# YuePanEdward/MULLS

Hardware: AMD Instinct MI355X
Metric: scan-pair registrations/sec (64-beam ~120k pts, 20 ICP iters); dT vs ref (higher is better)
Workload: dtype f32

## Files before the change

mulls_amd/csrc/accum.h:

```cpp
#pragma once
#include "device_util.h"

namespace
{
__device__ __forceinline__ float w_dist_adaptive(float dist, int iter_num)
{
	const float unit_dist = 30.0f, b_min = 0.7f, b_max = 1.3f, b_step = 0.05f;
	float t = b_min + b_step * iter_num;
	float b_current = (t < b_max) ? t : b_max;
	float temp = (float)(b_current + (1.0 - b_current) * dist / unit_dist);
	temp = (float)((temp > 0.01) ? (double)temp : 0.01);
	return temp;
}
__device__ __forceinline__ float w_intensity(float i1, float i2)
{
	float ratio = fabsf(i1 - i2) / 255.0f;
	return (float)exp(-1.0 * ratio);
}
__device__ __forceinline__ float w_residual(float res, float thre)
{
	return (res > thre) ? ((2 * res * thre + (1 * 1 - 2 * 1) * (thre * thre)) / res / res) : 1.0f;
}
__device__ __forceinline__ int metric_of(int cls) { return (cls == 1 || cls == 3) ? 1 : (cls == 5 ? 2 : 0); }
}


__device__ __forceinline__ float point_wi(const float4 P, const float4 Q) { return w_intensity((float)(P.w + 0.0001), (float)(Q.w + 0.0001)); }

struct AccumCtx
{
	int metric, iter_num;
	bool residual_pass, dist_w, resid_w, inten_w, faithful;
	bool li_diag;
	float class_w, window;
};
__device__ __forceinline__ float class_weight(const RunParams &rp, int cls, bool residual_pass, const int cnt[MULLS_NC])
{
	if (rp.force_class_w)
		return rp.class_w_value;
	if (!residual_pass && rp.w_balance && (cls == 0 || cls == 4))
	{
		const int m1 = cnt[0] + cnt[4], m2 = cnt[2], m3 = cnt[1], m4 = cnt[3];
		const double v = rp.z_xy_ratio * (m2 + 2 * m3 - m4) / (0.0001 + 2.0 * m1);
		return (float)((0.01 > v) ? 0.01 : v);
	}
	return 1.0f;
}
__device__ __forceinline__ AccumCtx accum_ctx(const RunParams &rp, int cls, int iter_num, bool residual_pass, float class_w)
{
	AccumCtx A;
	A.metric = metric_of(cls);
	A.iter_num = iter_num;
	A.residual_pass = residual_pass;
	A.dist_w = rp.w_dist;
	A.resid_w = rp.w_resid && iter_num > rp.resid_from_iter;
	A.inten_w = rp.w_inten;
	A.faithful = rp.faithful;
	A.li_diag = A.metric == 1 && rp.faithful && rp.pull_comb && !residual_pass;
	A.class_w = class_w;
	A.window = A.metric == 0 ? rp.win_pl : (A.metric == 1 ? rp.win_li : rp.win_pt);
	return A;
}

__device__ __forceinline__ float corr_weight(const AccumCtx &A, int metric, const float4 P, const float4 Q, const float4 N, float wi)
{
	const float px = P.x, py = P.y, pz = P.z;
	const float qx = Q.x, qy = Q.y, qz = Q.z;
	const float dist = sqrtf(qx * qx + qy * qy + qz * qz);
	if (metric == 0)
	{
		float ntx = N.x, nty = N.y, ntz = N.z;
		float w = A.class_w;
		float dd = ntx * qx + nty * qy + ntz * qz - ntx * px - nty * py - ntz * pz;
		if (A.dist_w)
			w = w * w_dist_adaptive(dist, A.iter_num);
		if (A.resid_w)
			w = w * w_residual(fabsf(dd), A.window);
		if (A.inten_w)
			w = w * wi;
		return w;
	}
	if (metric == 1)
	{
		float vx = N.x, vy = N.y, vz = N.z;
		float dx = px - qx, dy = py - qy, dz = pz - qz;
		const double b0 = -vy * dz + vz * dy, b1 = -vz * dx + vx * dz, b2 = -vx * dy + vy * dx;
		float ex = (float)fabs(b0), ey = (float)fabs(b1), ez = (float)fabs(b2);
		float ed = sqrtf(ex * ex + ey * ey + ez * ez);
		float wx = A.class_w;
		if (A.dist_w)
			wx *= w_dist_adaptive(dist, A.iter_num);
		if (A.inten_w)
			wx *= wi;
		if (A.resid_w)
			wx = wx * w_residual(ed, A.window);
		return wx;
	}
	float dx = px - qx, dy = py - qy, dz = pz - qz;
	float wx = A.class_w;
	if (A.dist_w)
		wx = wx * w_dist_adaptive(dist, A.iter_num);
	if (A.resid_w)
		wx = wx * w_residual(sqrtf(dx * dx + dy * dy + dz * dz), A.window);
	if (A.inten_w)
		wx = wx * wi;
	return wx;
}

__device__ __forceinline__ constexpr int li_slot(int k) { return k == 0 ? 0 : (k == 6 ? 1 : (k == 11 ? 2 : (k == 15 ? 3 : (k == 18 ? 4 : (k == 20 ? 5 : (k >= 21 ? k - 15 : -1)))))); }
__device__ __forceinline__ constexpr int li_term(int slot) { return slot == 0 ? 0 : (slot == 1 ? 6 : (slot == 2 ? 11 : (slot == 3 ? 15 : (slot == 4 ? 18 : (slot == 5 ? 20 : slot + 15))))); }
#define ACC(k, v)                                              \
	do                                                         \
	{                                                          \
		if (MODE == 1)                                         \
		{                                                      \
			if (li_slot(k) >= T0 && li_slot(k) < T0 + NT)      \
				t[li_slot(k) >= T0 ? li_slot(k) - T0 : 0] = (TS)(v); \
		}                                                      \
		else if ((k) >= T0 && (k) < T0 + NT)                   \
			t[(k)-T0] = (TS)(v);                               \
	} while (0)
template <typename TS, int T0, int NT, int MODE = 0, int METRIC = -1>
__device__ __forceinline__ void point_terms(const AccumCtx &A, const double *x, const float4 P, const float4 Q, const float4 N, float wi, float &wdg, TS t[NT],
											 const float *wpre = nullptr)
{
	const int metric = METRIC >= 0 ? METRIC : A.metric;
	const bool residual_pass = A.residual_pass, faithful = A.faithful;
	const float px = P.x, py = P.y, pz = P.z;
	const float qx = Q.x, qy = Q.y, qz = Q.z;

	if (residual_pass)
	{
				const float cw = wdg;
		if (metric == 0)
		{
			float ntx = N.x, nty = N.y, ntz = N.z;
			float a = ntz * py - nty * pz;
			float b = ntx * pz - ntz * px;
			float c = nty * px - ntx * py;
			float dd = ntx * qx + nty * qy + ntz * qz - ntx * px - nty * py - ntz * pz;
			float res = (float)(ntx * x[0] + nty * x[1] + ntz * x[2] + a * x[3] + b * x[4] + c * x[5] - dd);
			ACC(0, cw * res * res);
			ACC(1, 1.0);
		}
		else
		{
			float dx = px - qx, dy = py - qy, dz = pz - qz;
			double A[3][6], bb[3];
			if (metric == 1)
			{
				float vx = N.x, vy = N.y, vz = N.z;
				A[0][0] = 0;
				A[0][1] = vz;
				A[0][2] = -vy;
				A[0][3] = -vz * pz - vy * py;
				A[0][4] = vy * px;
				A[0][5] = vz * px;
				A[1][0] = -vz;
				A[1][1] = 0;
				A[1][2] = vx;
				A[1][3] = vx * py;
				A[1][4] = -vx * px - vz * pz;
				A[1][5] = vz * py;
				A[2][0] = vy;
				A[2][1] = -vx;
				A[2][2] = 0;
				A[2][3] = vx * pz;
				A[2][4] = vy * pz;
				A[2][5] = -vy * py - vx * px;
				bb[0] = -vz * dy + vy * dz;
				bb[1] = -vx * dz + vz * dx;
				bb[2] = -vy * dx + vx * dy;
			}
			else
			{
				A[0][0] = 1, A[0][1] = 0, A[0][2] = 0, A[0][3] = 0, A[0][4] = pz, A[0][5] = -py;
				A[1][0] = 0, A[1][1] = 1, A[1][2] = 0, A[1][3] = -pz, A[1][4] = 0, A[1][5] = px;
				A[2][0] = 0, A[2][1] = 0, A[2][2] = 1, A[2][3] = py, A[2][4] = -px, A[2][5] = 0;
				bb[0] = -dx, bb[1] = -dy, bb[2] = -dz;
			}
			double r[3];
			for (int k = 0; k < 3; k++)
			{
				double t = 0;
				for (int j = 0; j < 6; j++)
					t += A[k][j] * x[j];
				r[k] = t - bb[k];
			}
			ACC(0, cw * (r[0] * r[0] + r[1] * r[1] + r[2] * r[2]));
			ACC(1, 3.0);
		}
		return;
	}

	if (metric == 0)
	{
		float ntx = N.x, nty = N.y, ntz = N.z;
		float a = ntz * py - nty * pz;
		float b = ntx * pz - ntz * px;
		float c = nty * px - ntx * py;
		float dd = ntx * qx + nty * qy + ntz * qz - ntx * px - nty * py - ntz * pz;
		const float w = wpre ? *wpre : corr_weight(A, 0, P, Q, N, wi);
		wdg = w;
		ACC(0, w * ntx * ntx);
		ACC(1, w * ntx * nty);
		ACC(2, w * ntx * ntz);
		ACC(3, w * a * ntx);
		ACC(4, w * b * ntx);
		ACC(5, w * c * ntx);
		ACC(6, w * nty * nty);
		ACC(7, w * nty * ntz);
		ACC(8, w * a * nty);
		ACC(9, w * b * nty);
		ACC(10, w * c * nty);
		ACC(11, w * ntz * ntz);
		ACC(12, w * a * ntz);
// ... 181 lines not shown
	{
		__syncthreads();
		if (threadIdx.x < 21 && li_slot((int)threadIdx.x) < 0)
			part[threadIdx.x] = 0.0;
		if (HALF)
		{
			slot_terms<double, 0, 6, 1, LANES>(A, x, valid, P, Q, N, wi, wdg, static_cast<double *>(R));
			__syncthreads();
			reduce_terms<double, 0, 6, 1, LANES>(static_cast<const double *>(R), part);
			__syncthreads();
			slot_terms<double, 6, 6, 1, LANES>(A, x, valid, P, Q, N, wi, wdg, static_cast<double *>(R));
			__syncthreads();
			reduce_terms<double, 6, 6, 1, LANES>(static_cast<const double *>(R), part);
		}
		else
		{
			slot_terms<double, 0, 12, 1, LANES>(A, x, valid, P, Q, N, wi, wdg, static_cast<double *>(R));
			__syncthreads();
			reduce_terms<double, 0, 12, 1, LANES>(static_cast<const double *>(R), part);
		}
	}
	else if (A.metric == 1 && HALF)
	{
		__syncthreads();
		slot_terms<double, 0, 7, 0, LANES>(A, x, valid, P, Q, N, wi, wdg, static_cast<double *>(R));
		__syncthreads();
		reduce_terms<double, 0, 7, 0, LANES>(static_cast<const double *>(R), part);
		__syncthreads();
		slot_terms<double, 7, 7, 0, LANES>(A, x, valid, P, Q, N, wi, wdg, static_cast<double *>(R));
		__syncthreads();
		reduce_terms<double, 7, 7, 0, LANES>(static_cast<const double *>(R), part);
		__syncthreads();
		slot_terms<double, 14, 7, 0, LANES>(A, x, valid, P, Q, N, wi, wdg, static_cast<double *>(R));
		__syncthreads();
		reduce_terms<double, 14, 7, 0, LANES>(static_cast<const double *>(R), part);
		__syncthreads();
		slot_terms<double, 21, 6, 0, LANES>(A, x, valid, P, Q, N, wi, wdg, static_cast<double *>(R));
		__syncthreads();
		reduce_terms<double, 21, 6, 0, LANES>(static_cast<const double *>(R), part);
	}
	else if (A.metric == 1)
	{
		__syncthreads();
		slot_terms<double, 0, 13, 0, LANES>(A, x, valid, P, Q, N, wi, wdg, static_cast<double *>(R));
		__syncthreads();
		reduce_terms<double, 0, 13, 0, LANES>(static_cast<const double *>(R), part);
		__syncthreads();
		slot_terms<double, 13, 13, 0, LANES>(A, x, valid, P, Q, N, wi, wdg, static_cast<double *>(R));
		__syncthreads();
		reduce_terms<double, 13, 13, 0, LANES>(static_cast<const double *>(R), part);
		__syncthreads();
		slot_terms<double, 26, 1, 0, LANES>(A, x, valid, P, Q, N, wi, wdg, static_cast<double *>(R));
		__syncthreads();
		reduce_terms<double, 26, 1, 0, LANES>(static_cast<const double *>(R), part);
	}
	else if (HALF)
	{
		__syncthreads();
		slot_terms<float, 0, 14, 0, LANES>(A, x, valid, P, Q, N, wi, wdg, static_cast<float *>(R));
		__syncthreads();
		reduce_terms<float, 0, 14, 0, LANES>(static_cast<const float *>(R), part);
		__syncthreads();
		slot_terms<float, 14, 13, 0, LANES>(A, x, valid, P, Q, N, wi, wdg, static_cast<float *>(R));
		__syncthreads();
		reduce_terms<float, 14, 13, 0, LANES>(static_cast<const float *>(R), part);
	}
	else
	{
		__syncthreads();
		slot_terms<float, 0, 27, 0, LANES>(A, x, valid, P, Q, N, wi, wdg, static_cast<float *>(R));
		__syncthreads();
		reduce_terms<float, 0, 27, 0, LANES>(static_cast<const float *>(R), part);
	}
	__syncthreads();
}

template <bool HALF = false, int LANES = MULLS_ACC_LANES>
__device__ __forceinline__ void trip_sum(const AccumCtx &A, const double *x, const CloudDesc &d, uint32_t trip0, const float4 *__restrict__ spos,
										  const float4 *__restrict__ mq, const uint8_t *__restrict__ flag, float *__restrict__ wd, void *R, double *part)
{
	const uint32_t s = trip0 + threadIdx.x;
	bool valid = false;
	float4 P = make_float4(0.0f, 0.0f, 0.0f, 0.0f), Q = P, N = P;
	float w = 0.0f, w0 = 0.0f;
	uint32_t g = 0;
	if (s < d.src_n)
	{
		g = d.src_off + s;
		const uint32_t f = flag[g];
		P = spos[g], Q = mq[2u * g], N = mq[2u * g + 1u];
		w = w0 = wd[g];
		valid = (f & (MULLS_F_ALIVE | MULLS_F_VALID)) == (MULLS_F_ALIVE | MULLS_F_VALID);
	}
	trip_sum_regs<HALF, LANES>(A, x, valid, P, Q, N, w, R, part);
	if (valid && __float_as_uint(w) != __float_as_uint(w0))
		wd[g] = w;
}

__device__ __forceinline__ void combine_rows(const RunParams &rp, bool want_residual, const double (*sums)[MULLS_NTERM_PAD], double *comb, int t)
{
	const int order[MULLS_NC] = {0, 2, 4, 1, 3, 5};
	double val;
	if (want_residual)
	{
		val = 0.0;
		if (t < 2)
			for (int i = 0; i < MULLS_NC; i++)
				if (rp.used[order[i]])
					val += sums[order[i]][t];
	}
	else if (t < 21)
	{
		int r = 0, rem = t;
		while (rem >= 6 - r)
		{
			rem -= 6 - r;
			r++;
		}
		const bool diag = rem == 0;
		double lower = 0.0, upper = 0.0;
		for (int i = 0; i < MULLS_NC; i++)
		{
			const int cls = order[i];
			if (!rp.used[cls])
				continue;
			const double v = sums[cls][t];
			if (metric_of(cls) == 1 && !diag)
				upper += v;
			else
				lower += v;
		}
		val = diag ? lower : (rp.faithful ? lower : lower + upper);
	}
	else
	{
		val = 0.0;
		for (int i = 0; i < MULLS_NC; i++)
			if (rp.used[order[i]])
				val += sums[order[i]][t];
	}
	comb[t] = val;
}
```

mulls_amd/csrc/batch.cpp:

```cpp
#include "batch.h"

namespace mulls_drv
{
void rows12(const double colmajor[16], double out[12])
{
	for (int r = 0; r < 3; r++)
		for (int c = 0; c < 4; c++)
			out[r * 4 + c] = colmajor[r + 4 * c];
}


void fill_crop_box(const RunParams &rp, const double tgt_bound[6], const uint32_t keys[6], mulls_result &R)
{
	R.cropped = rp.crop ? 1 : 0;
	for (int k = 0; k < 3 && rp.crop; k++)
	{
		const uint32_t kmin = keys[k], kmax = keys[3 + k];
		const bool none = kmin == 0xffffffffu && kmax == 0u;
		const double mmin = none ? 1.7976931348623157e308 : (double)ord_to_float(kmin);
		const double mmax = none ? -1.7976931348623157e308 : (double)ord_to_float(kmax);
		const double b1min = tgt_bound[k], b1max = tgt_bound[3 + k];
		const float pad = 1.0f;
		R.crop_box[k] = ((b1min > mmin) ? b1min : mmin) - pad;
		R.crop_box[3 + k] = ((b1max < mmax) ? b1max : mmax) + pad;
// ... 241 lines not shown
		for (int p = 0; p < B->n; p++)
			for (int c = 0; c < MULLS_NC; c++)
				if (P->used_feature_type[c] == '1')
					for (uint32_t s = 0; s < B->descs_h[p * MULLS_NC + c].src_cap; s += MULLS_SRC_PER_BLOCK)
					{
						Job j = {(uint32_t)p, (uint32_t)c, s, MULLS_SRC_PER_BLOCK};
						B->cjobs_h.push_back(j);
					}
	}
	B->bjobs_h.clear();
	B->fjobs_h.clear();
	B->ejobs_h.clear();
	bool any_class_job = false;
	for (int p = 0; p < B->n; p++)
		for (int c = 0; c < MULLS_NC; c++)
		{
			const CloudDesc &d = B->descs_h[p * MULLS_NC + c];
			if (!used[c] || d.src_cap == 0 || d.tier != MULLS_TIER_BM)
				continue;
			const bool whole = mode == 3 && d.src_cap <= MULLS_BIG_CLASS_MAX;
			if (whole)
			{
				Job j = {(uint32_t)p, (uint32_t)c, 0u, d.src_cap | MULLS_JOB_CLASS};
				B->bjobs_h.push_back(j);
				any_class_job = true;
			}
			for (uint32_t s = 0; s < d.src_cap; s += MULLS_SRC_PER_BLOCK)
			{
				Job j = {(uint32_t)p, (uint32_t)c, s, MULLS_SRC_PER_BLOCK};
				B->ejobs_h.push_back(j);
				if (!whole)
				{
					B->bjobs_h.push_back(j);
					B->fjobs_h.push_back(j);
				}
			}
		}
	if (!any_class_job)
		B->ejobs_h.clear();
	B->cjobs_dev_h = B->cjobs_h;
	{
		auto first_of = [&](uint32_t pair) {
			return std::lower_bound(B->cjobs_dev_h.begin(), B->cjobs_dev_h.end(), pair, [](const Job &j, uint32_t q) { return j.pair < q; });
		};
		auto cost = [&](const Job &j) {
			const CloudDesc &d = B->descs_h[j.pair * MULLS_NC + j.cls];
			return (uint64_t)j.count * (uint64_t)(64u + d.tgt_n0 / 64u);
		};
		for (int k = 0; k < nsub; k++)
			std::stable_sort(first_of((uint32_t)((long)B->n * k / nsub)), first_of((uint32_t)((long)B->n * (k + 1) / nsub)),
							 [&](const Job &a, const Job &b) { return cost(a) > cost(b); });
	}
	B->tjobs_h.clear();
	for (int p = 0; p < B->n; p++)
		for (int c = 0; c < MULLS_NC; c++)
			if (P->used_feature_type[c] == '1' && B->descs_h[p * MULLS_NC + c].tier == MULLS_TIER_BM)
				for (uint32_t s = 0; s < B->descs_h[p * MULLS_NC + c].tgt_n0; s += MULLS_BLOCK)
				{
					Job j = {(uint32_t)p, (uint32_t)c, s, 0};
					B->tjobs_h.push_back(j);
				}
	B->ajobs_h.clear();
	{
		for (int k = 0; k < 2; k++)
			for (int b = 0; b < 4; b++)
				B->ajob_split[k][b] = 0;
		for (int k = 0; k < nsub; k++)
		{
			const uint32_t lo = (uint32_t)((long)B->n * k / nsub), hi = (uint32_t)((long)B->n * (k + 1) / nsub);
			for (int bucket = 0; bucket < 3; bucket++)
			{
				B->ajob_split[k][bucket] = (uint32_t)B->ajobs_h.size();
				for (uint32_t j = 0; j < (uint32_t)B->jobs_h.size(); j++)
				{
					const Job &jb = B->jobs_h[j];
					if (jb.start % 1024u != 0u || jb.pair < lo || jb.pair >= hi)
						continue;
					const uint32_t slots = std::min(1024u, B->descs_h[jb.pair * MULLS_NC + jb.cls].src_cap - jb.start);
					if ((slots > 512u ? 0 : (slots > 256u ? 1 : 2)) == bucket)
						B->ajobs_h.push_back(j);
				}
			}
			B->ajob_split[k][3] = (uint32_t)B->ajobs_h.size();
		}
	}
	{
		std::vector<uint32_t> &tab = B->setup_tab_h;
		tab.clear();
		const uint32_t *trips = tgt_grid_bucket_trips();
		for (int k = 0; k < MULLS_TG_BUCKETS; k++)
		{
			B->tg_split[k] = (uint32_t)tab.size();
			for (uint32_t ci = 0; ci < (uint32_t)B->descs_h.size(); ci++)
			{
				const CloudDesc &d = B->descs_h[ci];
				const uint32_t need = (d.tgt_n0 + 511u) / 512u;
				if (d.tier == MULLS_TIER_LDS && need <= trips[k] && (k == 0 || need > trips[k - 1]))
					tab.push_back(ci);
			}
		}
		B->tg_split[MULLS_TG_BUCKETS] = (uint32_t)tab.size();
		for (int seg = 0; seg < 3; seg++)
		{
			B->crop_split[seg] = (uint32_t)tab.size();
			for (uint32_t ci = 0; ci < (uint32_t)B->descs_h.size(); ci++)
			{
				const bool lds = B->descs_h[ci].tier == MULLS_TIER_LDS;
				if (seg == 0 ? !B->src_one_wg[ci / MULLS_NC] : (seg == 1 ? !lds : lds))
					tab.push_back(ci * 2u + (seg ? 1u : 0u));
			}
		}
		B->crop_split[3] = (uint32_t)tab.size();
		B->srcp_split[0] = (uint32_t)tab.size();
		for (int p = 0; p < B->n; p++)
			if (B->src_one_wg[p])
				tab.push_back((uint32_t)p);
		B->srcp_split[1] = (uint32_t)tab.size();
	}
	B->njobs = (uint32_t)B->jobs_h.size();
	B->jobs_key = key;
}

int wait_epoch_word(mulls_ctx *ctx, volatile uint32_t *word, uint32_t want, hipEvent_t last, hipStream_t stream)
{
	const auto t0 = std::chrono::steady_clock::now();
	bool seen = false;
	for (uint64_t spins = 0;; spins++)
	{
		if (*word == want)
		{
			std::atomic_thread_fence(std::memory_order_acquire);
			seen = true;
			break;
		}
		if ((spins & 0xfff) == 0xfff && std::chrono::duration<double>(std::chrono::steady_clock::now() - t0).count() > 2.0)
			break;
	}
	if (seen && ctx->profiling != 1)
		return MULLS_OK;
	if (seen && last)
	{
		hipError_t e;
		while ((e = hipEventQuery(last)) == hipErrorNotReady)
		{
		}
		if (e == hipSuccess)
			return MULLS_OK;
	}
	HIPCHK(ctx, hipStreamSynchronize(stream ? stream : ctx->stream));
	if (*word != want)
	{
		ctx->err = "device did not publish the iteration epoch";
		return MULLS_E_HIP;
	}
	return MULLS_OK;
}

void unpack_out(const mulls_batch *B, const uint8_t used[MULLS_NC], int p, PairOut &o, bool comb)
{
	int n_used = 0;
	for (int c = 0; c < MULLS_NC; c++)
		n_used += used[c] ? 1 : 0;
	const size_t row = sizeof(double) * MULLS_NTERM_PAD, rec = 128 + row * (size_t)(comb ? 1 : n_used);
	const unsigned char *src = reinterpret_cast<const unsigned char *>(B->outs_h) + rec * (size_t)p;
	std::memcpy(o.n_valid, src, 128);
	src += 128;
// ... 366 lines not shown
	B->fill_ms = std::chrono::duration<double>(std::chrono::steady_clock::now() - t_fill0).count() * 1e3;
	B->fill_pack_ms = pack_s * 1e3;
	B->fill_bytes = (uint64_t)stage_rec * 16;
	return MULLS_OK;
}

int prepare_run(mulls_ctx *ctx, mulls_batch *B, const mulls_params *P_jobs, RunParams &rp, uint32_t *lds_cap_out, int *tier_out, int nsub, bool allow_mixed)
{
	hipStream_t st = ctx->stream;
	const int n = B->n;
	uint32_t lds_cap = 0;
	const int tier = choose_tier(ctx, B, rp.used, &lds_cap, allow_mixed ? P_jobs : nullptr);
	if (tier < 0)
	{
		ctx->err = "nn mode 3 (grid staged in LDS) needs every searched target class cloud to hold <= 9728 points";
		return MULLS_E_INVALID;
	}
	build_jobs(B, P_jobs, nsub > 0 ? nsub : subbatch_count(ctx, n), tier);
	*lds_cap_out = lds_cap;
	*tier_out = tier;
	int n_used = 0;
	for (int c = 0; c < MULLS_NC; c++)
		n_used += rp.used[c];
	rp.bm_h0 = 0.0f;
	rp.bm_maxwords = rp.bm_stride = 0u;
	rp.grid_h0 = ctx->opt[MULLS_OPT_GRID_H0] > 0.0 ? std::max(0.05f, (float)ctx->opt[MULLS_OPT_GRID_H0]) : MULLS_GRID_H0;
	rp.lds_dedup = 0;
	rp.grid_maxcells = MULLS_MAXCELLS;
	rp.cell_stride = ((rp.grid_maxcells + 1u + 15u) & ~15u);
	if (tier == 2 || tier == 3)
	{
		rp.grid_maxcells = lds_cells_for(lds_cap);
		const bool class_level = tier == 3 || (!B->cjobs_h.empty() && B->cjobs_h[0].count != MULLS_SRC_PER_BLOCK);
		const long left = 160L * 1024L - 64L - (long)MULLS_LDS_CELL_RESERVE - (long)MULLS_LDS_QCHUNK * 16L - (long)MULLS_LDS_AUX - (long)lds_cap * 18L;
		const bool dedup_fits = !rp.normal_shooting && left / 2 - 8 >= 4096 && ctx->opt[MULLS_OPT_LDS_DEDUP] != 0.0;
		if (tier == 3 && !dedup_fits)
		{
			ctx->err = "internal: a mixed batch whose LDS-tier clouds do not fit the on-chip duplicate table";
			return MULLS_E_INVALID;
		}
		if (class_level && dedup_fits)
		{
			rp.lds_dedup = 1;
			rp.grid_maxcells = (uint32_t)std::min<long>(left / 2 - 8, (long)MULLS_MAXCELLS);
		}
		rp.cell_stride = ((rp.grid_maxcells + 1u + 15u) & ~15u);
	}
	const size_t nl = B->lclouds_h.size();
	if (nl)
	{
		rp.bm_h0 = MULLS_BM_H0;
		rp.bm_auto = 1;
		if (ctx->opt[MULLS_OPT_BM_H0] > 0.0)
		{
			rp.bm_h0 = std::max(0.05f, (float)ctx->opt[MULLS_OPT_BM_H0]);
			rp.bm_auto = 0;
		}
		size_t words = std::min<size_t>(MULLS_BM_MAXWORDS, MULLS_BM_TOTALWORDS / nl);
		words = std::max<size_t>(words & ~(size_t)15, 4096);
		rp.bm_maxwords = rp.bm_stride = (uint32_t)words;
	}

	bool grew = false, g2 = false;
	int rc = MULLS_OK;
	auto A = [&](int r) { if (rc == MULLS_OK) rc = r; };
	A(grow(ctx, &B->jobs, &B->cap_jobs[0], (size_t)B->njobs, &g2));
	grew |= g2;
	A(grow(ctx, &B->partial, &B->cap_jobs[1], (size_t)B->njobs * MULLS_NTERM));
	A(grow(ctx, &B->tjobs, &B->cap_jobs[2], B->tjobs_h.size(), &g2));
	grew |= g2;
	A(grow(ctx, &B->cjobs, &B->cap_jobs[3], B->cjobs_h.size(), &g2));
	grew |= g2;
	A(grow(ctx, &B->bjobs, &B->cap_bjobs[0], B->bjobs_h.size(), &g2));
	grew |= g2;
	A(grow(ctx, &B->fjobs, &B->cap_bjobs[1], B->fjobs_h.size(), &g2));
	grew |= g2;
	A(grow(ctx, &B->lclouds, &B->cap_bjobs[2], B->lclouds_h.size(), &g2));
	grew |= g2;
	A(grow(ctx, &B->ejobs, &B->cap_bjobs[3], B->ejobs_h.size(), &g2));
	grew |= g2;
	A(grow(ctx, &B->wl, &B->cap_wl, B->cjobs_h.size()));
	A(grow(ctx, &B->ajobs, &B->cap_ajobs, B->ajobs_h.size(), &g2));
	grew |= g2;
	A(grow(ctx, &B->setup_tab, &B->cap_setup_tab, B->setup_tab_h.size(), &g2));
	grew |= g2;
	if (!B->wl_ctr)
		A(dmalloc(ctx, &B->wl_ctr, 16));
	if (rc == MULLS_OK)
		HIPCHK(ctx, hipMemsetAsync(B->wl_ctr, 0, 16 * sizeof(uint32_t), st));
	A(grow(ctx, &B->descs_init, &B->cap_jobs[4], B->descs_h.size(), &g2));
	grew |= g2;
	A(grow(ctx, &B->bbox_init, &B->cap_jobs[5], (size_t)n * 6, &g2));
	grew |= g2;
	if (tier == 2 || tier == 3)
		A(grow(ctx, &B->cell_start, &B->cap_cells[1], (size_t)n * n_used * rp.cell_stride));
	if (nl)
	{
		const size_t words = nl * (size_t)rp.bm_stride, cells = B->n_tgt + (size_t)n * MULLS_NC + 1;
		A(grow(ctx, &B->bm, &B->cap_bm, words));
		A(grow(ctx, &B->pf, &B->cap_pf, words));
		A(grow(ctx, &B->bm_cs, &B->cap_bm_cs, cells));
		A(grow(ctx, &B->cell_cnt, &B->cap_cells[0], cells));
		A(grow(ctx, &B->bm_rank, &B->cap_bm_rank, 2 * B->n_tgt));
		if (rc == MULLS_OK)
		{
			HIPCHK(ctx, hipMemsetAsync(B->cell_cnt, 0, cells * sizeof(uint32_t), st));
		}
	}
	if (rc != MULLS_OK)
		return rc;
	if (grew || B->dev_key != B->jobs_key || B->dev_key.empty())
	{
		SegCopier up(ctx);
		up.add_host(B->jobs, B->jobs_h.data(), sizeof(Job) * B->njobs);
		up.add_host(B->tjobs, B->tjobs_h.data(), sizeof(Job) * B->tjobs_h.size());
		up.add_host(B->cjobs, B->cjobs_dev_h.data(), sizeof(Job) * B->cjobs_dev_h.size());
		up.add_host(B->bjobs, B->bjobs_h.data(), sizeof(Job) * B->bjobs_h.size());
		up.add_host(B->fjobs, B->fjobs_h.data(), sizeof(Job) * B->fjobs_h.size());
		up.add_host(B->ejobs, B->ejobs_h.data(), sizeof(Job) * B->ejobs_h.size());
		up.add_host(B->lclouds, B->lclouds_h.data(), sizeof(uint32_t) * B->lclouds_h.size());
		up.add_host(B->ajobs, B->ajobs_h.data(), sizeof(uint32_t) * B->ajobs_h.size());
		up.add_host(B->setup_tab, B->setup_tab_h.data(), sizeof(uint32_t) * B->setup_tab_h.size());
		up.add_host(B->descs_init, B->descs_h.data(), sizeof(CloudDesc) * B->descs_h.size());
		up.add_host(B->bbox_init, B->bbox_h, sizeof(uint32_t) * 6 * n);
		if (up.flush(st) != MULLS_OK)
		{
			(void)hipStreamSynchronize(st);
			return MULLS_E_HIP;
		}
		HIPCHK(ctx, hipStreamSynchronize(st));
		B->dev_key = B->jobs_key;
	}
	{
		SegCopier reset(ctx);
		reset.add_dev(B->descs, B->descs_init, sizeof(CloudDesc) * B->descs_h.size());
		reset.add_dev(B->bbox, B->bbox_init, sizeof(uint32_t) * 6 * n);
		if (reset.flush(st) != MULLS_OK)
			return MULLS_E_HIP;
	}
	return MULLS_OK;
}


bool setup_former_shape(const RunParams &rp) { return rp.debug_stop == 30u; }

void queue_clone_crop(hipStream_t st, const mulls_batch *B, const RunParams &rp)
{
	const uint32_t nbig_segs = (uint32_t)B->big_segs_h.size(), nbig_clouds = (uint32_t)B->big_clouds_h.size();
	if (setup_former_shape(rp))
	{
		launch_clone_src(st, *B, rp, (uint32_t)B->setup_jobs_h.size());
		launch_crop(st, *B, rp, (uint32_t)B->n, nbig_segs, nbig_clouds);
		return;
	}
	const bool one_wg = !rp.undistort;
	launch_clone_src(st, *B, rp, one_wg ? B->n_setup_jobs_rest : (uint32_t)B->setup_jobs_h.size());
	if (one_wg)
		launch_src_setup(st, *B, rp, B->setup_tab + B->srcp_split[0], B->srcp_split[1] - B->srcp_split[0]);
	if (one_wg)
		launch_crop(st, *B, rp, (uint32_t)B->n, nbig_segs, nbig_clouds, B->setup_tab + B->crop_split[0], B->crop_split[rp.tgt_map ? 2 : 3] - B->crop_split[0]);
	else
		launch_crop(st, *B, rp, (uint32_t)B->n, nbig_segs, nbig_clouds);
}

int apply_keep_masks(mulls_ctx *ctx, const mulls_batch *B, const std::vector<uint8_t> &skeep, const std::vector<uint8_t> &tkeep, const char *what)
{
	hipStream_t st = ctx->stream;
	uint8_t *d_sk = nullptr, *d_tk = nullptr;
	if (dmalloc(ctx, &d_sk, skeep.size()) != MULLS_OK || dmalloc(ctx, &d_tk, tkeep.size()) != MULLS_OK)
		return MULLS_E_HIP;
	hipError_t e = hipMemcpyAsync(d_sk, skeep.data(), skeep.size(), hipMemcpyHostToDevice, st);
	if (e == hipSuccess)
		e = hipMemcpyAsync(d_tk, tkeep.data(), tkeep.size(), hipMemcpyHostToDevice, st);
	if (e == hipSuccess)
	{
		launch_thin(st, *B, (uint32_t)B->n, d_sk, d_tk);
		e = hipStreamSynchronize(st);
	}
	(void)hipFree(d_sk);
	(void)hipFree(d_tk);
	if (e != hipSuccess)
	{
		ctx->err = std::string(what) + hipGetErrorString(e);
		return MULLS_E_HIP;
	}
	return MULLS_OK;
}

void queue_target_grids(hipStream_t st, const mulls_batch *B, const RunParams &rp, int tier, bool fused_tgt)
{
	if (fused_tgt && setup_former_shape(rp))
		(void)launch_tgt_grid(st, *B, rp, (uint32_t)B->n);
	else if (fused_tgt)
		(void)launch_tgt_grid(st, *B, rp, (uint32_t)B->n, B->setup_tab, B->tg_split);
	else if (tier == 2)
		launch_grid_build_sort(st, *B, rp, (uint32_t)B->n);
	launch_bm_build(st, *B, (uint32_t)B->lclouds_h.size(), (uint32_t)B->tjobs_h.size());
}

int queue_tier_search(mulls_ctx *ctx, const mulls_batch *B, const RunParams &rp, int tier, uint32_t lds_cap, uint32_t parity)
{
	hipStream_t st = ctx->stream;
	if (tier == 2)
	{
// ... 51 lines not shown
```

mulls_amd/csrc/batch.h:

```cpp
#pragma once
#include <hip/hip_runtime_api.h>

#include <algorithm>
#include <atomic>
#include <chrono>
#include <cmath>
#include <cstdio>
#include <cstdlib>
#include <cstring>
#include <string>
#include <vector>

#include "../../include/mulls_hip.h"
#include "device_types.h"
#include "hostmath.h"
#include "icp_step.h"
#include "launch.h"
#include "ctx.h"

struct SegCopier
{
	mulls_ctx *ctx;
	std::vector<CopySeg> segs;
	struct Pending
	{
		void *dst;
		const void *src;
		size_t bytes;
	};
	std::vector<Pending> host;
	explicit SegCopier(mulls_ctx *c) : ctx(c) {}
	void add_host(void *dst, const void *src, size_t bytes)
	{
		if (bytes)
			host.push_back({dst, src, bytes});
	}
	void add_dev(void *dst, const void *src, size_t bytes)
	{
		const size_t piece = (size_t)0xfffffff0u;
		for (size_t off = 0; off < bytes; off += piece)
		{
			const size_t b = std::min(piece, bytes - off);
			segs.push_back({(unsigned long long)(uintptr_t)dst + off, (unsigned long long)(uintptr_t)src + off, (uint32_t)b, 0u});
		}
	}
	int flush(hipStream_t st);
};

struct mulls_batch : BatchDev
{
	int n = 0;
	size_t n_src = 0, n_tgt = 0;
	std::vector<CloudDesc> descs_h;
	std::vector<PairSetup> setup_h;
	std::vector<Job> setup_jobs_h;
	uint32_t n_setup_jobs_rest = 0;
	std::vector<uint8_t> src_one_wg;
	std::vector<uint32_t> setup_tab_h;
	uint32_t tg_split[MULLS_TG_BUCKETS + 1] = {}, crop_split[4] = {}, srcp_split[2] = {};
	size_t cap_setup_tab = 0;
	std::vector<Job> big_segs_h, big_clouds_h;
	uint32_t n_big_tgt = 0;
	std::vector<Job> jobs_h;
	std::vector<Job> cjobs_h;
	std::vector<Job> cjobs_dev_h;
	std::vector<Job> bjobs_h;
	std::vector<Job> fjobs_h;
	std::vector<Job> ejobs_h;
	std::vector<uint32_t> lclouds_h;
	int tier_mode = -1;
	std::vector<Job> tjobs_h;
	std::vector<uint32_t> ajobs_h;
	uint32_t ajob_split[2][4] = {{0, 0, 0, 0}, {0, 0, 0, 0}};
	IcpOut *icp_outs_pin = nullptr;
	size_t cap_icp_pin = 0;
	std::string jobs_key;
	uint32_t njobs = 0;
	uint4 *nn_cand = nullptr;
	LiveWord *live_mask = nullptr;
	size_t cap_live = 0;
	uint32_t tick = 1;
	size_t cap_outs = 0;
	size_t cap_big[4] = {};
	size_t cap_bjobs[4] = {};
	size_t cap_bm_cs = 0;
	size_t cap_bm_rank = 0;
	size_t cap_ajobs = 0;
	size_t cap_icp_outs = 0;
	size_t cap_steps = 0;
	uint32_t epoch2 = 0, epoch3 = 0;
	int nsub = 1;
	double fill_ms = 0.0, fill_pack_ms = 0.0;
	uint64_t fill_bytes = 0;
	size_t cap_wl = 0;
	unsigned long long *dbg = nullptr;
	size_t cap_bm = 0, cap_pf = 0;
	PairState *states_h = nullptr;
	PairOut *outs_h = nullptr;
	volatile uint32_t *epoch_h = nullptr;
	uint32_t *epoch_dev = nullptr;
	uint32_t epoch = 0;
	uint32_t epoch1 = 0;
	uint32_t *bbox_h = nullptr;
	uint8_t *upload_h = nullptr;
	CloudDesc *descs_init = nullptr;
	uint32_t *bbox_init = nullptr;
	std::string dev_key;
	size_t cap_jobs[6] = {}, cap_cells[2] = {};
	size_t cap_stage = 0, cap_src[13] = {}, cap_tgt[5] = {}, cap_pairs[5] = {}, cap_setup_jobs = 0, cap_pin[4] = {};
};

namespace mulls_drv
{
using mulls::Mat4;
using mulls::Mat6;

inline float ord_to_float(uint32_t k)
{
	const uint32_t u = (k & 0x80000000u) ? (k & 0x7fffffffu) : ~k;
	float f;
	std::memcpy(&f, &u, sizeof(f));
	return f;
}
inline int metric_of(int c) { return (c == MULLS_PILLAR || c == MULLS_BEAM) ? 1 : (c == MULLS_VERTEX ? 2 : 0); }
inline int packed(int r, int c) { return r * 6 - r * (r - 1) / 2 + (c - r); }
void rows12(const double colmajor[16], double out[12]);

struct PairHost : mulls::PairIter
{
	bool first = true;
	uint32_t alive_prev[MULLS_NC];
};

void fill_crop_box(const RunParams &rp, const double tgt_bound[6], const uint32_t keys[6], mulls_result &R);
int check_params(mulls_ctx *ctx, const mulls_params *P);
void init_cert(const mulls_ctx *ctx, RunParams &rp);
int subbatch_count(const mulls_ctx *ctx, int n);
void options_init(mulls_ctx *ctx);
bool option_value_ok(int option, double *value);
uint32_t lds_dedup_max_pts();
void assign_tiers(mulls_batch *B, const uint8_t used[MULLS_NC], int mode);
void build_jobs(mulls_batch *B, const mulls_params *P, int nsub, int mode);
int wait_epoch_word(mulls_ctx *ctx, volatile uint32_t *word, uint32_t want, hipEvent_t last = nullptr, hipStream_t stream = nullptr);
inline int wait_epoch(mulls_ctx *ctx, mulls_batch *B) { return wait_epoch_word(ctx, B->epoch_h, B->epoch); }
void unpack_out(const mulls_batch *B, const uint8_t used[MULLS_NC], int p, PairOut &o, bool comb = false);
uint32_t lds_cells_for(uint32_t cap);
int choose_tier(const mulls_ctx *ctx, const mulls_batch *B, const uint8_t used[MULLS_NC], uint32_t *lds_cap, const mulls_params *P_mixed = nullptr);
int batch_fill(mulls_ctx *ctx, mulls_batch *B, const mulls_pair *pairs, int n, const mulls_params *P = nullptr);
int prepare_run(mulls_ctx *ctx, mulls_batch *B, const mulls_params *P_jobs, RunParams &rp, uint32_t *lds_cap_out, int *tier_out, int nsub = 0, bool allow_mixed = false);
void queue_clone_crop(hipStream_t st, const mulls_batch *B, const RunParams &rp);
bool setup_former_shape(const RunParams &rp);
int apply_keep_masks(mulls_ctx *ctx, const mulls_batch *B, const std::vector<uint8_t> &skeep, const std::vector<uint8_t> &tkeep, const char *what);
void queue_target_grids(hipStream_t st, const mulls_batch *B, const RunParams &rp, int tier, bool fused_tgt);
int queue_tier_search(mulls_ctx *ctx, const mulls_batch *B, const RunParams &rp, int tier, uint32_t lds_cap, uint32_t parity);
mulls::IcpConst icp_const(const mulls_params *P);
int take_epochs(mulls_ctx *ctx, mulls_batch *B, uint32_t n, RunParams &rp);

struct EvTimer
{
	mulls_ctx *ctx;
	hipStream_t stream = nullptr;
	int base = 0;
	int used = 0;
	bool open = false;
	double *slot[5];
	void begin(double *acc)
	{
		open = ctx->profiling == 1 || (ctx->profiling == 2 && acc == &ctx->prof.ms_nn);
		if (!open)
			return;
		slot[used / 2] = acc;
		(void)hipEventRecord(ctx->ev[base + used], stream ? stream : ctx->stream);
// ... 27 lines not shown
```

mulls_amd/csrc/big_tier.h:

```cpp
#pragma once
#include "lds_tier.h"

namespace
{
__device__ __forceinline__ void grp16_min2(nnkey &bk, float &sec)
{
	nnkey g = bk;
	dpp_min_step<0xB1>(g);
	dpp_min_step<0x4E>(g);
	dpp_min_step<0x141>(g);
	dpp_min_step<0x140>(g);
	float c = (bk == g) ? sec : key_dist(bk);
	dpp_fmin_step<0xB1>(c);
	dpp_fmin_step<0x4E>(c);
	dpp_fmin_step<0x141>(c);
	dpp_fmin_step<0x140>(c);
	sec = c;
	bk = g;
}
__device__ __forceinline__ void take_one(const float4 c, float px, float py, float pz, nnkey &bk, float &sec)
{
	const float dx = px - c.x, dy = py - c.y, dz = pz - c.z;
	const float dist = (dx * dx + dy * dy) + dz * dz;
	sec = __builtin_amdgcn_fmed3f(sec, dist, key_dist(bk));
// ... 437 lines not shown
		}
	}
	if (U)
	{
		const bool dbg = rp.dbg_ticks && rp.debug_stop == 21u;
		const unsigned long long t_dbg = dbg ? wall_clock64() : 0ull;
		const uint32_t sub = threadIdx.x & (MULLS_GRID_GROUP - 1u), grp = threadIdx.x / MULLS_GRID_GROUP;
		const bool probe_own = tgt_n >= 4u * g.nocc;
		for (uint32_t i = grp; i < U; i += BLK / MULLS_GRID_GROUP)
		{
			nnkey bk;
			float sec, Rfin;
			CandOut co = {0xffffffffu, 0xffffffffu, 0.0f};
			search_query_bm(g, B, ts, CL.uq[i], C.r, C.m, sub, probe_own, bk, sec, Rfin, co);
			if (sub == 0)
			{
				const uint32_t slot = CL.us[i] & ~MULLS_US16_KCERT, s = q0 + slot, gi = d.src_off + s;
				const float best = key_dist(bk);
				const int bi = (int)(uint32_t)bk;
				const bool matched = bi >= 0 && !((double)best > C.max_dist_sqr);
				if (class_level)
					CL.res[slot] = make_uint2(matched ? (uint32_t)bi : 0xffffffffu, __float_as_uint(best));
				else
				{
					nn_idx[gi] = matched ? bi : -1;
					nn_d2[gi] = best;
				}
				const float lb_new = fminf(sqrtf(sec), Rfin);
				hint2[gi] = make_int2(bi, __float_as_int(lb_new));
				if (C.cand)
					C.cand[gi] = make_uint4(co.cx, co.cy, __float_as_uint(fminf(sqrtf(co.b2), Rfin) - lb_new), C.epoch);
				if (matched)
				{
					matched_cnt++;
					if (C.gate)
						claim((uint32_t)bi, s);
				}
			}
		}
		if (dbg)
		{
			__syncthreads();
			if (threadIdx.x == 0)
			{
				atomicAdd(&rp.dbg_ticks[13], (unsigned long long)U);
				atomicAdd(&rp.dbg_ticks[7], wall_clock64() - t_dbg);
			}
		}
	}
	for (int off = 32; off > 0; off >>= 1)
		matched_cnt += __shfl_down(matched_cnt, off);
	if (!class_level)
	{
#pragma unroll
		for (int k = 0; k < TRIPS; k++)
			if ((ST[k] & MULLS_FS_ALIVE) && M[k] != MULLS_NEEDS_SEARCH)
			{
				const uint32_t gi = d.src_off + q0 + threadIdx.x + (uint32_t)k * BLK;
				nn_idx[gi] = M[k];
				nn_d2[gi] = D0[k];
			}
		if ((threadIdx.x & 63) == 0)
			CL.red[threadIdx.x >> 6] = matched_cnt;
		__syncthreads();
		if (threadIdx.x == 0)
		{
			uint32_t any = 0;
			for (int w = 0; w < BLK / 64; w++)
				any |= CL.red[w];
			if (any)
				d.n_matched = 1u;
		}
		return;
	}
	if ((threadIdx.x & 63) == 0)
		CL.red[threadIdx.x >> 6] = matched_cnt;
	__threadfence_block();
	__syncthreads();
	uint32_t total_matched = 0;
	for (int w = 0; w < BLK / 64; w++)
		total_matched += CL.red[w];

	const float thr = ps.thr[cls], max_sqr = thr * thr;
	const bool any_match = total_matched > 0u, strict = rp.rej_strict != 0;
	uint32_t n_alive = 0, n_valid = 0;
#pragma unroll
	for (int k = 0; k < TRIPS; k++)
	{
		const uint32_t st = ST[k];
		if (!(st & MULLS_FS_ALIVE))
			continue;
		const uint32_t s = q0 + threadIdx.x + (uint32_t)k * BLK, gi = d.src_off + s;
		int32_t m = M[k];
		float dist = D0[k];
		bool standing = (st & MULLS_FS_STANDING) != 0;
		if (m == MULLS_NEEDS_SEARCH)
		{
			const uint2 found = CL.res[threadIdx.x + (uint32_t)k * BLK];
			m = (int32_t)found.x;
			standing = m >= 0 && __float_as_int(dist) == m;
			dist = __uint_as_float(found.y);
		}
		if (hashed && m >= 0 && big_hash_get(CL, (uint32_t)m) != s)
			m = -1;
		bool alive = true, valid, dir_ok = (st & MULLS_FS_DIR_OK) != 0;
		if (any_match)
		{
			valid = m >= 0;
			if (C.gate && m < 0)
			{
				alive = false;
				valid = false;
			}
			if (valid)
			{
				valid = strict ? dist < max_sqr : !(dist > max_sqr);
				if (valid)
				{
					wd[gi] = dist;
					if (!standing)
					{
						match[gi] = m;
						const float4 q2 = tpos[d.tgt_off + (uint32_t)m], n2 = tnrm[d.tgt_off + (uint32_t)m];
						mq[2u * gi] = q2;
						mq[2u * gi + 1u] = n2;
						if (normal_check)
						{
							const float3 n1 = *reinterpret_cast<const float3 *>(snrm + gi);
							const double dot = (double)n1.x * (double)n2.x + (double)n1.y * (double)n2.y + (double)n1.z * (double)n2.z;
							const float c = (float)fabs(dot);
							dir_ok = !((double)c < rp.cos_bearing);
						}
					}
				}
			}
		}
		else if (C.gate)
		{
			alive = false;
			valid = false;
		}
		else
			valid = (st & MULLS_FS_VALID) != 0;
		if (valid && normal_check && !dir_ok)
			valid = false;
		const uint32_t nf = (alive ? MULLS_F_ALIVE : 0u) | (valid ? MULLS_F_VALID : 0u);
		if (nf != (st & (MULLS_FS_ALIVE | MULLS_FS_VALID)))
			flag[gi] = (uint8_t)nf;
		n_alive += alive ? 1u : 0u;
		n_valid += valid ? 1u : 0u;
	}
	for (int off = 32; off > 0; off >>= 1)
	{
		n_alive += __shfl_down(n_alive, off);
		n_valid += __shfl_down(n_valid, off);
	}
	if ((threadIdx.x & 63) == 0)
	{
		CL.red[BLK / 64 + (threadIdx.x >> 6)] = n_alive;
		CL.red[2 * (BLK / 64) + (threadIdx.x >> 6)] = n_valid;
	}
	__syncthreads();
	if (threadIdx.x == 0)
	{
		uint32_t ta = 0, tv = 0;
		for (int w = 0; w < BLK / 64; w++)
		{
			ta += CL.red[BLK / 64 + w];
			tv += CL.red[2 * (BLK / 64) + w];
		}
		d.n_matched = total_matched;
		d.alive_next = ta;
		d.valid_next = tv;
		d.n_search = U;
	}
}
}
```

mulls_amd/csrc/device_types.h:

```cpp
#pragma once
#include <stdint.h>

#define MULLS_NC 6
#define MULLS_NTERM 27
#define MULLS_BLOCK 256
#define MULLS_SRC_PER_THREAD 2
#define MULLS_SRC_PER_BLOCK (MULLS_BLOCK * MULLS_SRC_PER_THREAD)
#define MULLS_NN_BLOCK 128
#define MULLS_NN_PTS 4
#define MULLS_TILE 2048

#define MULLS_MAXCELLS 65536u
#define MULLS_BM_MAXWORDS (1u << 22)
#define MULLS_BM_TOTALWORDS (1u << 28)
#define MULLS_BM_H0 0.25f
#define MULLS_LDS_BLOCK 1024
#define MULLS_LDS_MAXPTS 9728u
#define MULLS_ACC_BLOCK 128
#define MULLS_LDS_QCHUNK 1024u
#define MULLS_LDS_AUX (320u + 2u * MULLS_LDS_QCHUNK)
#define MULLS_CERT_BLOCK 512
#define MULLS_CERT_SMALL 64u
#define MULLS_CERT_SMALL_LOCKSTEP 512u
#define MULLS_LDS_CELL_RESERVE 9216
// ... 40 lines not shown
	uint32_t src_cap;
	uint32_t big_slot;
	uint32_t src_big_slot;
	uint32_t n_search;
	uint32_t stage_fmt;
	uint32_t tier;
	uint32_t grid_slot;
	uint32_t src_c;
	uint32_t compacted;
};
struct LiveWord
{
	unsigned long long alive;
	uint32_t below, pad_;
};
#define MULLS_STAGE_AOS48 0u
#define MULLS_STAGE_PACK32 1u
#define MULLS_STAGE_PACK28 2u

struct GridDesc
{
	float ox, oy, oz;
	float inv_h, h;
	uint32_t nx, ny, nz;
	uint32_t ncell;
	uint32_t cell_off;
	uint32_t wpr;
	uint32_t nocc;
};

struct PairState
{
	double T[12];
	double x[6];
	float thr[MULLS_NC];
	int32_t iter;
	int32_t active;
	int32_t want_residual;
	int32_t pad_[3];
};

struct PairSetup
{
	double guess[12];
	double tgt_bound[6];
	double inv_q[4];
	double inv_t[4];
};

#define MULLS_NTERM_PAD 28
struct PairOut
{
	double sums[MULLS_NC][MULLS_NTERM_PAD];
	double comb[MULLS_NTERM_PAD];
	uint32_t n_valid[MULLS_NC];
	uint32_t n_alive[MULLS_NC];
	uint32_t src_n[MULLS_NC];
	uint32_t tgt_n[MULLS_NC];
	uint32_t bbox[6];
	uint32_t pad_[2];
};

struct IcpOut
{
	double T[16];
	double info[36];
	double sigma2;
	unsigned long long src_pts, tgt_pts, corr_pts;
	float ratio;
	int32_t code, iters, singular, trace_len;
	uint32_t ncorr[MULLS_NC], nsrc0[MULLS_NC], ntgt0[MULLS_NC], bbox[6];
	uint32_t pad_;
	unsigned long long tgt_job_pts, pair_evals;
};

struct Job
{
	uint32_t pair;
	uint32_t cls;
	uint32_t start;
	uint32_t count;
};

#define MULLS_COPY_SEGS 24
struct CopySeg
{
	unsigned long long dst, src;
	uint32_t bytes, pad_;
};
struct CopyArgs
{
	CopySeg seg[MULLS_COPY_SEGS];
};

struct RunParams
{
	uint8_t used[MULLS_NC];
	uint8_t w_balance, w_resid, w_dist, w_inten;
	uint8_t crop;
	uint8_t undistort;
	uint8_t normal_shooting;
	uint8_t faithful;
	uint8_t rej_strict;
	float z_xy_ratio;
	float win_pt, win_pl, win_li;
	uint8_t force_class_w;
	uint8_t bm_auto;
	float class_w_value;
	double cos_bearing;
	int32_t resid_from_iter;
	uint32_t debug_stop;
	uint32_t cell_stride;
	uint32_t grid_maxcells;
	float grid_h0;
	float bm_h0;
	uint32_t bm_maxwords;
	uint32_t bm_stride;
	uint32_t pull_comb;
	uint32_t lds_dedup;
	uint32_t tick_base;
	uint32_t cert;
	float cert_slack_min, cert_slack_max, cert_slack_rate;
	uint32_t kcert;
	uint32_t kcert_min;
	uint4 *cand;
	const float4 *tgt_stage;
	const uint16_t *tgt_map;
	unsigned long long *dbg_ticks;
	LiveWord *live_mask;
};
#define MULLS_COMPACT_MAX (3u * MULLS_CERT_BLOCK)
```

mulls_amd/csrc/device_util.h:

```cpp

#pragma once
#include <hip/hip_runtime.h>
#include <stdint.h>

#include "device_types.h"

#pragma clang fp contract(off)

__device__ __forceinline__ uint32_t xcd_job(uint32_t b, uint32_t n)
{
	const uint32_t q = n >> 3, r = n & 7u, x = b & 7u;
	return x * q + min(x, r) + (b >> 3);
}

namespace
{

typedef float f2 __attribute__((ext_vector_type(2)));

__device__ __forceinline__ uint32_t f2ord(float f)
{
	uint32_t u = __float_as_uint(f);
	return (u & 0x80000000u) ? ~u : (u | 0x80000000u);
}
__device__ __forceinline__ float ord2f(uint32_t k)
{
	uint32_t u = (k & 0x80000000u) ? (k & 0x7fffffffu) : ~k;
	return __uint_as_float(u);
}

__device__ __forceinline__ void load_staged(const float4 *__restrict__ stage, uint32_t off, uint32_t fmt, uint32_t n, uint32_t i, float4 &pos, float4 &nrm)
{
	if (fmt == MULLS_STAGE_PACK32)
	{
		pos = stage[(size_t)off + i];
		nrm = stage[(size_t)off + n + i];
	}
	else if (fmt == MULLS_STAGE_PACK28)
	{
		pos = stage[(size_t)off + i];
		const float *f = reinterpret_cast<const float *>(stage + (size_t)off + n) + 3u * (size_t)i;
		nrm = make_float4(f[0], f[1], f[2], 0.0f);
	}
	else
	{
		const float4 *rec = stage + (size_t)off + (size_t)i * 3;
		const float4 a = rec[0], b = rec[1], c = rec[2];
		pos = make_float4(a.x, a.y, a.z, c.x);
		nrm = make_float4(b.x, b.y, b.z, c.y);
	}
}
__device__ __forceinline__ void identity_step(float4 &p, float4 &n)
{
	const double x = p.x, y = p.y, z = p.z, nx = n.x, ny = n.y, nz = n.z;
	p.x = (float)(1.0 * x + 0.0 * y + 0.0 * z + 0.0);
	p.y = (float)(0.0 * x + 1.0 * y + 0.0 * z + 0.0);
	p.z = (float)(0.0 * x + 0.0 * y + 1.0 * z + 0.0);
	n.x = (float)(1.0 * nx + 0.0 * ny + 0.0 * nz);
	n.y = (float)(0.0 * nx + 1.0 * ny + 0.0 * nz);
	n.z = (float)(0.0 * nx + 0.0 * ny + 1.0 * nz);
}
__device__ __forceinline__ float4 load_staged_pos(const float4 *__restrict__ stage, uint32_t off, uint32_t fmt, uint32_t i)
{
	return fmt == MULLS_STAGE_AOS48 ? stage[(size_t)off + (size_t)i * 3] : stage[(size_t)off + i];
}

__device__ __forceinline__ void tgt_record(const float4 *__restrict__ tgt_stage, const uint16_t *__restrict__ tgt_map, const CloudDesc &d, uint32_t m,
											const float4 *__restrict__ tpos, const float4 *__restrict__ tnrm, float4 &q, float4 &n)
{
	if (tgt_map)
		load_staged(tgt_stage, d.tgt_stage, (d.stage_fmt >> 2) & 3u, d.tgt_n0, tgt_map[d.tgt_off + m], q, n);
	else
		q = tpos[d.tgt_off + m], n = tnrm[d.tgt_off + m];
}
__device__ __forceinline__ float4 tgt_point(const float4 *__restrict__ tgt_stage, const uint16_t *__restrict__ tgt_map, const CloudDesc &d, uint32_t m,
											 const float4 *__restrict__ tpos)
{
	return tgt_map ? load_staged_pos(tgt_stage, d.tgt_stage, (d.stage_fmt >> 2) & 3u, tgt_map[d.tgt_off + m]) : tpos[d.tgt_off + m];
}

__device__ __forceinline__ uint32_t live_word_base(const CloudDesc &d, uint32_t cloud) { return (d.src_off >> 6) + cloud; }

__device__ __forceinline__ bool class_called(const RunParams &rp, const CloudDesc &d, int cls)
{
	return rp.used[cls] && d.alive_cur >= 3u && d.tgt_n >= 3u;
}

__device__ __forceinline__ uint32_t block_sum_u32(uint32_t v, uint32_t *lds4)
{
	for (int off = 32; off > 0; off >>= 1)
		v += __shfl_down(v, off);
	int lane = threadIdx.x & 63, wave = threadIdx.x >> 6;
	__syncthreads();
	if (lane == 0)
		lds4[wave] = v;
	__syncthreads();
	return lds4[0] + lds4[1] + lds4[2] + lds4[3];
}

}

namespace
{
__device__ __forceinline__ int grid_cell(float v, float o, float inv_h, uint32_t n)
{
	const float c = floorf((v - o) * inv_h);
	return (int)fminf(fmaxf(c, 0.0f), (float)(n - 1u));
}
__device__ __forceinline__ uint32_t grid_cell_id(const GridDesc &g, float x, float y, float z)
{
	return ((uint32_t)grid_cell(z, g.oz, g.inv_h, g.nz) * g.ny + (uint32_t)grid_cell(y, g.oy, g.inv_h, g.ny)) * g.nx +
		   (uint32_t)grid_cell(x, g.ox, g.inv_h, g.nx);
}
struct BmGrid
{
	const unsigned long long *bm;
	const uint32_t *pf;
	const uint32_t *cs;
};
__device__ __forceinline__ void bm_row_range(const BmGrid &B, uint32_t rowword, uint32_t xa, uint32_t xb, uint32_t &lo, uint32_t &hi)
{
	const uint32_t wa = rowword + (xa >> 6), wb = rowword + (xb >> 6);
	const unsigned long long A = B.bm[wa], Z = B.bm[wb];
	const uint32_t r0 = B.pf[wa] + (uint32_t)__popcll(A & ((1ull << (xa & 63u)) - 1ull));
	const uint32_t r1 = B.pf[wb] + (uint32_t)__popcll(Z & (~0ull >> (63u - (xb & 63u))));
	lo = hi = 0;
	if (r1 > r0)
	{
		lo = B.cs[r0];
		hi = B.cs[r1];
	}
}
__device__ __forceinline__ void grid_scan_box(const GridDesc &g, const BmGrid &B, const float4 *__restrict__ ts,
											   float px, float py, float pz, float R, uint32_t sub, float &best, int &bi)
{
	const float Rm = R * 1.0001f + 1e-4f;
	const int x0 = grid_cell(px - Rm, g.ox, g.inv_h, g.nx), x1 = grid_cell(px + Rm, g.ox, g.inv_h, g.nx);
	const int y0 = grid_cell(py - Rm, g.oy, g.inv_h, g.ny), y1 = grid_cell(py + Rm, g.oy, g.inv_h, g.ny);
	const int z0 = grid_cell(pz - Rm, g.oz, g.inv_h, g.nz), z1 = grid_cell(pz + Rm, g.oz, g.inv_h, g.nz);
	const int nyc = y1 - y0 + 1, nrows = nyc * (z1 - z0 + 1);
	const uint32_t gshift = (threadIdx.x & 63u) & ~(MULLS_GRID_GROUP - 1u);
	for (int base = 0; base < nrows; base += (int)MULLS_GRID_GROUP)
	{
		const int j = base + (int)sub;
		uint32_t lo = 0, hi = 0;
		if (j < nrows)
		{
			const uint32_t rowword = ((uint32_t)(z0 + j / nyc) * g.ny + (uint32_t)(y0 + j % nyc)) * g.wpr;
			bm_row_range(B, rowword, (uint32_t)x0, (uint32_t)x1, lo, hi);
		}
		const uint32_t nonempty = (uint32_t)(__ballot(hi > lo) >> gshift) & 0xffffu;
		if (!nonempty)
			continue;
#pragma unroll
		for (int half = 0; half < 2; half++)
		{
			if (!((nonempty >> (8 * half)) & 0xffu))
				continue;
			float4 q[8];
			bool ok[8];
#pragma unroll
			for (int jj = 0; jj < 8; jj++)
			{
				const uint32_t t = __shfl(lo, 8 * half + jj, MULLS_GRID_GROUP) + sub;
				ok[jj] = t < __shfl(hi, 8 * half + jj, MULLS_GRID_GROUP);
				if (ok[jj])
					q[jj] = ts[t];
			}
#pragma unroll
// ... 117 lines not shown
```

mulls_amd/csrc/driver.cpp:

```cpp
#include "batch.h"

#include <sched.h>
#include <cstdio>
#include <cstdlib>

#include <mutex>
#include <unordered_map>
namespace
{
std::mutex g_stagger_mu;
std::unordered_map<void *, void *> g_stagger;
}
void staggered_note(void *p, void *base)
{
	std::lock_guard<std::mutex> lk(g_stagger_mu);
	g_stagger[p] = base;
}
void *staggered_base(void *p, bool forget)
{
	std::lock_guard<std::mutex> lk(g_stagger_mu);
	auto it = g_stagger.find(p);
	if (it == g_stagger.end())
		return p;
	void *b = it->second;
// ... 231 lines not shown
			if (e)
				(void)hipEventDestroy(e);
		if (ctx->ev_setup)
			(void)hipEventDestroy(ctx->ev_setup);
		if (ctx->stream2)
			(void)hipStreamDestroy(ctx->stream2);
		if (ctx->stream)
			(void)hipStreamDestroy(ctx->stream);
		delete ctx;
	}

	const char *mulls_last_error(const mulls_ctx *ctx) { return ctx ? ctx->err.c_str() : "null context"; }

	int mulls_set_profiling(mulls_ctx *ctx, int on)
	try
	{
		if (!ctx)
			return MULLS_E_INVALID;
		ctx->profiling = on == 2 ? 2 : (on != 0 ? 1 : 0);
		return MULLS_OK;
	}
	catch (...)
	{
		return mulls::abi_caught(const_cast<mulls_ctx *>(ctx));
	}

	int mulls_get_profile(const mulls_ctx *ctx, mulls_profile *out)
	try
	{
		if (!ctx || !out)
			return MULLS_E_INVALID;
		*out = ctx->prof;
		return MULLS_OK;
	}
	catch (...)
	{
		return mulls::abi_caught(const_cast<mulls_ctx *>(ctx));
	}

	void *mulls_stream(mulls_ctx *ctx) { return ctx ? (void *)ctx->stream : nullptr; }

	int mulls_set_option(mulls_ctx *ctx, int option, double value)
	{
		if (!ctx || !option_known(option))
			return MULLS_E_INVALID;
		if (!option_value_ok(option, &value))
		{
			ctx->err = "mulls_set_option: value out of the option's range";
			return MULLS_E_INVALID;
		}
		ctx->opt[option] = value;
		return MULLS_OK;
	}
	int mulls_get_option(const mulls_ctx *ctx, int option, double *value)
	{
		if (!ctx || !value || !option_known(option))
			return MULLS_E_INVALID;
		*value = ctx->opt[option];
		return MULLS_OK;
	}

	int mulls_set_nn_mode(mulls_ctx *ctx, int mode)
	try
	{
		if (!ctx || mode < 0 || mode > 4)
			return MULLS_E_INVALID;
		ctx->nn_mode = mode;
		return MULLS_OK;
	}
	catch (...)
	{
		return mulls::abi_caught(const_cast<mulls_ctx *>(ctx));
	}

	void mulls_batch_destroy(mulls_ctx *ctx, mulls_batch *B)
	{
		if (!B)
			return;
		if (ctx)
			(void)hipSetDevice(ctx->device);
		void *dev[] = {B->stage, B->tmp_pos, B->tmp_nrm, B->spos, B->snrm, B->tpos, B->tnrm, B->flag, B->match, B->nn_idx, B->nn_hint, B->nn_cand, B->live_mask, B->mq, B->wd,
					   B->nn_d2, B->winner, B->descs, B->setup, B->states, B->outs, B->ticket, B->bbox, B->setup_jobs, B->big_segs, B->big_clouds, B->seg_cnt, B->big_box, B->jobs, B->partial,
					   B->tjobs, B->cjobs, B->bjobs, B->fjobs, B->ejobs, B->lclouds, B->bm_cs, B->wl, B->wl_ctr, B->grids, B->tsorted, B->tmap, B->dbg, B->cell_cnt, B->cell_start, B->bm, B->pf, B->descs_init, B->bbox_init,
					   B->ajobs, B->icp_outs, B->steps, B->bm_rank, B->setup_tab};
		for (void *p : dev)
			if (p)
				staggered_free(p);
		if (B->states_h)
			(void)hipHostFree(B->states_h);
		if (B->outs_h)
			(void)hipHostFree(B->outs_h);
		if (B->bbox_h)
			(void)hipHostFree(B->bbox_h);
		if (B->epoch_h)
			(void)hipHostFree((void *)B->epoch_h);
		if (B->upload_h)
			(void)hipHostFree(B->upload_h);
		if (B->icp_outs_pin)
			(void)hipHostFree(B->icp_outs_pin);
		delete B;
	}

	int mulls_batch_create(mulls_ctx *ctx, const mulls_pair *pairs, int n, mulls_batch **out)
	try
	{
		if (!ctx || !pairs || n <= 0 || !out)
			return MULLS_E_INVALID;
		*out = nullptr;
		mulls_batch *B = new mulls_batch();
		const int rc = batch_fill(ctx, B, pairs, n);
		if (rc != MULLS_OK)
		{
			mulls_batch_destroy(ctx, B);
			return rc;
		}
		*out = B;
		return MULLS_OK;
	}
	catch (...)
	{
		return mulls::abi_caught(const_cast<mulls_ctx *>(ctx));
	}


	int mulls_icp_batch(mulls_ctx *ctx, const mulls_pair *pairs, int n, const mulls_params *params, mulls_result *results)
	try
	{
		if (!ctx)
			return MULLS_E_INVALID;
		int rc = check_params(ctx, params);
		if (rc != MULLS_OK)
			return rc;
		if (!pairs || n <= 0 || !results)
			return MULLS_E_INVALID;
		if (!ctx->scratch)
			ctx->scratch = new mulls_batch();
		rc = batch_fill(ctx, ctx->scratch, pairs, n, params);
		if (rc != MULLS_OK)
			return rc;
		rc = mulls_batch_run(ctx, ctx->scratch, params, results);
		ctx->prof.ms_stage = ctx->scratch->fill_ms, ctx->prof.ms_stage_pack = ctx->scratch->fill_pack_ms, ctx->prof.stage_bytes = ctx->scratch->fill_bytes;
		return rc;
	}
	catch (...)
	{
		return mulls::abi_caught(const_cast<mulls_ctx *>(ctx));
	}

	int mulls_icp(mulls_ctx *ctx, const mulls_pair *pair, const mulls_params *params, mulls_result *result)
	try
	{
		return mulls_icp_batch(ctx, pair, 1, params, result);
	}
	catch (...)
	{
		return mulls::abi_caught(const_cast<mulls_ctx *>(ctx));
	}

}
```

mulls_amd/csrc/k_reduce.hip:

```cpp
#include "device_util.h"
#include "accum.h"
#include "solve_wave.h"

template <int LANES, int MIN_WG>
__global__ __launch_bounds__(LANES, MIN_WG) void k_accum(const uint32_t *__restrict__ leaders, const Job *__restrict__ jobs, const CloudDesc *__restrict__ descs,
														 const PairState *__restrict__ states, RunParams rp, const float4 *__restrict__ spos,
														 const float4 *__restrict__ mq, const uint8_t *__restrict__ flag, float *__restrict__ wd,
														 double *__restrict__ partial)
{
	extern __shared__ __attribute__((aligned(16))) unsigned char lds_raw[];
	__shared__ double part[MULLS_NTERM_PAD];
	const uint32_t job_idx = leaders[xcd_job(blockIdx.x, gridDim.x)];
	const Job job = jobs[job_idx];
	const PairState &ps = states[job.pair];
	if (!ps.active && !ps.want_residual)
		return;
	const CloudDesc *pd = descs + job.pair * MULLS_NC;
	const bool residual_pass = ps.want_residual != 0;
	int cnt[MULLS_NC];
	for (int c = 0; c < MULLS_NC; c++)
		cnt[c] = (int)(class_called(rp, pd[c], c) ? pd[c].valid_next : pd[c].n_valid);
	const AccumCtx A = accum_ctx(rp, job.cls, ps.iter, residual_pass, class_weight(rp, job.cls, residual_pass, cnt));
	trip_sum<true, LANES>(A, ps.x, pd[job.cls], job.start, spos, mq, flag, wd, lds_raw, part);
	if (threadIdx.x < MULLS_NTERM)
		partial[(size_t)job_idx * MULLS_NTERM + threadIdx.x] = part[threadIdx.x];
}

namespace
{
template <typename TS, int W0, int WIN, int MODE, int METRIC, int A0>
__device__ __forceinline__ void add_window(const AccumCtx &A, const double *x, const float4 P, const float4 Q, const float4 N, float wi, float &w, double *acc, const float *wpre)
{
	TS t[WIN];
#pragma unroll
	for (int k = 0; k < WIN; k++)
		t[k] = (TS)0;
	point_terms<TS, W0, WIN, MODE, METRIC>(A, x, P, Q, N, wi, w, t, wpre);
#pragma unroll
	for (int k = 0; k < WIN; k++)
		acc[W0 - A0 + k] += (double)t[k];
}
#ifndef MULLS_ACCW_WIN
#define MULLS_ACCW_WIN 9
#endif
#ifndef MULLS_ACCW_WIN_D
#define MULLS_ACCW_WIN_D 12
#endif
template <typename TS, int W0, int REM, int MODE, int METRIC, int A0>
__device__ __forceinline__ void add_windows(const AccumCtx &A, const double *x, const float4 P, const float4 Q, const float4 N, float wi, float &w, double *acc, const float *wpre)
{
	constexpr int WMAX = sizeof(TS) == 8 ? MULLS_ACCW_WIN_D : MULLS_ACCW_WIN;
	constexpr int WIN = REM < WMAX ? REM : WMAX;
	add_window<TS, W0, WIN, MODE, METRIC, A0>(A, x, P, Q, N, wi, w, acc, wpre);
	if constexpr (REM > WIN)
		add_windows<TS, W0 + WIN, REM - WIN, MODE, METRIC, A0>(A, x, P, Q, N, wi, w, acc, wpre);
}
template <typename TS, int NT, int MODE, int METRIC, int T0, int NTW>
__device__ __forceinline__ void wave_trip(const AccumCtx &A, const double *x, const CloudDesc &d, uint32_t trip0, const float4 *__restrict__ spos, const float4 *__restrict__ mq,
										   const uint8_t *__restrict__ flag, float *__restrict__ wd, double *__restrict__ out, bool owner, const LiveWord *__restrict__ live,
										   uint32_t cloud)
{
	const uint32_t lane = threadIdx.x & 63u;
	const uint32_t src_n = d.src_n, src_off = d.src_off;
	const uint32_t n_here = min(src_n - trip0, (uint32_t)MULLS_ACC_LANES), iters = (n_here + 63u) >> 6;
	const bool compacted = d.compacted != 0u;
	const uint32_t last = src_off + (compacted ? max(d.src_c, 1u) : src_n) - 1u;
	const unsigned long long below_me = (1ull << lane) - 1ull;
	static_assert(MULLS_ACC_LANES / 64 <= 64, "one LiveWord per lane covers a trip");
	uint32_t lw_lo = 0u, lw_hi = 0u, lw_below = 0u;
	if (compacted)
	{
		const LiveWord w = live[live_word_base(d, cloud) + (trip0 >> 6) + min(lane, iters - 1u)];
		lw_lo = (uint32_t)w.alive, lw_hi = (uint32_t)(w.alive >> 32), lw_below = w.below;
	}
	struct Rec
	{
		uint32_t f, g;
		bool live;
		float4 P, Q;
		float3 N;
		float w;
	};
	const bool need_w = A.residual_pass, writes_w = !A.residual_pass && (METRIC != 2 || !A.faithful);
	auto load = [&](uint32_t i) {
		Rec r;
		uint32_t g = src_off + trip0 + lane + 64u * i;
		r.live = true;
		if (compacted)
		{
			const unsigned long long alive = ((unsigned long long)(uint32_t)__builtin_amdgcn_readlane((int)lw_hi, (int)i) << 32) | (uint32_t)__builtin_amdgcn_readlane((int)lw_lo, (int)i);
			g = src_off + (uint32_t)__builtin_amdgcn_readlane((int)lw_below, (int)i) + (uint32_t)__popcll(alive & below_me);
			r.live = ((alive >> lane) & 1ull) != 0ull;
		}
		g = min(g, last);
		r.g = g;
		r.f = flag[g];
		r.P = spos[g], r.Q = mq[2u * g], r.N = *reinterpret_cast<const float3 *>(mq + 2u * g + 1u);
		r.w = need_w ? wd[g] : 0.0f;
		return r;
	};
	double acc[NTW];
#pragma unroll
	for (int k = 0; k < NTW; k++)
		acc[k] = -0.0;
#define MULLS_PIN_REC(r) asm volatile("" : "+v"((r).f), "+v"((r).P.x), "+v"((r).Q.x), "+v"((r).N.x), "+v"((r).w))
#if MULLS_ACCW_PREFETCH
	Rec cur = load(0);
#endif
	for (uint32_t i = 0; i < iters; i++)
	{
#if MULLS_ACCW_PREFETCH
		MULLS_PIN_REC(cur);
		Rec nxt = cur;
		if (i + 1u < iters)
			nxt = load(i + 1u);
#else
		Rec cur = load(i);
		MULLS_PIN_REC(cur);
#endif
		const uint32_t s = trip0 + lane + 64u * i;
		const bool valid = s < src_n && cur.live && (cur.f & (MULLS_F_ALIVE | MULLS_F_VALID)) == (MULLS_F_ALIVE | MULLS_F_VALID);
		if (valid)
		{
			float w = cur.w;
			const float4 N4 = make_float4(cur.N.x, cur.N.y, cur.N.z, 0.0f);
			const float wi = (A.inten_w && !A.residual_pass) ? point_wi(cur.P, cur.Q) : 1.0f;
			const float wpre = A.residual_pass ? 0.0f : corr_weight(A, METRIC, cur.P, cur.Q, N4, wi);
			add_windows<TS, T0, NTW, MODE, METRIC, T0>(A, x, cur.P, cur.Q, N4, wi, w, acc, A.residual_pass ? nullptr : &wpre);
			if (owner && writes_w)
				wd[cur.g] = w;
		}
#if MULLS_ACCW_PREFETCH
		cur = nxt;
#endif
	}
	if (NTW == NT && lane < MULLS_NTERM)
	{
		const bool has = MODE == 1 ? li_slot((int)lane) >= 0 : (int)lane < NT;
		if (!has)
			out[lane] = 0.0;
	}
#pragma unroll
	for (int k = 0; k < NTW; k++)
	{
		double sum = acc[k];
		sum = dpp_add_f64<0xB1>(sum);
		sum = dpp_add_f64<0x4E>(sum);
		sum = dpp_add_f64<0x141>(sum);
		sum = dpp_add_f64<0x140>(sum);
		sum = dpp_add_f64_rows<0x142, 0xa>(sum);
		sum = dpp_add_f64_rows<0x143, 0xc>(sum);
		acc[k] = sum;
	}
	if (lane == 63u)
	{
#pragma unroll
		for (int k = 0; k < NTW; k++)
			out[MODE == 1 ? li_term(T0 + k) : T0 + k] = acc[k];
	}
}
}

#ifndef MULLS_ACCW_SPLIT
#define MULLS_ACCW_SPLIT 1
#endif
#ifndef MULLS_ACCW_PREFETCH
#define MULLS_ACCW_PREFETCH 0
#endif
#ifndef MULLS_ACCW_OCC
#define MULLS_ACCW_OCC 4
#endif
#define MULLS_ACCW_WAVES 4
__global__ __launch_bounds__(64 * MULLS_ACCW_WAVES, MULLS_ACCW_OCC) void k_accum_wave(const uint32_t *__restrict__ leaders, uint32_t n_trips, const Job *__restrict__ jobs,
																					   const CloudDesc *__restrict__ descs, const PairState *__restrict__ states, RunParams rp,
																					   const float4 *__restrict__ spos, const float4 *__restrict__ mq, const uint8_t *__restrict__ flag,
																					   float *__restrict__ wd, double *__restrict__ partial)
{
	const uint32_t wave = threadIdx.x >> 6, part = wave % MULLS_ACCW_SPLIT;
	const uint32_t trip = blockIdx.x * (MULLS_ACCW_WAVES / MULLS_ACCW_SPLIT) + wave / MULLS_ACCW_SPLIT;
	if (trip >= n_trips)
		return;
	const uint32_t job_idx = leaders[trip];
	const Job job = jobs[job_idx];
	const PairState &ps = states[job.pair];
	if (!ps.active && !ps.want_residual)
		return;
	const CloudDesc *pd = descs + job.pair * MULLS_NC;
	const bool residual_pass = ps.want_residual != 0;
	int cnt[MULLS_NC];
	for (int c = 0; c < MULLS_NC; c++)
		cnt[c] = (int)(class_called(rp, pd[c], c) ? pd[c].valid_next : pd[c].n_valid);
	const AccumCtx A = accum_ctx(rp, job.cls, ps.iter, residual_pass, class_weight(rp, job.cls, residual_pass, cnt));
	const CloudDesc &d = pd[job.cls];
	const uint32_t ci = job.pair * MULLS_NC + job.cls;
	double *out = partial + (size_t)job_idx * MULLS_NTERM;
	if (d.src_n <= job.start)
	{
		if (part == 0u && (threadIdx.x & 63u) < MULLS_NTERM)
			out[threadIdx.x & 63u] = 0.0;
		return;
	}
	if (residual_pass || A.metric == 1)
	{
		if (part)
			return;
		if (!residual_pass)
			wave_trip<double, 12, 1, 1, 0, 12>(A, ps.x, d, job.start, spos, mq, flag, wd, out, true, rp.live_mask, ci);
		else if (A.metric == 0)
			wave_trip<double, 2, 0, 0, 0, 2>(A, ps.x, d, job.start, spos, mq, flag, wd, out, true, rp.live_mask, ci);
		else if (A.metric == 1)
			wave_trip<double, 2, 0, 1, 0, 2>(A, ps.x, d, job.start, spos, mq, flag, wd, out, true, rp.live_mask, ci);
		else
			wave_trip<double, 2, 0, 2, 0, 2>(A, ps.x, d, job.start, spos, mq, flag, wd, out, true, rp.live_mask, ci);
	}
#if MULLS_ACCW_SPLIT == 2
	else if (A.metric == 0)
	{
		if (part == 0u)
			wave_trip<float, 27, 0, 0, 0, 14>(A, ps.x, d, job.start, spos, mq, flag, wd, out, true, rp.live_mask, ci);
		else
			wave_trip<float, 27, 0, 0, 14, 13>(A, ps.x, d, job.start, spos, mq, flag, wd, out, false, rp.live_mask, ci);
	}
	else
	{
		if (part == 0u)
			wave_trip<float, 27, 0, 2, 0, 14>(A, ps.x, d, job.start, spos, mq, flag, wd, out, true, rp.live_mask, ci);
		else
			wave_trip<float, 27, 0, 2, 14, 13>(A, ps.x, d, job.start, spos, mq, flag, wd, out, false, rp.live_mask, ci);
	}
#else
	else if (A.metric == 0)
		wave_trip<float, 27, 0, 0, 0, 27>(A, ps.x, d, job.start, spos, mq, flag, wd, out, true, rp.live_mask, ci);
	else
		wave_trip<float, 27, 0, 2, 0, 27>(A, ps.x, d, job.start, spos, mq, flag, wd, out, true, rp.live_mask, ci);
#endif
}

namespace
{
struct FinishLds
{
	double sums[MULLS_NC][MULLS_NTERM_PAD], comb[MULLS_NTERM_PAD];
	uint32_t cnt[32];
};
__device__ __forceinline__ void finish_pair(CloudDesc *pd, const PairState &ps, const RunParams &rp, const double *__restrict__ partial,
											 PairOut &o, const uint32_t *__restrict__ pair_bbox, FinishLds *M = nullptr)
{
	if (threadIdx.x >= 192 && threadIdx.x < 198)
	{
		const uint32_t v = pair_bbox[threadIdx.x - 192];
		o.bbox[threadIdx.x - 192] = v;
		if (M)
			M->cnt[24 + threadIdx.x - 192] = v;
	}
	if (threadIdx.x < MULLS_NC * MULLS_NTERM)
	{
		const int c = threadIdx.x / MULLS_NTERM, t = threadIdx.x % MULLS_NTERM;
		if (rp.used[c])
		{
			constexpr uint32_t STEP = MULLS_ACC_LANES / MULLS_SRC_PER_BLOCK;
			double sum = 0.0;
			uint32_t j = pd[c].job_begin;
			const uint32_t je = pd[c].job_end;
			for (; j + 32u * STEP <= je; j += 32u * STEP)
			{
				double v[32];
#pragma unroll
				for (uint32_t k = 0; k < 32u; k++)
					v[k] = partial[(size_t)(j + k * STEP) * MULLS_NTERM + t];
#pragma unroll
				for (uint32_t k = 0; k < 32u; k++)
					sum += v[k];
			}
			for (; j + 16u * STEP <= je; j += 16u * STEP)
			{
				double v[16];
#pragma unroll
				for (uint32_t k = 0; k < 16u; k++)
					v[k] = partial[(size_t)(j + k * STEP) * MULLS_NTERM + t];
#pragma unroll
				for (uint32_t k = 0; k < 16u; k++)
					sum += v[k];
			}
			for (; j < je; j += STEP)
				sum += partial[(size_t)j * MULLS_NTERM + t];
			o.sums[c][t] = sum;
			if (M)
				M->sums[c][t] = sum;
		}
	}
	__syncthreads();
	if (rp.pull_comb && threadIdx.x >= 64 && threadIdx.x < 64 + MULLS_NTERM)
	{
		if (M)
		{
			combine_rows(rp, ps.want_residual != 0, M->sums, M->comb, (int)threadIdx.x - 64);
			o.comb[threadIdx.x - 64] = M->comb[threadIdx.x - 64];
		}
		else
			combine_rows(rp, ps.want_residual != 0, o.sums, o.comb, (int)threadIdx.x - 64);
	}
	if (threadIdx.x < MULLS_NC)
	{
		const int c = threadIdx.x;
		CloudDesc &d = pd[c];
		if (ps.active)
		{
			if (class_called(rp, d, c))
			{
				d.n_valid = d.valid_next;
				d.alive_cur = d.alive_next;
			}
			d.alive_next = 0;
			d.valid_next = 0;
			d.n_matched = 0;
		}
		o.n_valid[c] = d.n_valid;
// ... 286 lines not shown
					S.alive_prev[c] = n_alive[c];
					S.ncorr[c] = n_valid[c];
					S.corr_pts += n_valid[c];
				}
				L.go = mulls::step_counts(h, K, n_valid) ? 1 : 0;
			}
		}
		__syncthreads();
		if (L.go && l < 64)
			solve_wave(h, K, L.comb, L.iter, L.ws);
		__syncthreads();
		if (l == 0)
		{
			L.done = (!h.active && !h.want_residual) ? 1 : 0;
			L.left = L.done ? 0 : 1;
			if (L.done)
				h.guess = h.temp * h.guess;
		}
		__syncthreads();
		PairState &ps = states[pair];
		if (l < 12)
			ps.T[l] = h.temp.at(l / 4, l % 4);
		else if (l < 18)
			ps.x[l - 12] = h.x[l - 12];
		else if (l < 24)
			ps.thr[l - 18] = h.thr[l - 18];
		else if (l == 24)
		{
			ps.iter = h.want_residual ? h.iters - 1 : L.iter + 1;
			ps.active = h.active ? 1 : 0;
			ps.want_residual = h.want_residual ? 1 : 0;
		}
		if (l < 64)
		{
			unsigned long long *dst = reinterpret_cast<unsigned long long *>(&steps[pair]);
			const unsigned long long *src = reinterpret_cast<const unsigned long long *>(&S);
			for (uint32_t w = (uint32_t)l; w < sizeof(mulls::StepState) / 8; w += 64u)
				dst[w] = src[w];
		}
		if (L.done)
		{
			IcpOut &O = results[pair];
			if (l < 16)
				O.T[l] = h.guess.v[l];
			if (l < 36)
				O.info[l] = h.info.v[l];
			if (l >= 40 && l < 46)
			{
				const int c = l - 40;
				O.ncorr[c] = S.ncorr[c];
				O.nsrc0[c] = S.nsrc0[c];
				O.ntgt0[c] = S.ntgt0[c];
				O.bbox[c] = S.bbox[c];
			}
			if (l == 63)
			{
				O.sigma2 = h.sigma2;
				O.ratio = h.ratio;
				O.code = h.code;
				O.iters = h.iters;
				O.singular = h.singular;
				O.trace_len = 0;
				O.src_pts = S.src_pts;
				O.tgt_pts = S.tgt_pts;
				O.corr_pts = S.corr_pts;
				O.tgt_job_pts = S.tgt_job_pts;
				O.pair_evals = S.pair_evals;
			}
		}
	}
	return L.left != 0;
}

__global__ __launch_bounds__(64) void k_step(const CloudDesc *__restrict__ descs, PairState *__restrict__ states, RunParams rp, mulls::IcpConst K,
											 const PairOut *__restrict__ out, mulls::StepState *__restrict__ steps, IcpOut *__restrict__ results, int brute,
											 uint32_t pair_base)
{
	__shared__ StepLds L;
	(void)step_pair(pair_base + blockIdx.x, descs, states, rp, K, out, steps, results, brute, L);
}

__global__ __launch_bounds__(64) void k_sum_step(CloudDesc *__restrict__ descs, PairState *__restrict__ states, RunParams rp, mulls::IcpConst K,
												 const double *__restrict__ partial, PairOut *__restrict__ out, const uint32_t *__restrict__ bbox,
												 mulls::StepState *__restrict__ steps, IcpOut *__restrict__ results, int brute, uint32_t pair_base)
{
	__shared__ StepLds L;
	__shared__ FinishLds F;
	const uint32_t pair = pair_base + blockIdx.x;
	const bool live = states[pair].active || states[pair].want_residual;
	unsigned long long sw[STEP_WORDS_PER_LANE];
	if (live)
	{
		const unsigned long long *src = reinterpret_cast<const unsigned long long *>(&steps[pair]);
#pragma unroll
		for (uint32_t k = 0; k < STEP_WORDS_PER_LANE; k++)
			sw[k] = src[min(threadIdx.x + 64u * k, STEP_WORDS - 1u)];
		finish_pair_wave(descs + pair * MULLS_NC, states[pair], rp, partial, out[pair], bbox + pair * 6, F);
	}
	__syncthreads();
	if (threadIdx.x < MULLS_NTERM_PAD)
		L.comb[threadIdx.x] = F.comb[threadIdx.x];
	if (threadIdx.x < 30u)
		L.cnt[threadIdx.x] = F.cnt[threadIdx.x];
	(void)step_pair(pair, descs, states, rp, K, out, steps, results, brute, L, sw);
}

__global__ __launch_bounds__(MULLS_BLOCK) void k_finish_step(CloudDesc *__restrict__ descs, PairState *__restrict__ states, RunParams rp, mulls::IcpConst K,
															  const double *__restrict__ partial, PairOut *__restrict__ out, const uint32_t *__restrict__ bbox,
															  mulls::StepState *__restrict__ steps, IcpOut *__restrict__ results, int brute, uint32_t *__restrict__ ticket,
															  volatile unsigned long long *host_word, uint32_t epoch, uint32_t pair_base)
{
	__shared__ StepLds L;
	const uint32_t pair = pair_base + blockIdx.x;
	const bool live = states[pair].active || states[pair].want_residual;
	unsigned long long sw[STEP_WORDS_PER_LANE];
	if (live && threadIdx.x < 64u)
	{
		const unsigned long long *src = reinterpret_cast<const unsigned long long *>(&steps[pair]);
#pragma unroll
		for (uint32_t k = 0; k < STEP_WORDS_PER_LANE; k++)
			sw[k] = src[min(threadIdx.x + 64u * k, STEP_WORDS - 1u)];
	}
	__shared__ FinishLds F;
	if (live)
		finish_pair(descs + pair * MULLS_NC, states[pair], rp, partial, out[pair], bbox + pair * 6, &F);
	__syncthreads();
	if (threadIdx.x < MULLS_NTERM_PAD)
		L.comb[threadIdx.x] = F.comb[threadIdx.x];
	else if (threadIdx.x >= 64u && threadIdx.x < 94u)
		L.cnt[threadIdx.x - 64u] = F.cnt[threadIdx.x - 64u];
	const bool left = step_pair(pair, descs, states, rp, K, out, steps, results, brute, L, sw);
	if (threadIdx.x == 0)
	{
		unsigned long long *t64 = reinterpret_cast<unsigned long long *>(ticket);
		const unsigned long long old = atomicAdd(t64, ((unsigned long long)(left ? 1u : 0u) << 32) | 1ull);
		if ((uint32_t)old == gridDim.x - 1u)
		{
			const uint32_t n_left = (uint32_t)(old >> 32) + (left ? 1u : 0u);
			*t64 = 0ull;
			__threadfence_system();
			*host_word = (unsigned long long)epoch << 32 | n_left;
		}
	}
}

__global__ __launch_bounds__(1024) void k_step_publish(const PairState *__restrict__ states, uint32_t npairs, volatile unsigned long long *host_word, uint32_t epoch)
{
	int mine = 0;
	for (uint32_t p = threadIdx.x; p < npairs; p += 1024u)
		mine += (states[p].active || states[p].want_residual) ? 1 : 0;
	__shared__ uint32_t s_left;
	if (threadIdx.x == 0)
		s_left = 0u;
	__syncthreads();
	for (int off = 32; off > 0; off >>= 1)
		mine += __shfl_down(mine, off);
	if ((threadIdx.x & 63u) == 0u && mine)
		atomicAdd(&s_left, (uint32_t)mine);
	__syncthreads();
	if (threadIdx.x == 0)
	{
		__threadfence_system();
		*host_word = (unsigned long long)epoch << 32 | s_left;
	}
}

static_assert(sizeof(PairState) % 16 == 0, "PairState must be a whole number of uint4 words");
__global__ void k_push_states(const uint4 *__restrict__ host_words, uint4 *__restrict__ dev_words, uint32_t nwords)
{
	const uint32_t i = blockIdx.x * blockDim.x + threadIdx.x;
	if (i < nwords)
		dev_words[i] = host_words[i];
}

__global__ void k_transform_aos(float4 *__restrict__ recs, uint32_t n, const double *__restrict__ T )
{
	const uint32_t i = blockIdx.x * blockDim.x + threadIdx.x;
	if (i >= n)
		return;
	float4 a = recs[(size_t)i * 3], b = recs[(size_t)i * 3 + 1];
	double x = a.x, y = a.y, z = a.z, nx = b.x, ny = b.y, nz = b.z;
	a.x = (float)(T[0] * x + T[1] * y + T[2] * z + T[3]);
	a.y = (float)(T[4] * x + T[5] * y + T[6] * z + T[7]);
	a.z = (float)(T[8] * x + T[9] * y + T[10] * z + T[11]);
	b.x = (float)(T[0] * nx + T[1] * ny + T[2] * nz);
	b.y = (float)(T[4] * nx + T[5] * ny + T[6] * nz);
	b.z = (float)(T[8] * nx + T[9] * ny + T[10] * nz);
	recs[(size_t)i * 3] = a;
	recs[(size_t)i * 3 + 1] = b;
}

__global__ void k_set_corr(uint32_t src_off, const int32_t *__restrict__ cs, const int32_t *__restrict__ ct, const float *__restrict__ cd,
						   uint32_t n, uint8_t *__restrict__ flag, int32_t *__restrict__ match, float *__restrict__ wd, uint32_t tgt_off,
						   const float4 *__restrict__ tpos, const float4 *__restrict__ tnrm, float4 *__restrict__ mq)
{
	const uint32_t i = blockIdx.x * blockDim.x + threadIdx.x;
	if (i >= n)
		return;
	const uint32_t g = src_off + (uint32_t)cs[i];
	flag[g] = MULLS_F_ALIVE | MULLS_F_VALID;
	match[g] = ct[i];
	mq[2u * g] = tpos[tgt_off + (uint32_t)ct[i]];
	mq[2u * g + 1u] = tnrm[tgt_off + (uint32_t)ct[i]];
	wd[g] = cd ? cd[i] : 0.0f;
}

#include "launch.h"

bool accum_takes_waves(const RunParams &rp, const uint32_t split[4], uint32_t wave_min_trips)
{
	const uint32_t n_trips = split[3] - split[0];
	return wave_min_trips && n_trips >= wave_min_trips && rp.faithful && rp.pull_comb;
}

void launch_accum(hipStream_t st, const BatchDev &b, const RunParams &rp, const uint32_t split[4], bool single, uint32_t wave_min_trips)
{
	(void)dev_launch<3>([](DevLaunch &) {
		return hipFuncSetAttribute(reinterpret_cast<const void *>(k_accum<1024, 2>), hipFuncAttributeMaxDynamicSharedMemorySize, (int)MULLS_RED_BYTES_HALF) == hipSuccess;
	});
	const uint32_t n_trips = split[3] - split[0];
	if (accum_takes_waves(rp, split, wave_min_trips))
	{
		hipLaunchKernelGGL(k_accum_wave, dim3((n_trips + MULLS_ACCW_WAVES / MULLS_ACCW_SPLIT - 1u) / (MULLS_ACCW_WAVES / MULLS_ACCW_SPLIT)), dim3(64 * MULLS_ACCW_WAVES), 0, st, b.ajobs + split[0], n_trips, b.jobs, b.descs, b.states, rp, b.spos,
						   b.mq, b.flag, b.wd, b.partial);
		return;
	}
	if (single)
	{
		if (split[3] > split[0])
			hipLaunchKernelGGL((k_accum<1024, 2>), dim3(split[3] - split[0]), dim3(1024), MULLS_RED_BYTES_HALF, st, b.ajobs + split[0], b.jobs, b.descs, b.states, rp, b.spos, b.mq,
							   b.flag, b.wd, b.partial);
		return;
	}
	if (split[1] > split[0])
		hipLaunchKernelGGL((k_accum<1024, 2>), dim3(split[1] - split[0]), dim3(1024), MULLS_RED_BYTES_HALF, st, b.ajobs + split[0], b.jobs, b.descs, b.states, rp, b.spos, b.mq, b.flag,
						   b.wd, b.partial);
	if (split[2] > split[1])
		hipLaunchKernelGGL((k_accum<512, 4>), dim3(split[2] - split[1]), dim3(512), MULLS_RED_BYTES_HALF / 2, st, b.ajobs + split[1], b.jobs, b.descs, b.states, rp, b.spos, b.mq, b.flag,
						   b.wd, b.partial);
	if (split[3] > split[2])
		hipLaunchKernelGGL((k_accum<256, 8>), dim3(split[3] - split[2]), dim3(256), MULLS_RED_BYTES_HALF / 4, st, b.ajobs + split[2], b.jobs, b.descs, b.states, rp, b.spos, b.mq, b.flag,
						   b.wd, b.partial);
}

void launch_finish(hipStream_t st, const BatchDev &b, const RunParams &rp, uint32_t pair_base, uint32_t npairs, uint32_t *ticket, volatile uint32_t *host_epoch, uint32_t epoch)
{
	if (!npairs)
		return;
	const bool direct = rp.pull_comb && npairs <= 64u;
	hipLaunchKernelGGL(k_finish, dim3(npairs), dim3(MULLS_BLOCK), 0, st, b.descs, b.states, rp, b.partial, b.outs, b.bbox, pair_base,
					   direct ? reinterpret_cast<uint4 *>(b.outs_pin) : nullptr, ticket, host_epoch, epoch);
	if (direct)
		return;
	uint32_t n_used = 0;
	for (int c = 0; c < MULLS_NC; c++)
		n_used += rp.used[c] ? 1u : 0u;
	const uint32_t nwords = npairs * (8u + (MULLS_NTERM_PAD / 2u) * (rp.pull_comb ? 1u : n_used));
	hipLaunchKernelGGL(k_pull_outs, dim3((nwords + MULLS_BLOCK - 1) / MULLS_BLOCK), dim3(MULLS_BLOCK), 0, st, reinterpret_cast<const uint4 *>(b.outs),
					   reinterpret_cast<uint4 *>(b.outs_pin), rp, pair_base, npairs, ticket, host_epoch, epoch);
}

void launch_step_init(hipStream_t st, const BatchDev &b, const mulls::IcpConst &K, uint32_t npairs)
{
	if (npairs)
		hipLaunchKernelGGL(k_step_init, dim3((npairs + 63u) / 64u), dim3(64), 0, st, npairs, b.setup, K, b.steps, b.states);
}

void launch_finish_step(hipStream_t st, const BatchDev &b, const RunParams &rp, const mulls::IcpConst &K, uint32_t pair_base, uint32_t npairs, unsigned long long *host_word, uint32_t epoch,
						int brute, uint32_t *ticket, bool sum_step)
{
	if (!npairs)
		return;
	if (ticket)
	{
		hipLaunchKernelGGL(k_finish_step, dim3(npairs), dim3(MULLS_BLOCK), 0, st, b.descs, b.states, rp, K, b.partial, b.outs, b.bbox, b.steps, b.icp_outs, brute, ticket, host_word, epoch,
						   pair_base);
		return;
	}
	if (sum_step && rp.pull_comb)
		hipLaunchKernelGGL(k_sum_step, dim3(npairs), dim3(64), 0, st, b.descs, b.states, rp, K, b.partial, b.outs, b.bbox, b.steps, b.icp_outs, brute, pair_base);
	else
	{
		hipLaunchKernelGGL(k_finish, dim3(npairs), dim3(MULLS_BLOCK), 0, st, b.descs, b.states, rp, b.partial, b.outs, b.bbox, pair_base, static_cast<uint4 *>(nullptr),
						   static_cast<uint32_t *>(nullptr), static_cast<volatile uint32_t *>(nullptr), 0u);
		hipLaunchKernelGGL(k_step, dim3(npairs), dim3(64), 0, st, b.descs, b.states, rp, K, b.outs, b.steps, b.icp_outs, brute, pair_base);
	}
	hipLaunchKernelGGL(k_step_publish, dim3(1), dim3(1024), 0, st, b.states + pair_base, npairs, host_word, epoch);
}

void launch_push_states(hipStream_t st, const BatchDev &b, uint32_t pair_base, uint32_t npairs)
{
	const PairState *host_states = b.states_pin + pair_base;
	PairState *dev_states = b.states + pair_base;
	const uint32_t nwords = npairs * (uint32_t)(sizeof(PairState) / 16);
	if (nwords)
		hipLaunchKernelGGL(k_push_states, dim3((nwords + 255) / 256), dim3(256), 0, st, reinterpret_cast<const uint4 *>(host_states),
						   reinterpret_cast<uint4 *>(dev_states), nwords);
}

void launch_transform_aos(hipStream_t st, float4 *recs, uint32_t n, const double *T12)
{
	if (n)
		hipLaunchKernelGGL(k_transform_aos, dim3((n + 255) / 256), dim3(256), 0, st, recs, n, T12);
}

void launch_set_corr(hipStream_t st, const BatchDev &b, uint32_t src_off, const int32_t *cs, const int32_t *ct, const float *cd, uint32_t n, uint32_t tgt_off)
{
	if (n)
		hipLaunchKernelGGL(k_set_corr, dim3((n + 255) / 256), dim3(256), 0, st, src_off, cs, ct, cd, n, b.flag, b.match, b.wd, tgt_off, b.tpos, b.tnrm, b.mq);
}
```

mulls_amd/csrc/k_search.hip:

```cpp
#include "device_util.h"
#include "lds_tier.h"
#include "big_tier.h"

template <int NPTS>
__device__ __forceinline__ void nn_scan_group(const float *__restrict__ X, const float *__restrict__ Y, const float *__restrict__ Z, uint32_t j,
											   const float (&px)[NPTS], const float (&py)[NPTS], const float (&pz)[NPTS], float (&best)[NPTS],
											   uint32_t (&grp)[NPTS], uint32_t gidx)
{
	const float4 x0 = *reinterpret_cast<const float4 *>(X + j), x1 = *reinterpret_cast<const float4 *>(X + j + 4);
	const float4 y0 = *reinterpret_cast<const float4 *>(Y + j), y1 = *reinterpret_cast<const float4 *>(Y + j + 4);
	const float4 z0 = *reinterpret_cast<const float4 *>(Z + j), z1 = *reinterpret_cast<const float4 *>(Z + j + 4);
	const float tx[8] = {x0.x, x0.y, x0.z, x0.w, x1.x, x1.y, x1.z, x1.w};
	const float ty[8] = {y0.x, y0.y, y0.z, y0.w, y1.x, y1.y, y1.z, y1.w};
	const float tz[8] = {z0.x, z0.y, z0.z, z0.w, z1.x, z1.y, z1.z, z1.w};
#pragma unroll
	for (int u = 0; u < NPTS; u++)
	{
		float dd[8];
#pragma unroll
		for (int v = 0; v < 8; v++)
		{
			const float dx = px[u] - tx[v], dy = py[u] - ty[v], dz = pz[u] - tz[v];
			dd[v] = (dx * dx + dy * dy) + dz * dz;
		}
// ... 91 lines not shown
		{
			const uint32_t t = grp[u] + v;
			if (t < tgt_n)
			{
				float ddx = px[u] - tp[4 * t], ddy = py[u] - tp[4 * t + 1], ddz = pz[u] - tp[4 * t + 2];
				float dist = (ddx * ddx + ddy * ddy) + ddz * ddz;
				if (dist == best[u])
					idx = (int)t;
			}
		}
		const bool matched = idx >= 0 && !((double)best[u] > max_dist_sqr);
		nn_idx[d.src_off + s[u]] = matched ? idx : -1;
		nn_d2[d.src_off + s[u]] = best[u];
		if (matched)
		{
			matched_cnt++;
			if (gate)
				atomicMin(&winner[d.tgt_off + idx], key_hi | (unsigned long long)s[u]);
		}
	}
	for (int off = 32; off > 0; off >>= 1)
		matched_cnt += __shfl_down(matched_cnt, off);
	if ((threadIdx.x & 63) == 0 && matched_cnt)
		atomicAdd(&d.n_matched, matched_cnt);
}

__global__ __launch_bounds__(MULLS_BIG_BLOCK, 4) void k_cert_big(const Job *__restrict__ jobs, CloudDesc *__restrict__ descs, const PairState *__restrict__ states, RunParams rp,
																 float4 *__restrict__ spos, float4 *__restrict__ snrm, const GridDesc *__restrict__ grids,
																 const unsigned long long *__restrict__ bm, const uint32_t *__restrict__ pf, const uint32_t *__restrict__ cs,
																 const float4 *__restrict__ tsorted, uint8_t *flag, int32_t *__restrict__ nn_idx, float *__restrict__ nn_d2,
																 unsigned long long *__restrict__ winner, uint32_t split, const float4 *__restrict__ tpos,
																 const float4 *__restrict__ tnrm, int32_t *__restrict__ nn_hint, int32_t *__restrict__ match, float *__restrict__ wd,
																 float4 *__restrict__ mq)
{
	__shared__ BigLds<MULLS_BIG_BLOCK * 3> s_big;
	const uint32_t wg = xcd_job(blockIdx.x, gridDim.x);
	const Job job = jobs[wg / split];
	const uint32_t part = wg % split;
	const PairState &ps = states[job.pair];
	if (!ps.active || (rp.normal_shooting && (job.cls == 0 || job.cls == 2 || job.cls == 4)))
		return;
	const uint32_t ci = job.pair * MULLS_NC + job.cls;
	CloudDesc &d = descs[ci];
	const bool class_level = (job.count & MULLS_JOB_CLASS) != 0u;
	const uint32_t cnt = (job.count & ~MULLS_JOB_CLASS) ? (job.count & ~MULLS_JOB_CLASS) : (uint32_t)MULLS_SRC_PER_BLOCK;
	uint32_t q0, q1;
	if (class_level)
	{
		if (part)
			return;
		q0 = 0u, q1 = min(d.src_n, cnt);
	}
	else
	{
		const uint32_t per = cnt / split;
		q0 = job.start + part * per, q1 = min(d.src_n, q0 + per);
		if (q0 >= q1)
			return;
	}
	const GridDesc g = grids[ci];
	const BmGrid B = {bm + g.cell_off, pf + g.cell_off, cs + d.tgt_off + ci};
	cert_big<MULLS_BIG_BLOCK, 3>(s_big, rp, ps, job.cls, q0, q1, class_level, d, g, B, tsorted + d.tgt_off, spos, snrm, flag, nn_idx, nn_d2, winner, tnrm, match, wd, tpos,
								 reinterpret_cast<int2 *>(nn_hint), mq);
}

__global__ __launch_bounds__(MULLS_BLOCK) void k_filter(const Job *__restrict__ jobs, CloudDesc *__restrict__ descs,
														 const PairState *__restrict__ states, RunParams rp,
														 const float4 *__restrict__ snrm, const float4 *__restrict__ tnrm, uint8_t *__restrict__ flag,
														 const int32_t *__restrict__ nn_idx, const float *__restrict__ nn_d2,
														 int32_t *__restrict__ match, float *__restrict__ wd,
														 const unsigned long long *__restrict__ winner, const float4 *__restrict__ tpos,
														 float4 *__restrict__ mq, uint32_t big)
{
	__shared__ uint32_t red4[4];
	const Job job = jobs[xcd_job(blockIdx.x, gridDim.x)];
	const PairState &ps = states[job.pair];
	if (!ps.active)
		return;
	CloudDesc &d = descs[job.pair * MULLS_NC + job.cls];
	if (!class_called(rp, d, job.cls))
		return;
	const float thr = ps.thr[job.cls];
	const FilterCtx F = {d.alive_cur >= 500u, d.n_matched > 0u, job.cls != 5, rp.lds_dedup != 0u && !big, rp.rej_strict != 0, thr * thr, rp.cos_bearing,
						 (unsigned long long)(0xffffffffu - (rp.tick_base + (uint32_t)ps.iter)) << 32, big ? nullptr : rp.tgt_stage, big ? nullptr : rp.tgt_map};
	uint32_t n_alive = 0, n_valid = 0;
#pragma unroll
	for (int u = 0; u < MULLS_SRC_PER_THREAD; u++)
	{
		const uint32_t s = job.start + threadIdx.x + u * MULLS_BLOCK;
		if (s < d.src_n)
			filter_point(F, d, s, snrm, tnrm, flag, nn_idx, nn_d2, match, wd, winner, tpos, mq, n_alive, n_valid);
	}
	const uint32_t ta = block_sum_u32(n_alive, red4);
	const uint32_t tv = block_sum_u32(n_valid, red4);
	if (threadIdx.x == 0)
	{
		if (ta)
			atomicAdd(&d.alive_next, ta);
		if (tv)
			atomicAdd(&d.valid_next, tv);
	}
}


__device__ __forceinline__ bool first_goes_direct(const RunParams &rp, const CloudDesc &d, int cls)
{
	return class_called(rp, d, cls);
}

template <int BLK, int SMALL, bool PARK = false, int FLAT_TRIPS = (BLK == 512 ? 3 : 2)>
__device__ __forceinline__ bool cert_job(CertLds<SMALL> &CL, const RunParams &rp, const PairState &ps, const Job &job, CloudDesc &d, const GridDesc &g, uint32_t *W, float4 *__restrict__ spos,
										  float4 *__restrict__ snrm, const uint32_t *__restrict__ cell_start, const float4 *__restrict__ tsorted, uint8_t *flag,
										  int32_t *__restrict__ nn_idx, float *__restrict__ nn_d2, unsigned long long *__restrict__ winner, const float4 *__restrict__ tnrm,
										  int32_t *__restrict__ match, float *__restrict__ wd, const float4 *__restrict__ tpos, int32_t *__restrict__ nn_hint,
										  float4 *__restrict__ mq, uint32_t *park = nullptr)
{
	const bool flat = rp.lds_dedup != 0u && rp.debug_stop != 9u && job.start == 0u && job.count >= d.src_n && d.src_n <= (uint32_t)(BLK * FLAT_TRIPS) && class_called(rp, d, job.cls);
	return flat ? cert_class_flat<BLK, FLAT_TRIPS, true, SMALL, PARK>(CL, rp, ps, job, d, g, W, spos, snrm, cell_start, tsorted, flag, nn_idx, nn_d2, winner, tnrm, match, wd, tpos, nn_hint, mq, park)
				: cert_class<BLK, true, SMALL>(CL, rp, ps, job, d, g, W, spos, snrm, cell_start, tsorted, flag, nn_idx, nn_d2, winner, tnrm, match, wd, tpos, nn_hint, mq);
}

template <int BLK, int TRIPS = (BLK == 512 ? 3 : 2), int SMALL = MULLS_CERT_SMALL_LOCKSTEP>
__global__ __launch_bounds__(BLK, BLK == 512 ? 8 : 4) void k_cert(const Job *__restrict__ cjobs, CloudDesc *__restrict__ descs,
															const PairState *__restrict__ states, RunParams rp, float4 *__restrict__ spos,
															float4 *__restrict__ snrm, const GridDesc *__restrict__ grids,
															const uint32_t *__restrict__ cell_start, const float4 *__restrict__ tsorted, uint8_t *flag,
															int32_t *__restrict__ nn_idx, float *__restrict__ nn_d2, unsigned long long *__restrict__ winner,
															const float4 *__restrict__ tnrm, int32_t *__restrict__ match, float *__restrict__ wd,
															const float4 *__restrict__ tpos, int32_t *__restrict__ nn_hint, float4 *__restrict__ mq,
															uint32_t *__restrict__ wl, uint32_t *__restrict__ wl_ctr, uint32_t parity)
{
	extern __shared__ __attribute__((aligned(16))) unsigned char lds_raw[];
	uint32_t *W = reinterpret_cast<uint32_t *>(lds_raw);
	if (blockIdx.x == 0 && threadIdx.x == 0)
		wl_ctr[2u * (parity ^ 1u)] = wl_ctr[2u * (parity ^ 1u) + 1u] = 0u;
	const Job job = cjobs[blockIdx.x];
	const PairState &ps = states[job.pair];
	if (!ps.active || (rp.normal_shooting && (job.cls == 0 || job.cls == 2 || job.cls == 4)))
		return;
	CloudDesc &d = descs[job.pair * MULLS_NC + job.cls];
	const GridDesc g = grids[job.pair * MULLS_NC + job.cls];
	__shared__ CertLds<SMALL> s_cert;
	constexpr bool PARK = BLK == 512;
	__shared__ uint32_t s_park[PARK ? 2 * TRIPS * BLK : 1];
	if (!cert_job<BLK, SMALL, PARK, TRIPS>(s_cert, rp, ps, job, d, g, W, spos, snrm, cell_start, tsorted, flag, nn_idx, nn_d2, winner, tnrm, match, wd, tpos, nn_hint, mq, s_park))
		if (threadIdx.x == 0)
			wl[atomicAdd(&wl_ctr[2u * parity], 1u)] = blockIdx.x;
}

#define MULLS_FUSED_PARK_BYTES (2u * 3u * MULLS_LDS_BLOCK * 4u)
__device__ __forceinline__ uint32_t *fused_park(unsigned char *lds_raw, uint32_t cap) { return reinterpret_cast<uint32_t *>(lds_raw + (((size_t)cap * 2u + 15u) & ~(size_t)15)); }

__global__ __launch_bounds__(MULLS_LDS_BLOCK) void k_cert_nn(const Job *__restrict__ cjobs, CloudDesc *__restrict__ descs, const PairState *__restrict__ states,
															  RunParams rp, float4 *__restrict__ spos, float4 *__restrict__ snrm, const GridDesc *__restrict__ grids,
															  const uint32_t *__restrict__ cell_start, const float4 *__restrict__ tsorted, uint8_t *flag,
															  int32_t *__restrict__ nn_idx, float *__restrict__ nn_d2, unsigned long long *__restrict__ winner,
															  const float4 *__restrict__ tnrm, int32_t *__restrict__ match, float *__restrict__ wd,
															  const float4 *__restrict__ tpos, int32_t *__restrict__ nn_hint, float4 *__restrict__ mq, uint32_t cap, uint32_t first)
{
	extern __shared__ __attribute__((aligned(16))) unsigned char lds_raw[];
	const Job job = cjobs[blockIdx.x];
	const PairState &ps = states[job.pair];
	if (!ps.active || (rp.normal_shooting && (job.cls == 0 || job.cls == 2 || job.cls == 4)))
		return;
	CloudDesc &d = descs[job.pair * MULLS_NC + job.cls];
	const GridDesc g = grids[job.pair * MULLS_NC + job.cls];
	__shared__ CertLds<MULLS_CERT_SMALL> s_cert;
// ... 359 lines not shown
```

mulls_amd/csrc/launch.h:

```cpp
#pragma once
#include <hip/hip_runtime_api.h>
#include <stdint.h>

#include "device_types.h"

#include <hip/hip_vector_types.h>
#include <mutex>

struct DevLaunch
{
	bool ready = false, ok = false;
	size_t dyn_max[2] = {0, 0};
	uint32_t n_cu = 256;
};
template <int TAG, class Init>
inline DevLaunch dev_launch(Init init)
{
	static std::mutex mu;
	static DevLaunch table[64];
	int dev = 0;
	if (hipGetDevice(&dev) != hipSuccess || dev < 0 || dev >= 64)
		dev = 0;
	std::lock_guard<std::mutex> lock(mu);
	DevLaunch &D = table[dev];
	if (!D.ready)
	{
		int cus = 0;
		if (hipDeviceGetAttribute(&cus, hipDeviceAttributeMultiprocessorCount, dev) == hipSuccess && cus > 0)
			D.n_cu = (uint32_t)cus;
		D.ok = init(D);
		D.ready = true;
	}
	return D;
}
namespace mulls
{
struct IcpConst;
struct StepState;
}
struct BatchDev
{
	float4 *stage = nullptr;
	float4 *tmp_pos = nullptr, *tmp_nrm = nullptr;
	float4 *spos = nullptr, *snrm = nullptr, *tpos = nullptr, *tnrm = nullptr;
	uint8_t *flag = nullptr;
	int32_t *match = nullptr, *nn_idx = nullptr, *nn_hint = nullptr;
	float4 *mq = nullptr;
	float *wd = nullptr, *nn_d2 = nullptr;
	unsigned long long *winner = nullptr;
	CloudDesc *descs = nullptr;
	PairSetup *setup = nullptr;
	PairState *states = nullptr;
	PairState *states_pin = nullptr;
	PairOut *outs = nullptr;
	PairOut *outs_pin = nullptr;
	uint32_t *bbox = nullptr;
	Job *setup_jobs = nullptr;
	uint32_t *setup_tab = nullptr;
	Job *big_segs = nullptr, *big_clouds = nullptr;
	uint32_t *seg_cnt = nullptr, *big_box = nullptr;
	Job *jobs = nullptr;
	double *partial = nullptr;
	Job *tjobs = nullptr;
	Job *cjobs = nullptr;
	Job *bjobs = nullptr, *fjobs = nullptr, *ejobs = nullptr;
	uint32_t *lclouds = nullptr;
	uint32_t *bm_cs = nullptr;
	uint32_t *bm_rank = nullptr;
	uint32_t *ajobs = nullptr;
	IcpOut *icp_outs = nullptr;
	mulls::StepState *steps = nullptr;
	uint32_t *wl = nullptr;
	uint32_t *wl_ctr = nullptr;
	GridDesc *grids = nullptr;
	float4 *tsorted = nullptr;
	uint16_t *tmap = nullptr;
	uint32_t *cell_cnt = nullptr, *cell_start = nullptr;
	unsigned long long *bm = nullptr;
	uint32_t *pf = nullptr;
	uint32_t *ticket = nullptr;
};
void launch_clone_src(hipStream_t st, const BatchDev &b, const RunParams &rp, uint32_t njobs);
void launch_crop(hipStream_t st, const BatchDev &b, const RunParams &rp, uint32_t npairs, uint32_t nbig_segs, uint32_t nbig_clouds, const uint32_t *wgs = nullptr, uint32_t nwgs = 0);
void launch_src_setup(hipStream_t st, const BatchDev &b, const RunParams &rp, const uint32_t *pairs, uint32_t npairs);
void launch_copy_segs(hipStream_t st, const CopySeg *segs, uint32_t n);
void launch_motion_comp(hipStream_t st, float4 *recs, uint32_t n, const double q[4], const double t[3], float thre);
void launch_thin(hipStream_t st, const BatchDev &b, uint32_t npairs, const uint8_t *src_keep, const uint8_t *tgt_keep);
int launch_tgt_grid(hipStream_t st, const BatchDev &b, const RunParams &rp, uint32_t npairs, const uint32_t *clouds = nullptr, const uint32_t *split = nullptr);
const uint32_t *tgt_grid_bucket_trips();
void launch_grid_build_sort(hipStream_t st, const BatchDev &b, const RunParams &rp, uint32_t npairs);
void launch_bm_build(hipStream_t st, const BatchDev &b, uint32_t nl, uint32_t ntjobs);
size_t nn_lds_bytes(uint32_t cap, uint32_t maxcells, bool dedup);
int launch_nn_lds(hipStream_t st, const BatchDev &b, const RunParams &rp, const Job *jobs, uint32_t njobs, uint32_t cap, uint32_t *wl, uint32_t *wl_ctr, uint32_t parity,
				  bool first = false);
int launch_cert_mixed(hipStream_t st, const BatchDev &b, const RunParams &rp, const Job *cjobs, uint32_t n_lds, const Job *bjobs, uint32_t n_big, uint32_t max_wgs, uint32_t rounds,
					  uint32_t cap, bool first = false);
void launch_cert_big(hipStream_t st, const BatchDev &b, const RunParams &rp, const Job *jobs, uint32_t njobs, uint32_t max_wgs);
void launch_nn(hipStream_t st, const BatchDev &b, const RunParams &rp, const Job *jobs, uint32_t njobs);
void launch_nn_shoot(hipStream_t st, const BatchDev &b, const RunParams &rp, const Job *jobs, uint32_t njobs);
void launch_filter(hipStream_t st, const BatchDev &b, const RunParams &rp, const Job *jobs, uint32_t njobs, bool big = false);
void launch_accum(hipStream_t st, const BatchDev &b, const RunParams &rp, const uint32_t split[4], bool single = false, uint32_t wave_min_trips = 0);
bool accum_takes_waves(const RunParams &rp, const uint32_t split[4], uint32_t wave_min_trips);
void launch_finish(hipStream_t st, const BatchDev &b, const RunParams &rp, uint32_t pair_base, uint32_t npairs, uint32_t *ticket, volatile uint32_t *host_epoch, uint32_t epoch);
void launch_push_states(hipStream_t st, const BatchDev &b, uint32_t pair_base, uint32_t npairs);
void launch_step_init(hipStream_t st, const BatchDev &b, const mulls::IcpConst &K, uint32_t npairs);
void launch_finish_step(hipStream_t st, const BatchDev &b, const RunParams &rp, const mulls::IcpConst &K, uint32_t pair_base, uint32_t npairs, unsigned long long *host_word, uint32_t epoch,
						int brute, uint32_t *ticket = nullptr, bool sum_step = false);
void launch_transform_aos(hipStream_t st, float4 *recs, uint32_t n, const double *T12);
void launch_set_corr(hipStream_t st, const BatchDev &b, uint32_t src_off, const int32_t *cs, const int32_t *ct, const float *cd, uint32_t n, uint32_t tgt_off);
```

mulls_amd/csrc/lds_tier.h:

```cpp
#pragma once
#include "device_util.h"
struct FilterCtx
{
	bool gate, any_match, normal_check, dedup_done, strict;
	float max_sqr;
	double cos_thre;
	unsigned long long key_hi;
	const float4 *tgt_stage;
	const uint16_t *tgt_map;
};
__device__ __forceinline__ void filter_point(const FilterCtx &F, const CloudDesc &d, uint32_t s, const float4 *__restrict__ snrm,
											  const float4 *__restrict__ tnrm, uint8_t *__restrict__ flag, const int32_t *__restrict__ nn_idx,
											  const float *__restrict__ nn_d2, int32_t *__restrict__ match, float *__restrict__ wd,
											  const unsigned long long *__restrict__ winner, const float4 *__restrict__ tpos,
											  float4 *__restrict__ mq, uint32_t &n_alive, uint32_t &n_valid)
{
	const uint32_t g = d.src_off + s;
	const uint32_t f = flag[g];
	if (!(f & MULLS_F_ALIVE))
		return;
	bool alive = true, valid, fresh = false;
	int m;
	float4 n2 = make_float4(0.0f, 0.0f, 0.0f, 0.0f);
	if (F.any_match)
	{
		m = nn_idx[g];
		valid = m >= 0;
		if (F.gate && (m < 0 || (!F.dedup_done && winner[d.tgt_off + m] != (F.key_hi | (unsigned long long)s))))
		{
			alive = false;
			valid = false;
		}
		if (valid)
		{
			const float dist = nn_d2[g];
			valid = F.strict ? dist < F.max_sqr : !(dist > F.max_sqr);
			if (valid)
			{
				wd[g] = dist;
				if (match[g] == m)
					n2 = mq[2u * g + 1u];
				else
				{
					match[g] = m;
					float4 q2;
					tgt_record(F.tgt_stage, F.tgt_map, d, (uint32_t)m, tpos, tnrm, q2, n2);
					mq[2u * g] = q2;
					mq[2u * g + 1u] = n2;
				}
				fresh = true;
			}
		}
	}
	else if (F.gate)
	{
		alive = false;
		valid = false;
		m = -1;
	}
	else
	{
		valid = (f & MULLS_F_VALID) != 0;
		m = match[g];
	}
	if (valid && F.normal_check)
	{
		const float4 n1 = snrm[g];
		if (!fresh)
			n2 = mq[2u * g + 1u];
		const double dot = (double)n1.x * (double)n2.x + (double)n1.y * (double)n2.y + (double)n1.z * (double)n2.z;
		const float c = (float)fabs(dot);
		if ((double)c < F.cos_thre)
			valid = false;
	}
	flag[g] = (uint8_t)((alive ? MULLS_F_ALIVE : 0u) | (valid ? MULLS_F_VALID : 0u));
	n_alive += alive ? 1u : 0u;
	n_valid += valid ? 1u : 0u;
}
namespace
{
typedef unsigned long long nnkey;
#define NNKEY_NONE 0x7f800000ffffffffull
__device__ __forceinline__ nnkey nn_key(float dist, uint32_t idx) { return ((nnkey)__float_as_uint(dist) << 32) | idx; }
__device__ __forceinline__ float key_dist(nnkey k) { return __uint_as_float((uint32_t)(k >> 32)); }
__device__ __forceinline__ bool key_found(nnkey k) { return (uint32_t)k != 0xffffffffu; }

struct LdsGrid
{
	const float *P;
	const uint16_t *IDX, *CS;
	__device__ __forceinline__ uint32_t cs(uint32_t i) const { return CS[i]; }
	__device__ __forceinline__ void cand(uint32_t t, float &x, float &y, float &z, uint32_t &i) const
	{
		const float *p = P + 3u * t;
		x = p[0], y = p[1], z = p[2];
		i = IDX[t];
	}
};
struct GlobGrid
{
	const float4 *ts;
	const uint16_t *CS;
	__device__ __forceinline__ uint32_t cs(uint32_t i) const { return CS[i]; }
	__device__ __forceinline__ void cand(uint32_t t, float &x, float &y, float &z, uint32_t &i) const
	{
		const float4 v = ts[t];
		x = v.x, y = v.y, z = v.z;
		i = __float_as_uint(v.w);
	}
};

template <int CTRL>
__device__ __forceinline__ void dpp_min_step(nnkey &bk)
{
	const uint32_t oh = (uint32_t)__builtin_amdgcn_update_dpp(0, (int)(uint32_t)(bk >> 32), CTRL, 0xf, 0xf, false);
	const uint32_t ol = (uint32_t)__builtin_amdgcn_update_dpp(0, (int)(uint32_t)bk, CTRL, 0xf, 0xf, false);
	const nnkey o = ((nnkey)oh << 32) | ol;
	bk = o < bk ? o : bk;
}
#define MULLS_LDS_GSH (MULLS_LDS_GROUP == 16u ? 4 : (MULLS_LDS_GROUP == 8u ? 3 : 2))
template <int GSH>
__device__ __forceinline__ uint32_t sub_lanes(uint32_t gsh) { return GSH >= 0 ? (1u << (GSH >= 0 ? GSH : 0)) : (1u << gsh); }
// ... 337 lines not shown
	const float lb_new = fminf(sqrtf(sec), Rfin);
	hint2[d.src_off + s] = make_int2((int32_t)(((uint32_t)bi & 0xffffu) | (min(trips, 31u) << 16)), __float_as_int(lb_new));
#if MULLS_LDS_KCERT
	if (C.cand)
		C.cand[d.src_off + s] = make_uint4(co.cx, co.cy, __float_as_uint(fminf(sqrtf(co.b2), Rfin) - lb_new), C.epoch);
#else
	(void)co;
#endif
	if (matched)
	{
		if (C.dedup)
			dedup_min<W16>(W, (uint32_t)bi, s);
		else if (C.gate)
			atomicMin(&winner[d.tgt_off + bi], C.key_hi | (unsigned long long)s);
	}
	return matched;
}

#define MULLS_FS_ALIVE 1u
#define MULLS_FS_VALID 2u
#define MULLS_FS_DIR_OK 4u
#define MULLS_FS_STANDING 8u
#define MULLS_FS_SEARCH 16u
template <bool W16, int D0>
__device__ __forceinline__ bool commit_search_park(const ClassCtx &C, const CloudDesc &d, uint32_t s, nnkey bk, float sec, float Rfin, uint32_t trips, const CandOut &co,
													int2 *__restrict__ hint2, uint32_t *W, uint32_t *park)
{
	const float best = key_dist(bk);
	const int bi = (int)(uint32_t)bk;
	const bool matched = bi >= 0 && !((double)best > C.max_dist_sqr);
	const float lb_new = fminf(sqrtf(sec), Rfin);
	hint2[d.src_off + s] = make_int2((int32_t)(((uint32_t)bi & 0xffffu) | (min(trips, 31u) << 16)), __float_as_int(lb_new));
#if MULLS_LDS_KCERT
	if (C.cand)
		C.cand[d.src_off + s] = make_uint4(co.cx, co.cy, __float_as_uint(fminf(sqrtf(co.b2), Rfin) - lb_new), C.epoch);
#else
	(void)co;
#endif
	const uint32_t w0 = park[s], st = (w0 >> 24) & ~MULLS_FS_SEARCH;
	const int32_t pm = (int32_t)(w0 & 0xffffffu) - 2, m = matched ? bi : -1;
	park[s] = ((st | ((matched && bi == pm) ? MULLS_FS_STANDING : 0u)) << 24) | (uint32_t)(m + 2);
	park[(uint32_t)D0 + s] = __float_as_uint(best);
	if (matched && C.dedup)
		dedup_min<W16>(W, (uint32_t)bi, s);
	return matched;
}

template <int BLK, bool W16 = false>
__device__ __forceinline__ void class_tail(const RunParams &rp, const PairState &ps, const ClassCtx &C, CloudDesc &d, const Job &job, uint32_t q_end,
											uint32_t matched_cnt, uint32_t searched, const uint32_t *W, uint32_t *red, const float4 *__restrict__ snrm,
											const float4 *__restrict__ tnrm, uint8_t *flag, int32_t *__restrict__ nn_idx, float *__restrict__ nn_d2,
											int32_t *__restrict__ match, float *__restrict__ wd, const unsigned long long *__restrict__ winner,
											const float4 *__restrict__ tpos, float4 *__restrict__ mq)
{
	if (C.dedup)
	{
		__threadfence_block();
		__syncthreads();
		for (uint32_t s = job.start + threadIdx.x; s < q_end; s += BLK)
			if (flag[d.src_off + s] & MULLS_F_ALIVE)
			{
				const int m = nn_idx[d.src_off + s];
				if (m >= 0 && !dedup_holds<W16>(W, (uint32_t)m, s))
					nn_idx[d.src_off + s] = -1;
			}
	}
	for (int off = 32; off > 0; off >>= 1)
		matched_cnt += __shfl_down(matched_cnt, off);
	if (!rp.lds_dedup)
	{
		if ((threadIdx.x & 63) == 0 && matched_cnt)
			atomicAdd(&d.n_matched, matched_cnt);
		return;
	}
	__threadfence_block();
	__syncthreads();
	if ((threadIdx.x & 63) == 0)
		red[threadIdx.x >> 6] = matched_cnt;
	__syncthreads();
	uint32_t total_matched = 0;
	for (int w = 0; w < BLK / 64; w++)
		total_matched += red[w];
	const float thr = ps.thr[job.cls];
	const FilterCtx F = {C.gate, total_matched > 0u, job.cls != 5, true, rp.rej_strict != 0, thr * thr, rp.cos_bearing, C.key_hi, rp.tgt_stage, rp.tgt_map};
	uint32_t n_alive = 0, n_valid = 0;
	for (uint32_t s = job.start + threadIdx.x; s < q_end; s += BLK)
		filter_point(F, d, s, snrm, tnrm, flag, nn_idx, nn_d2, match, wd, winner, tpos, mq, n_alive, n_valid);
	for (int off = 32; off > 0; off >>= 1)
	{
		n_alive += __shfl_down(n_alive, off);
		n_valid += __shfl_down(n_valid, off);
	}
	if ((threadIdx.x & 63) == 0)
	{
		red[BLK / 64 + (threadIdx.x >> 6)] = n_alive;
		red[2 * (BLK / 64) + (threadIdx.x >> 6)] = n_valid;
	}
	__syncthreads();
	if (threadIdx.x == 0)
	{
		uint32_t ta = 0, tv = 0;
		for (int w = 0; w < BLK / 64; w++)
		{
			ta += red[BLK / 64 + w];
			tv += red[2 * (BLK / 64) + w];
		}
		d.n_matched = total_matched;
		d.alive_next = ta;
		d.valid_next = tv;
		d.n_search = searched;
	}
}
template <int BLK, int TRIPS, bool W16, bool COMPACT = false>
__device__ __forceinline__ void class_tail_flat(const RunParams &rp, const PairState &ps, const ClassCtx &C, CloudDesc &d, const Job &job, uint32_t q_end,
												 uint32_t matched_cnt, uint32_t searched, const uint32_t *W, uint32_t *red, float4 *snrm,
												 const float4 *__restrict__ tnrm, uint8_t *flag, const int32_t *__restrict__ nn_idx, const float *__restrict__ nn_d2,
												 int32_t *__restrict__ match, float *__restrict__ wd, const float4 *__restrict__ tpos, float4 *__restrict__ mq,
												 float4 *spos = nullptr, int2 *hint2 = nullptr)
{
	__threadfence_block();
	__syncthreads();
	uint32_t FL[TRIPS];
	int32_t M[TRIPS], PM[TRIPS];
	float D[TRIPS];
	float3 N1[TRIPS], T2[TRIPS];
	float4 P4[COMPACT ? TRIPS : 1], Q2[COMPACT ? TRIPS : 1], N2[COMPACT ? TRIPS : 1];
	int2 H[COMPACT ? TRIPS : 1];
	uint32_t NF[COMPACT ? TRIPS : 1];
#if MULLS_LDS_KCERT
	uint4 CR[COMPACT ? TRIPS : 1];
#endif
	const uint32_t last = d.src_off + (q_end ? q_end - 1u : 0u);
#pragma unroll
	for (int k = 0; k < TRIPS; k++)
	{
		const uint32_t gi = min(d.src_off + threadIdx.x + (uint32_t)k * BLK, last);
		FL[k] = flag[gi];
		M[k] = nn_idx[gi];
		D[k] = nn_d2[gi];
		N1[k] = *reinterpret_cast<const float3 *>(snrm + gi);
		if (COMPACT)
		{
			PM[k] = -1, T2[k] = make_float3(0.0f, 0.0f, 0.0f);
			P4[COMPACT ? k : 0] = spos[gi];
			H[COMPACT ? k : 0] = hint2[gi];
#if MULLS_LDS_KCERT
			CR[COMPACT ? k : 0] = C.cand ? C.cand[gi] : make_uint4(0u, 0u, 0u, 0u);
#endif
		}
		else
		{
			PM[k] = match[gi];
			T2[k] = *reinterpret_cast<const float3 *>(mq + 2u * gi + 1u);
		}
	}
	if (COMPACT)
	{
#pragma unroll
		for (int k = 0; k < TRIPS; k++)
		{
			asm volatile("" ::"v"(FL[k]), "v"(M[k]), "v"(D[k]), "v"(N1[k].x), "v"(P4[COMPACT ? k : 0].x), "v"(H[COMPACT ? k : 0].x));
#if MULLS_LDS_KCERT
			asm volatile("" ::"v"(CR[COMPACT ? k : 0].x));
#endif
		}
	}
	for (int off = 32; off > 0; off >>= 1)
		matched_cnt += __shfl_down(matched_cnt, off);
	if ((threadIdx.x & 63) == 0)
		red[threadIdx.x >> 6] = matched_cnt;
	__syncthreads();
	uint32_t total_matched = 0;
	for (int w = 0; w < BLK / 64; w++)
		total_matched += red[w];
	const float thr = ps.thr[job.cls], max_sqr = thr * thr;
	const bool any_match = total_matched > 0u, normal_check = job.cls != 5, strict = rp.rej_strict != 0;
	uint32_t n_alive = 0, n_valid = 0;
#pragma unroll
	for (int k = 0; k < TRIPS; k++)
	{
		const uint32_t s = threadIdx.x + (uint32_t)k * BLK, gi = d.src_off + s;
		if (COMPACT)
			NF[COMPACT ? k : 0] = 0u;
		if (s >= q_end || !(FL[k] & MULLS_F_ALIVE))
			continue;
		int32_t m = M[k];
		if (C.dedup && m >= 0 && !dedup_holds<W16>(W, (uint32_t)m, s))
			m = -1;
		bool alive = true, valid, newrec = false;
		float3 n2 = T2[k];
		if (any_match)
		{
			valid = m >= 0;
			if (C.gate && m < 0)
			{
				alive = false;
				valid = false;
			}
			if (valid)
			{
				const float dist = D[k];
				valid = strict ? dist < max_sqr : !(dist > max_sqr);
				if (valid)
				{
					if (!COMPACT)
						wd[gi] = dist;
					if (PM[k] != m)
					{
						float4 q2, n4;
						tgt_record(rp.tgt_stage, rp.tgt_map, d, (uint32_t)m, tpos, tnrm, q2, n4);
						if (COMPACT)
							Q2[COMPACT ? k : 0] = q2, N2[COMPACT ? k : 0] = n4, newrec = true;
						else
						{
							match[gi] = m;
							mq[2u * gi] = q2;
							mq[2u * gi + 1u] = n4;
						}
						n2 = make_float3(n4.x, n4.y, n4.z);
					}
				}
			}
		}
		else if (C.gate)
		{
			alive = false;
			valid = false;
		}
		else
			valid = (FL[k] & MULLS_F_VALID) != 0;
		if (valid && normal_check)
		{
			const double dot = (double)N1[k].x * (double)n2.x + (double)N1[k].y * (double)n2.y + (double)N1[k].z * (double)n2.z;
			const float c = (float)fabs(dot);
			if ((double)c < rp.cos_bearing)
				valid = false;
		}
		const uint32_t nf = (alive ? MULLS_F_ALIVE : 0u) | (valid ? MULLS_F_VALID : 0u);
		if (COMPACT)
		{
			NF[COMPACT ? k : 0] = nf | (newrec ? 8u : 0u);
			M[k] = newrec ? m : PM[k];
		}
		else if (nf != FL[k])
			flag[gi] = (uint8_t)nf;
		n_alive += alive ? 1u : 0u;
		n_valid += valid ? 1u : 0u;
	}
	uint32_t *words = red + 3 * (BLK / 64);
	unsigned long long bal[COMPACT ? TRIPS : 1];
	if (COMPACT)
	{
#pragma unroll
		for (int k = 0; k < TRIPS; k++)
		{
			bal[COMPACT ? k : 0] = __ballot((NF[COMPACT ? k : 0] & MULLS_F_ALIVE) != 0u);
			if ((threadIdx.x & 63) == 0)
				words[k * (BLK / 64) + (threadIdx.x >> 6)] = (uint32_t)__popcll(bal[COMPACT ? k : 0]);
		}
	}
	for (int off = 32; off > 0; off >>= 1)
	{
		n_alive += __shfl_down(n_alive, off);
		n_valid += __shfl_down(n_valid, off);
	}
	if ((threadIdx.x & 63) == 0)
	{
		red[BLK / 64 + (threadIdx.x >> 6)] = n_alive;
		red[2 * (BLK / 64) + (threadIdx.x >> 6)] = n_valid;
	}
	__syncthreads();
	if (COMPACT)
	{
		const uint32_t lane = threadIdx.x & 63u, wave = threadIdx.x >> 6, src_off = d.src_off;
		const unsigned long long below_me = (1ull << lane) - 1ull;
		LiveWord *lw = rp.live_mask + live_word_base(d, job.pair * MULLS_NC + job.cls);
		const uint32_t n_words = (q_end + 63u) >> 6;
		uint32_t run = 0;
#pragma unroll
		for (int k = 0; k < TRIPS; k++)
		{
			uint32_t below = run;
			for (int w = 0; w < BLK / 64; w++)
			{
				const uint32_t c = words[k * (BLK / 64) + w];
				below += (uint32_t)w < wave ? c : 0u;
				run += c;
			}
			const uint32_t word = (uint32_t)k * (BLK / 64) + wave;
			if (lane == 0u && word < n_words)
			{
				LiveWord v;
				v.alive = bal[COMPACT ? k : 0], v.below = below, v.pad_ = 0u;
				lw[word] = v;
			}
			const uint32_t nf = NF[COMPACT ? k : 0];
			if (nf & MULLS_F_ALIVE)
			{
				const uint32_t ci = src_off + below + (uint32_t)__popcll(bal[COMPACT ? k : 0] & below_me);
				spos[ci] = P4[COMPACT ? k : 0];
				*reinterpret_cast<float3 *>(snrm + ci) = N1[k];
				hint2[ci] = H[COMPACT ? k : 0];
#if MULLS_LDS_KCERT
				if (C.cand)
					C.cand[ci] = CR[COMPACT ? k : 0];
#endif
				flag[ci] = (uint8_t)(nf & (MULLS_F_ALIVE | MULLS_F_VALID));
				match[ci] = M[k];
				if (nf & MULLS_F_VALID)
					wd[ci] = D[k];
				if (nf & 8u)
				{
					mq[2u * ci] = Q2[COMPACT ? k : 0];
					mq[2u * ci + 1u] = N2[COMPACT ? k : 0];
				}
			}
		}
#pragma unroll
		for (int k = 0; k < TRIPS; k++)
		{
			const uint32_t s = threadIdx.x + (uint32_t)k * BLK;
			if (s >= run && s < q_end)
				flag[src_off + s] = 0u;
		}
		if (threadIdx.x == 0)
		{
			d.src_c = run;
			d.compacted = 1u;
			if (rp.dbg_ticks)
				atomicAdd(&rp.dbg_ticks[5], (unsigned long long)(q_end - run));
		}
	}
	if (threadIdx.x == 0)
	{
		uint32_t ta = 0, tv = 0;
		for (int w = 0; w < BLK / 64; w++)
		{
			ta += red[BLK / 64 + w];
			tv += red[2 * (BLK / 64) + w];
		}
		d.n_matched = total_matched;
		d.alive_next = ta;
		d.valid_next = tv;
		d.n_search = searched;
	}
}

template <int SMALL>
struct CertLds
{
	float4 uq[SMALL];
	uint32_t us[SMALL];
	static constexpr bool LOOK = MULLS_LDS_KCERT != 0 && SMALL >= 128 && SMALL <= MULLS_CERT_BLOCK;
	float um[LOOK ? SMALL : 1];
	uint32_t ucount, red[3 * 16];
};

#define MULLS_NEEDS_SEARCH (-2)

template <bool W16, class TPre, class TPos>
__device__ __forceinline__ bool kcert_point(const RunParams &rp, const uint4 cr, const int2 h, uint32_t iter, float px, float py, float pz, float moved, uint32_t tgt_n,
											 const TPre &pre, const TPos &pos, nnkey &bk, float &lb_next, uint4 &cr_next)
{
	constexpr int NO = W16 ? 4 : 2;
	const uint32_t hj = W16 ? ((uint32_t)h.x & 0xffffu) : (uint32_t)h.x;
	if (!(rp.kcert != 0u && cr.w - rp.tick_base <= iter))
		return false;
	const float hy = __int_as_float(h.y), crz = __uint_as_float(cr.z);
	const float Bp = (hy + crz) - 4.0f * 1.1920929e-7f * fmaxf(fabsf(hy), fabsf(crz));
	if (!(moved * 1.00001f < Bp * 0.99999f))
		return false;
	uint32_t ci[NO + 1], tok[NO + 1];
	bool ok[NO + 1];
	ci[0] = hj, ok[0] = true;
#pragma unroll
	for (int j = 0; j < NO; j++)
	{
		const uint32_t w = j < NO / 2 ? cr.x : cr.y, c = W16 ? (w >> ((j & 1) << 4)) & 0xffffu : w;
		ok[j + 1] = c < tgt_n;
		ci[j + 1] = ok[j + 1] ? c : hj;
	}
#pragma unroll
	for (int j = 0; j <= NO; j++)
		tok[j] = pre(ci[j]);
	float4 cp[NO + 1];
#pragma unroll
	for (int j = 0; j <= NO; j++)
		cp[j] = pos(tok[j]);
	bk = NNKEY_NONE;
	float sec = __builtin_inff();
	int slot = -1;
#pragma unroll
// ... 419 lines not shown
				if (CertLds<SMALL>::LOOK)
					CL.um[u] = moved;
			}
		}
		setSM(k, st_k, m_k);
	};

	static_assert(TRIPS == 2 || TRIPS == 3, "two trips' loads in flight");
	Rec r0 = load(0), r1 = load(1);
	if (C.dedup)
		dedup_init<W16>(W, tgt_n, BLK);
	if (threadIdx.x == 0)
		ucount = 0u;
	__syncthreads();
	FLAT_TICK(0)
	{
		const bool third = TRIPS == 3 && q_end > 2u * (uint32_t)BLK;
		cert(0, r0);
		if (third)
		{
			r0 = load(2);
			cert(1, r1);
			cert(2, r0);
		}
		else
		{
			cert(1, r1);
			if (TRIPS == 3)
				setSM(2, 0u, -1), setD0(2, 0.0f);
		}
	}
	__syncthreads();
	FLAT_TICK(2)
	uint32_t U = ucount;
	const uint32_t U0 = U;
	if (kc && U >= rp.kcert_min && U <= (uint32_t)SMALL)
		U = kcert_list<BLK, W16, SMALL>(CL, rp, ps, C, d, U, nn_idx, nn_d2, hint2, W, winner, tpos, matched_cnt);
	FLAT_TICK(1)
	if (rp.dbg_ticks && threadIdx.x == 0)
	{
		atomicAdd(&rp.dbg_ticks[13], (unsigned long long)U0);
		atomicAdd(&rp.dbg_ticks[7], (unsigned long long)U);
	}
	if (U > (uint32_t)SMALL)
	{
#pragma unroll
		for (int k = 0; k < TRIPS; k++)
			if ((getST(k) & MULLS_FS_ALIVE) && (PARK || !waits(k)))
			{
				const uint32_t gi = d.src_off + threadIdx.x + (uint32_t)k * BLK;
				nn_idx[gi] = waits(k) ? MULLS_NEEDS_SEARCH : getM(k);
				nn_d2[gi] = getD0(k);
			}
		return false;
	}
	if (U)
	{
		const GlobGrid L = {tsorted + d.tgt_off, reinterpret_cast<const uint16_t *>(cell_start) + g.cell_off};
		const uint32_t sub = threadIdx.x & (MULLS_LDS_GROUP - 1u), grp = threadIdx.x / MULLS_LDS_GROUP;
		for (uint32_t i = grp; i < U; i += BLK / MULLS_LDS_GROUP)
		{
			nnkey bk;
			float sec, Rfin;
			uint32_t trips;
			CandOut co = {0xffffffffu, 0xffffffffu, 0.0f};
			search_query<MULLS_GLOB_CHUNK>(g, L, uq[i], C.r, C.m, sub, bk, sec, Rfin, trips, co);
			if (sub == 0 && (PARK ? commit_search_park<W16, BLK * TRIPS>(C, d, us[i] & ~MULLS_US_KCERT, bk, sec, Rfin, trips, co, hint2, W, park)
								  : commit_search<W16>(C, d, us[i] & ~MULLS_US_KCERT, bk, sec, Rfin, trips, co, nn_idx, nn_d2, hint2, W, winner)))
				matched_cnt++;
		}
	}
	for (int off = 32; off > 0; off >>= 1)
		matched_cnt += __shfl_down(matched_cnt, off);
	if ((threadIdx.x & 63) == 0)
		red[threadIdx.x >> 6] = matched_cnt;
	__threadfence_block();
	__syncthreads();
	uint32_t total_matched = 0;
	for (int w = 0; w < BLK / 64; w++)
		total_matched += red[w];
	FLAT_TICK(3)

	const float thr = ps.thr[job.cls], max_sqr = thr * thr;
	const bool any_match = total_matched > 0u, strict = rp.rej_strict != 0;
	uint32_t n_alive = 0, n_valid = 0;
#pragma unroll
	for (int k = 0; k < TRIPS; k++)
	{
		const uint32_t st = getST(k);
		if (!(st & MULLS_FS_ALIVE))
			continue;
		const uint32_t s = threadIdx.x + (uint32_t)k * BLK, gi = d.src_off + s;
		int32_t m = getM(k);
		float dist = getD0(k);
		bool standing = (st & MULLS_FS_STANDING) != 0;
		if (PARK ? (st & MULLS_FS_SEARCH) != 0u : m == MULLS_NEEDS_SEARCH)
		{
			m = nn_idx[gi];
			dist = nn_d2[gi];
			standing = m >= 0 && match[gi] == m;
		}
		if (C.dedup && m >= 0 && !dedup_holds<W16>(W, (uint32_t)m, s))
			m = -1;
		bool alive = true, valid, dir_ok = (st & MULLS_FS_DIR_OK) != 0;
		if (any_match)
		{
			valid = m >= 0;
			if (C.gate && m < 0)
			{
				alive = false;
				valid = false;
			}
			if (valid)
			{
				if (!standing)
				{
					match[gi] = m;
					float4 q2, n2;
					tgt_record(rp.tgt_stage, rp.tgt_map, d, (uint32_t)m, tpos, tnrm, q2, n2);
					mq[2u * gi] = q2;
					mq[2u * gi + 1u] = n2;
					if (normal_check)
					{
						const float3 n1 = *reinterpret_cast<const float3 *>(snrm + gi);
						const double dot = (double)n1.x * (double)n2.x + (double)n1.y * (double)n2.y + (double)n1.z * (double)n2.z;
						const float c = (float)fabs(dot);
						dir_ok = !((double)c < rp.cos_bearing);
					}
				}
				valid = strict ? dist < max_sqr : !(dist > max_sqr);
				if (valid)
					wd[gi] = dist;
			}
		}
		else if (C.gate)
		{
			alive = false;
			valid = false;
		}
		else
			valid = (st & MULLS_FS_VALID) != 0;
		if (valid && normal_check && !dir_ok)
			valid = false;
		const uint32_t nf = (alive ? MULLS_F_ALIVE : 0u) | (valid ? MULLS_F_VALID : 0u);
		if (nf != (st & (MULLS_FS_ALIVE | MULLS_FS_VALID)))
			flag[gi] = (uint8_t)nf;
		n_alive += alive ? 1u : 0u;
		n_valid += valid ? 1u : 0u;
	}
	for (int off = 32; off > 0; off >>= 1)
	{
		n_alive += __shfl_down(n_alive, off);
		n_valid += __shfl_down(n_valid, off);
	}
	if ((threadIdx.x & 63) == 0)
	{
		red[BLK / 64 + (threadIdx.x >> 6)] = n_alive;
		red[2 * (BLK / 64) + (threadIdx.x >> 6)] = n_valid;
	}
	__syncthreads();
	if (threadIdx.x == 0)
	{
		uint32_t ta = 0, tv = 0;
		for (int w = 0; w < BLK / 64; w++)
		{
			ta += red[BLK / 64 + w];
			tv += red[2 * (BLK / 64) + w];
		}
		d.n_matched = total_matched;
		d.alive_next = ta;
		d.valid_next = tv;
		d.n_search = U;
	}
	FLAT_TICK(4)
	if (rp.dbg_ticks && threadIdx.x == 0)
		atomicAdd(&rp.dbg_ticks[6], 1ull);
#undef FLAT_TICK
	return true;
}

struct LdsLayout
{
	float4 *qpos;
	uint32_t *HIST;
	uint16_t *ORDER;
	float *P;
	uint16_t *IDX;
	uint16_t *CS;
	uint32_t *W;
};
__device__ __forceinline__ LdsLayout lds_layout(unsigned char *lds_raw, uint32_t cap, uint32_t grid_maxcells)
{
	LdsLayout L;
	L.qpos = reinterpret_cast<float4 *>(lds_raw);
	L.HIST = reinterpret_cast<uint32_t *>(L.qpos + MULLS_LDS_QCHUNK);
	L.ORDER = reinterpret_cast<uint16_t *>(L.HIST + 80);
	L.P = reinterpret_cast<float *>(reinterpret_cast<unsigned char *>(L.HIST) + MULLS_LDS_AUX);
	L.IDX = reinterpret_cast<uint16_t *>(L.P + 3u * cap);
	L.CS = L.IDX + cap;
	L.W = reinterpret_cast<uint32_t *>(L.CS + ((grid_maxcells + 8u) & ~1u));
	return L;
}

__device__ __forceinline__ void lds_search_class(const RunParams &rp, const PairState &ps, const Job &job, CloudDesc &d, const GridDesc &g,
												  const LdsLayout &Y, unsigned char *lds_raw, float4 *spos,
												  float4 *snrm, const uint32_t *__restrict__ cell_start,
												  const float4 *__restrict__ tsorted, uint8_t *flag, int32_t *__restrict__ nn_idx, float *__restrict__ nn_d2,
												  unsigned long long *__restrict__ winner, const float4 *__restrict__ tnrm, int32_t *__restrict__ match,
												  float *__restrict__ wd, const float4 *__restrict__ tpos, int32_t *__restrict__ nn_hint, float4 *__restrict__ mq,
												  bool first = false)
{
	unsigned long long t_prev = rp.dbg_ticks ? wall_clock64() : 0ull;
#define HEAVY_TICK(k)                                                 \
	if (rp.dbg_ticks)                                                 \
// ... 181 lines not shown
```

mulls_amd/csrc/loop.cpp:

```cpp
#include "batch.h"

using namespace mulls_drv;

namespace
{
struct Run
{
	mulls_ctx *ctx;
	mulls_batch *B;
	const mulls_params *P;
	mulls_result *results;
	int n;
	hipStream_t st;
	std::chrono::steady_clock::time_point wall0;
	EvTimer evt;
	RunParams rp;
	mulls::IcpConst K;
	uint32_t lds_cap = 0;
	uint32_t max_big_tgt = 0;
	int tier = 0;
	bool use_grid = false, dstep = false;
};
struct DrainOnError
{
// ... 211 lines not shown
		return MULLS_E_NOMEM;
	HIPCHK(ctx, hipMemcpyAsync(B->icp_outs_pin, B->icp_outs, sizeof(IcpOut) * (size_t)n, hipMemcpyDeviceToHost, R.st));
	HIPCHK(ctx, hipStreamSynchronize(R.st));
	R.evt.collect();
	const double wall_ms = std::chrono::duration<double>(std::chrono::steady_clock::now() - R.wall0).count() * 1e3;
	int max_it = 0;
	for (int p = 0; p < n; p++)
	{
		const IcpOut &o = B->icp_outs_pin[p];
		mulls_result &R = results[p];
		R.code = o.code;
		R.iters = o.iters;
		std::memcpy(R.T, o.T, sizeof(R.T));
		std::memcpy(R.info, o.info, sizeof(R.info));
		R.sigma = (float)std::sqrt(o.sigma2);
		R.confidence = o.ratio;
		R.singular = o.singular;
		R.ms_total = (float)(wall_ms / n);
		for (int c = 0; c < MULLS_NC; c++)
		{
			R.ncorr[c] = o.ncorr[c];
			R.nsrc0[c] = o.nsrc0[c];
			R.ntgt0[c] = o.ntgt0[c];
		}
		R.cropped = 0;
		std::memset(R.crop_box, 0, sizeof(R.crop_box));
		fill_crop_box(rp, B->setup_h[p].tgt_bound, o.bbox, R);
		R.trace_len = 0;
		ctx->prof.nn_src_pts += o.src_pts;
		ctx->prof.nn_tgt_unique += o.tgt_pts;
		ctx->prof.nn_tgt_pts += o.tgt_job_pts;
		ctx->prof.nn_corr_pts += o.corr_pts;
		ctx->prof.nn_pair_evals += o.pair_evals;
		max_it = std::max(max_it, o.iters);
	}
	ctx->prof.iterations = max_it;
	if (rp.dbg_ticks)
	{
		unsigned long long t[16];
		HIPCHK(ctx, hipMemcpy(t, rp.dbg_ticks, sizeof(t), hipMemcpyDeviceToHost));
		if (rp.debug_stop == 21u)
		{
			ctx->prof.icp_fused_ms[0] += (double)t[13], ctx->prof.icp_fused_ms[1] += (double)t[7] * 1e-5;
			return MULLS_OK;
		}
		for (int k = 0; k < 5; k++)
			ctx->prof.icp_fused_ms[k] += (double)t[k] * 1e-5;
		ctx->prof.icp_fused_ms[5] += (double)t[6];
		ctx->prof.icp_search_ms[0] += (double)t[13], ctx->prof.icp_search_ms[1] += (double)t[14], ctx->prof.icp_search_ms[2] += (double)t[15], ctx->prof.icp_search_ms[3] += (double)t[7];
		ctx->prof.icp_search_ms[4] += (double)t[5];
		for (int k = 0; k < 4; k++)
			ctx->prof.icp_phase_ms[k] += (double)t[8 + k] * 1e-5;
		ctx->prof.icp_phase_ms[4] += (double)t[12];
	}
	return MULLS_OK;
}

int run_device_step(Run &R)
{
	mulls_ctx *ctx = R.ctx;
	mulls_batch *B = R.B;
	const mulls_params *P = R.P;
	const RunParams &rp = R.rp;
	EvTimer &evt = R.evt;
	const int n = R.n;
	hipStream_t st = R.st;
	int rc;
	if (grow(ctx, &B->steps, &B->cap_steps, (size_t)n) != MULLS_OK || grow(ctx, &B->icp_outs, &B->cap_icp_outs, (size_t)n) != MULLS_OK)
		return MULLS_E_HIP;
	HIPCHK(ctx, hipMemsetAsync(B->icp_outs, 0, sizeof(IcpOut) * (size_t)n, st));
	launch_step_init(st, *B, R.K, (uint32_t)n);
	const bool few_launches = n <= (int)ctx->opt[MULLS_OPT_FEW_LAUNCHES_MAX_PAIRS];
	bool sum_step = ctx->opt[MULLS_OPT_SUM_STEP] != 0.0;
	for (size_t k = 0; sum_step && k < B->descs_h.size(); k++)
		sum_step = B->descs_h[k].job_end - B->descs_h[k].job_begin <= 4u * (1024u / MULLS_SRC_PER_BLOCK);
	struct Sub
	{
		int lo = 0, hi = 0;
		Slice L;
		hipStream_t st = nullptr;
		volatile unsigned long long *word = nullptr;
		unsigned long long *word_dev = nullptr;
		uint32_t *epoch_ctr = nullptr, *ticket = nullptr, *wl = nullptr, *wl_ctr = nullptr;
		uint32_t epoch0 = 0, nn_launches = 0, left = 0;
		int s = 0;
		bool done = false;
		EvTimer ev2[2] = {EvTimer{nullptr}, EvTimer{nullptr}};
	};
	const int nsub = B->nsub;
	Sub subs[2];
	for (int k = 0; k < nsub; k++)
	{
		Sub &S = subs[k];
		S.lo = (int)((long)n * k / nsub);
		S.hi = (int)((long)n * (k + 1) / nsub);
		S.L = slice_of(B, S.lo, S.hi, k);
		S.st = k == 0 ? ctx->stream : ctx->stream2;
		S.word = reinterpret_cast<volatile unsigned long long *>(B->epoch_h + 32 + 16 * k);
		S.word_dev = reinterpret_cast<unsigned long long *>(B->epoch_dev + 32 + 16 * k);
		S.epoch_ctr = k == 0 ? &B->epoch2 : &B->epoch3;
		S.epoch0 = *S.epoch_ctr;
		S.ticket = B->ticket + 2 + 4 * k;
		S.wl = B->wl + S.L.cjob_lo;
		S.wl_ctr = B->wl_ctr + 8 * k;
		S.left = (uint32_t)(S.hi - S.lo);
		for (int e = 0; e < 2; e++)
		{
			S.ev2[e].ctx = ctx;
			S.ev2[e].base = 10 * e;
		}
	}
	subs[0].ev2[0].used = evt.used;
	for (int k = 0; k < 5; k++)
		subs[0].ev2[0].slot[k] = evt.slot[k];
	evt.used = 0;
	if (nsub == 2)
	{
		HIPCHK(ctx, hipEventRecord(ctx->ev_setup, ctx->stream));
		HIPCHK(ctx, hipStreamWaitEvent(ctx->stream2, ctx->ev_setup, 0));
	}
	DrainOnError drain{ctx};
	auto wait_set = [&](Sub &S, int set) -> int {
		const uint32_t want = S.epoch0 + (uint32_t)set + 1u;
		const auto t0 = std::chrono::steady_clock::now();
		bool synced = false;
		for (uint64_t spins = 0;; spins++)
		{
			const unsigned long long w = *S.word;
			if ((int32_t)((uint32_t)(w >> 32) - want) >= 0)
			{
				std::atomic_thread_fence(std::memory_order_acquire);
				S.left = (uint32_t)w;
				return MULLS_OK;
			}
			if (synced)
				break;
			if ((spins & 0xfff) == 0xfff && std::chrono::duration<double>(std::chrono::steady_clock::now() - t0).count() > 2.0)
			{
				HIPCHK(ctx, hipStreamSynchronize(S.st));
				synced = true;
			}
		}
		ctx->err = "device did not publish the iteration epoch";
		return MULLS_E_HIP;
	};
	auto advance = [&](Sub &S) -> int {
		const int s = S.s;
		if (s > P->max_iter_num)
		{
			S.done = true;
			return MULLS_OK;
		}
		if (s >= 2)
		{
			const auto t_wait0 = std::chrono::steady_clock::now();
			int rcw;
			if ((rcw = wait_set(S, s - 2)) != MULLS_OK)
				return rcw;
			ctx->prof.ms_host_wait += std::chrono::duration<double>(std::chrono::steady_clock::now() - t_wait0).count() * 1e3;
			S.ev2[s & 1].collect();
			if (S.left == 0)
			{
				S.done = true;
				return MULLS_OK;
			}
		}
		hipStream_t sst = S.st;
		EvTimer &ev = S.ev2[s & 1];
		ev.stream = sst;
		const bool search = s < P->max_iter_num;
		if (search)
		{
			int rcs;
			if ((rcs = launch_search(R, sst, S.L, S.wl, S.wl_ctr, S.nn_launches++, ev, s)) != MULLS_OK)
			{
				(void)hipMemsetAsync(S.ticket, 0, 2 * sizeof(uint32_t), sst);
				return rcs;
			}
			if (&S == &subs[0])
				ctx->prof.launches_nn++;
		}
		ev.begin(search ? &ctx->prof.ms_accum : &ctx->prof.ms_residual);
		launch_accum(sst, *B, rp, S.L.ajob_split, few_launches, (uint32_t)ctx->opt[MULLS_OPT_ACCUM_WAVE_MIN_TRIPS]);
		launch_finish_step(sst, *B, rp, R.K, (uint32_t)S.lo, (uint32_t)(S.hi - S.lo), S.word_dev, ++*S.epoch_ctr, R.use_grid ? 0 : 1,
						   (few_launches || n <= (int)ctx->opt[MULLS_OPT_STEP_LAUNCH_MAX_PAIRS]) ? S.ticket : nullptr, sum_step);
		ev.end();
		{
			const hipError_t e = hipGetLastError();
			if (e != hipSuccess)
			{
				ctx->err = std::string("iteration launch set: ") + hipGetErrorString(e);
				(void)hipMemsetAsync(S.ticket, 0, 2 * sizeof(uint32_t), sst);
				return MULLS_E_HIP;
			}
		}
		S.s++;
		return MULLS_OK;
	};
	const auto t_loop0 = std::chrono::steady_clock::now();
	for (;;)
	{
		bool any = false;
		for (int k = 0; k < nsub; k++)
			if (!subs[k].done)
			{
				if ((rc = advance(subs[k])) != MULLS_OK)
					return rc;
				any = true;
			}
		if (!any)
			break;
	}
	ctx->prof.ms_host_launch += std::chrono::duration<double>(std::chrono::steady_clock::now() - t_loop0).count() * 1e3 - ctx->prof.ms_host_wait;
	if (nsub == 2)
	{
		HIPCHK(ctx, hipEventRecord(ctx->ev_setup, ctx->stream2));
		HIPCHK(ctx, hipStreamWaitEvent(ctx->stream, ctx->ev_setup, 0));
	}
	rc = results_from_device(R);
	if (rc != MULLS_OK)
		return rc;
	drain.armed = false;
	for (int k = 0; k < nsub; k++)
	{
		subs[k].ev2[0].collect();
		subs[k].ev2[1].collect();
	}
	return MULLS_OK;
}

int run_host_step(Run &R)
{
	mulls_ctx *ctx = R.ctx;
	mulls_batch *B = R.B;
	const mulls_params *P = R.P;
	mulls_result *results = R.results;
	const RunParams &rp = R.rp;
	const mulls::IcpConst &K = R.K;
	EvTimer &evt = R.evt;
	const int n = R.n;
	const bool use_grid = R.use_grid;
	hipStream_t st = R.st;
	const auto wall0 = R.wall0;
	int rc;

	std::vector<PairHost> H(n);
	for (int p = 0; p < n; p++)
	{
		PairHost &h = H[p];
		mulls::pair_iter_init(h, B->setup_h[p].guess, K);
		results[p].trace_len = 0;
		std::memset(results[p].ncorr, 0, sizeof(results[p].ncorr));
		std::memset(results[p].nsrc0, 0, sizeof(results[p].nsrc0));
		std::memset(results[p].ntgt0, 0, sizeof(results[p].ntgt0));
		results[p].cropped = 0;
		std::memset(results[p].crop_box, 0, sizeof(results[p].crop_box));
	}

	if (P->max_iter_num <= 0)
	{
		std::vector<CloudDesc> back(B->descs_h.size());
		std::vector<uint32_t> keys((size_t)n * 6);
		HIPCHK(ctx, hipMemcpyAsync(back.data(), B->descs, sizeof(CloudDesc) * back.size(), hipMemcpyDeviceToHost, st));
		HIPCHK(ctx, hipMemcpyAsync(keys.data(), B->bbox, sizeof(uint32_t) * keys.size(), hipMemcpyDeviceToHost, st));
		HIPCHK(ctx, hipStreamSynchronize(st));
		evt.collect();
		for (int p = 0; p < n; p++)
		{
// ... 268 lines not shown
```

mulls_amd/csrc/stage.cpp:

```cpp
#include "batch.h"

using namespace mulls_drv;

extern "C"
{
	int mulls_stage_transform(mulls_ctx *ctx, void *pts, uint32_t n, uint32_t stride, const double T[16])
	try
	{
		if (!ctx || (n && !pts) || stride != MULLS_POINT_BYTES || !T)
			return MULLS_E_INVALID;
		HIPCHK(ctx, hipSetDevice(ctx->device));
		float4 *d = nullptr;
		double *dT = nullptr;
		double t12[12];
		rows12(T, t12);
		if (dmalloc(ctx, &d, (size_t)n * 3) != MULLS_OK || dmalloc(ctx, &dT, 12) != MULLS_OK)
			return MULLS_E_HIP;
		hipError_t e = hipMemcpyAsync(d, pts, (size_t)n * MULLS_POINT_BYTES, hipMemcpyHostToDevice, ctx->stream);
		if (e == hipSuccess)
			e = hipMemcpyAsync(dT, t12, sizeof(t12), hipMemcpyHostToDevice, ctx->stream);
		if (e == hipSuccess)
		{
			launch_transform_aos(ctx->stream, d, n, dT);
			e = hipMemcpyAsync(pts, d, (size_t)n * MULLS_POINT_BYTES, hipMemcpyDeviceToHost, ctx->stream);
// ... 153 lines not shown
							   float angle_thre_degree, int32_t *match, float *d2, uint8_t *flags)
	try
	{
		if (!ctx || !src || !tgt || !match || !d2 || !flags)
			return MULLS_E_INVALID;
		HIPCHK(ctx, hipSetDevice(ctx->device));
		if (src->n == 0)
			return MULLS_OK;
		const int cls = normal_check ? MULLS_GROUND : MULLS_VERTEX;
		mulls_batch *B = nullptr;
		RunParams rp;
		int rc = stage_batch(ctx, cls, src, tgt, &B, &rp, normal_check ? "100000" : "000001");
		if (rc == MULLS_OK)
		{
			rp.cos_bearing = std::cos(angle_thre_degree / 180.0 * M_PI);
			identity_state(&B->states_h[0], 0);
			for (int c = 0; c < MULLS_NC; c++)
				B->states_h[0].thr[c] = dis_thre;
			hipStream_t st = ctx->stream;
			hipError_t e = hipSuccess;
			launch_push_states(st, *B, 0, 1);
			uint32_t lds_cap = 0;
			const int tier = choose_tier(ctx, B, rp.used, &lds_cap);
			rc = tier < 0 ? MULLS_E_INVALID : queue_tier_search(ctx, B, rp, tier, lds_cap, 0u);
			const uint32_t off = B->descs_h[cls].src_off;
			if (e == hipSuccess)
				e = hipMemcpyAsync(match, B->nn_idx + off, sizeof(int32_t) * src->n, hipMemcpyDeviceToHost, st);
			if (e == hipSuccess)
				e = hipMemcpyAsync(d2, B->nn_d2 + off, sizeof(float) * src->n, hipMemcpyDeviceToHost, st);
			if (e == hipSuccess)
				e = hipMemcpyAsync(flags, B->flag + off, src->n, hipMemcpyDeviceToHost, st);
			if (e == hipSuccess)
				e = hipStreamSynchronize(st);
			if (e != hipSuccess)
			{
				ctx->err = hipGetErrorString(e);
				rc = MULLS_E_HIP;
			}
			if (rc == MULLS_OK && (src->n < 3 || tgt->n < 3))
				for (uint32_t i = 0; i < src->n; i++)
				{
					match[i] = -1;
					d2[i] = 0.0f;
				}
		}
		mulls_batch_destroy(ctx, B);
		return rc;
	}
	catch (...)
	{
		return mulls::abi_caught(const_cast<mulls_ctx *>(ctx));
	}

	int mulls_stage_accumulate(mulls_ctx *ctx, int metric, const mulls_cloud *src, const mulls_cloud *tgt, const int32_t *corr_src,
							   const int32_t *corr_tgt, const float *corr_d2, uint32_t ncorr, int iter_num, float class_weight, int dist_w,
							   int resid_w, int inten_w, float window, double *out27, float *weight_out)
	try
	{
		if (!ctx || !src || !tgt || !out27 || metric < 0 || metric > 2 || (ncorr && (!corr_src || !corr_tgt)))
			return MULLS_E_INVALID;
		HIPCHK(ctx, hipSetDevice(ctx->device));
		for (int k = 0; k < 27; k++)
			out27[k] = 0.0;
		if (src->n == 0 || ncorr == 0)
			return MULLS_OK;
		for (uint32_t i = 0; i < ncorr; i++)
			if (corr_src[i] < 0 || (uint32_t)corr_src[i] >= src->n || corr_tgt[i] < 0 || (uint32_t)corr_tgt[i] >= tgt->n)
				return MULLS_E_INVALID;
		const int cls = metric == 0 ? MULLS_FACADE : (metric == 1 ? MULLS_PILLAR : MULLS_VERTEX);
		const char *used = metric == 0 ? "001000" : (metric == 1 ? "010000" : "000001");
		mulls_batch *B = nullptr;
		RunParams rp;
		int rc = stage_batch(ctx, cls, src, tgt, &B, &rp, used);
		int32_t *dcs = nullptr, *dct = nullptr;
		float *dcd = nullptr;
		if (rc == MULLS_OK)
		{
			rp.w_dist = dist_w != 0;
			rp.w_resid = resid_w != 0;
			rp.w_inten = inten_w != 0;
			rp.win_pl = rp.win_li = rp.win_pt = window;
			rp.force_class_w = 1;
			rp.class_w_value = class_weight;
			hipStream_t st = ctx->stream;
			hipError_t e = hipSuccess;
			if (dmalloc(ctx, &dcs, ncorr) != MULLS_OK || dmalloc(ctx, &dct, ncorr) != MULLS_OK || dmalloc(ctx, &dcd, ncorr) != MULLS_OK)
				e = hipErrorOutOfMemory;
			if (e == hipSuccess)
				e = hipMemcpyAsync(dcs, corr_src, sizeof(int32_t) * ncorr, hipMemcpyHostToDevice, st);
			if (e == hipSuccess)
				e = hipMemcpyAsync(dct, corr_tgt, sizeof(int32_t) * ncorr, hipMemcpyHostToDevice, st);
			if (e == hipSuccess && corr_d2)
				e = hipMemcpyAsync(dcd, corr_d2, sizeof(float) * ncorr, hipMemcpyHostToDevice, st);
			identity_state(&B->states_h[0], iter_num);
			launch_push_states(ctx->stream, *B, 0, 1);
			const uint32_t off = B->descs_h[cls].src_off;
			if (e == hipSuccess)
			{
				e = hipMemsetAsync(B->flag + off, MULLS_F_ALIVE, src->n, st);
				launch_set_corr(st, *B, off, dcs, dct, corr_d2 ? dcd : nullptr, ncorr, B->descs_h[cls].tgt_off);
				for (int k = 0; k < B->nsub; k++)
					launch_accum(st, *B, rp, B->ajob_split[k]);
				launch_finish(st, *B, rp, 0, 1, B->ticket, B->epoch_dev, ++B->epoch);
			}
			std::vector<float> wall(src->n);
			if (e == hipSuccess)
				e = hipMemcpyAsync(wall.data(), B->wd + off, sizeof(float) * src->n, hipMemcpyDeviceToHost, st);
			if (e == hipSuccess)
				e = hipStreamSynchronize(st);
			if (e != hipSuccess)
			{
				ctx->err = hipGetErrorString(e);
				rc = MULLS_E_HIP;
			}
			else
			{
				PairOut o;
				unpack_out(B, rp.used, 0, o);
				std::memcpy(out27, o.sums[cls], sizeof(double) * 27);
				if (weight_out)
					for (uint32_t i = 0; i < ncorr; i++)
						weight_out[i] = wall[corr_src[i]];
			}
		}
		if (dcs)
			(void)hipFree(dcs);
		if (dct)
			(void)hipFree(dct);
		if (dcd)
			(void)hipFree(dcd);
		mulls_batch_destroy(ctx, B);
		return rc;
	}
	catch (...)
	{
		return mulls::abi_caught(const_cast<mulls_ctx *>(ctx));
	}
}
```

Baseline: 309,500.

## Precompute accum trip records, recompute residual weights, add step-tick completion path

The accumulation kernel now reads a precomputed per-trip record built on the host (pair, class, start, offsets, live-word base). That record replaces the separate leader, job and live-mask lookups, and its fields are pinned to scalar registers. The correspondence weight is no longer stored in the search pass and reloaded in the residual pass; it is recomputed during the residual pass. The wd array is now stored only for the faithful vertex class or when store_w is set. A step-tick buffer is also added so the sum-step kernel can signal completion when many pairs run per launch. Together these aim to cut global memory traffic and per-wave setup latency, at the cost of extra ALU work in the residual pass and more complex bookkeeping.

```diff
diff --git a/mulls_amd/csrc/accum.h b/mulls_amd/csrc/accum.h
--- a/mulls_amd/csrc/accum.h
+++ b/mulls_amd/csrc/accum.h
@@ -32,8 +32,23 @@
 	int metric, iter_num;
 	bool residual_pass, dist_w, resid_w, inten_w, faithful;
 	bool li_diag;
+	bool d2_word;
+	bool store_w;
 	float class_w, window;
 };
+struct ClassCnt
+{
+	uint32_t alive_cur, tgt_n, valid_next, n_valid;
+};
+__device__ __forceinline__ int class_count(const RunParams &rp, int c, bool residual_pass, const ClassCnt &n)
+{
+	return (int)((!residual_pass && class_called(rp, c, n.alive_cur, n.tgt_n)) ? n.valid_next : n.n_valid);
+}
+__device__ __forceinline__ void class_counts(const RunParams &rp, const CloudDesc *pd, bool residual_pass, int cnt[MULLS_NC])
+{
+	for (int c = 0; c < MULLS_NC; c++)
+		cnt[c] = class_count(rp, c, residual_pass, ClassCnt{pd[c].alive_cur, pd[c].tgt_n, pd[c].valid_next, pd[c].n_valid});
+}
 __device__ __forceinline__ float class_weight(const RunParams &rp, int cls, bool residual_pass, const int cnt[MULLS_NC])
 {
 	if (rp.force_class_w)
@@ -57,6 +72,8 @@
 	A.inten_w = rp.w_inten;
 	A.faithful = rp.faithful;
 	A.li_diag = A.metric == 1 && rp.faithful && rp.pull_comb && !residual_pass;
+	A.d2_word = residual_reads_d2(rp, (uint32_t)cls);
+	A.store_w = rp.store_w != 0;
 	A.class_w = class_w;
 	A.window = A.metric == 0 ? rp.win_pl : (A.metric == 1 ? rp.win_li : rp.win_pt);
 	return A;
@@ -131,7 +148,7 @@
 
 	if (residual_pass)
 	{
-				const float cw = wdg;
+		const float cw = wdg;
 		if (metric == 0)
 		{
 			float ntx = N.x, nty = N.y, ntz = N.z;
@@ -479,18 +496,22 @@
 	const uint32_t s = trip0 + threadIdx.x;
 	bool valid = false;
 	float4 P = make_float4(0.0f, 0.0f, 0.0f, 0.0f), Q = P, N = P;
-	float w = 0.0f, w0 = 0.0f;
+	float w = 0.0f;
 	uint32_t g = 0;
+	const bool reads_d2 = A.residual_pass && A.d2_word;
 	if (s < d.src_n)
 	{
 		g = d.src_off + s;
 		const uint32_t f = flag[g];
 		P = spos[g], Q = mq[2u * g], N = mq[2u * g + 1u];
-		w = w0 = wd[g];
+		if (reads_d2)
+			w = wd[g];
 		valid = (f & (MULLS_F_ALIVE | MULLS_F_VALID)) == (MULLS_F_ALIVE | MULLS_F_VALID);
 	}
+	if (A.residual_pass && !reads_d2 && valid)
+		w = corr_weight(A, A.metric, P, Q, N, A.inten_w ? point_wi(P, Q) : 1.0f);
 	trip_sum_regs<HALF, LANES>(A, x, valid, P, Q, N, w, R, part);
-	if (valid && __float_as_uint(w) != __float_as_uint(w0))
+	if (A.store_w && valid && !A.residual_pass && !A.d2_word)
 		wd[g] = w;
 }
 
diff --git a/mulls_amd/csrc/batch.cpp b/mulls_amd/csrc/batch.cpp
--- a/mulls_amd/csrc/batch.cpp
+++ b/mulls_amd/csrc/batch.cpp
@@ -347,6 +347,14 @@
 				}
 			}
 			B->ajob_split[k][3] = (uint32_t)B->ajobs_h.size();
+		}
+		B->atrips_h.clear();
+		for (const uint32_t j : B->ajobs_h)
+		{
+			const Job &jb = B->jobs_h[j];
+			const CloudDesc &d = B->descs_h[jb.pair * MULLS_NC + jb.cls];
+			const uint32_t slots = std::min(1024u, d.src_cap - jb.start);
+			B->atrips_h.push_back({jb.pair, jb.cls, jb.start, j, d.src_off, (d.src_off >> 6) + jb.pair * MULLS_NC + jb.cls + (jb.start >> 6), std::max(1u, (slots + 63u) >> 6), 0u});
 		}
 	}
 	{
@@ -879,6 +887,8 @@
 	A(grow(ctx, &B->wl, &B->cap_wl, B->cjobs_h.size()));
 	A(grow(ctx, &B->ajobs, &B->cap_ajobs, B->ajobs_h.size(), &g2));
 	grew |= g2;
+	A(grow(ctx, &B->atrips, &B->cap_atrips, B->atrips_h.size(), &g2));
+	grew |= g2;
 	A(grow(ctx, &B->setup_tab, &B->cap_setup_tab, B->setup_tab_h.size(), &g2));
 	grew |= g2;
 	if (!B->wl_ctr)
@@ -917,6 +927,7 @@
 		up.add_host(B->ejobs, B->ejobs_h.data(), sizeof(Job) * B->ejobs_h.size());
 		up.add_host(B->lclouds, B->lclouds_h.data(), sizeof(uint32_t) * B->lclouds_h.size());
 		up.add_host(B->ajobs, B->ajobs_h.data(), sizeof(uint32_t) * B->ajobs_h.size());
+		up.add_host(B->atrips, B->atrips_h.data(), sizeof(TripRec) * B->atrips_h.size());
 		up.add_host(B->setup_tab, B->setup_tab_h.data(), sizeof(uint32_t) * B->setup_tab_h.size());
 		up.add_host(B->descs_init, B->descs_h.data(), sizeof(CloudDesc) * B->descs_h.size());
 		up.add_host(B->bbox_init, B->bbox_h, sizeof(uint32_t) * 6 * n);
diff --git a/mulls_amd/csrc/batch.h b/mulls_amd/csrc/batch.h
--- a/mulls_amd/csrc/batch.h
+++ b/mulls_amd/csrc/batch.h
@@ -72,6 +72,8 @@
 	std::vector<Job> tjobs_h;
 	std::vector<uint32_t> ajobs_h;
 	uint32_t ajob_split[2][4] = {{0, 0, 0, 0}, {0, 0, 0, 0}};
+	std::vector<TripRec> atrips_h;
+	size_t cap_atrips = 0;
 	IcpOut *icp_outs_pin = nullptr;
 	size_t cap_icp_pin = 0;
 	std::string jobs_key;
@@ -88,6 +90,8 @@
 	size_t cap_ajobs = 0;
 	size_t cap_icp_outs = 0;
 	size_t cap_steps = 0;
+	unsigned long long *step_tick = nullptr;
+	size_t cap_step_tick = 0;
 	uint32_t epoch2 = 0, epoch3 = 0;
 	int nsub = 1;
 	double fill_ms = 0.0, fill_pack_ms = 0.0;
diff --git a/mulls_amd/csrc/big_tier.h b/mulls_amd/csrc/big_tier.h
--- a/mulls_amd/csrc/big_tier.h
+++ b/mulls_amd/csrc/big_tier.h
@@ -543,7 +543,7 @@
 		total_matched += CL.red[w];
 
 	const float thr = ps.thr[cls], max_sqr = thr * thr;
-	const bool any_match = total_matched > 0u, strict = rp.rej_strict != 0;
+	const bool any_match = total_matched > 0u, strict = rp.rej_strict != 0, store_d2 = tail_stores_d2(rp, (uint32_t)cls);
 	uint32_t n_alive = 0, n_valid = 0;
 #pragma unroll
 	for (int k = 0; k < TRIPS; k++)
@@ -578,7 +578,8 @@
 				valid = strict ? dist < max_sqr : !(dist > max_sqr);
 				if (valid)
 				{
-					wd[gi] = dist;
+					if (store_d2)
+						wd[gi] = dist;
 					if (!standing)
 					{
 						match[gi] = m;
diff --git a/mulls_amd/csrc/device_types.h b/mulls_amd/csrc/device_types.h
--- a/mulls_amd/csrc/device_types.h
+++ b/mulls_amd/csrc/device_types.h
@@ -146,6 +146,20 @@
 	uint32_t count;
 };
 
+struct TripRec
+{
+	uint32_t pair, cls;
+	uint32_t start;
+	uint32_t job;
+	uint32_t src_off;
+	uint32_t live0;
+	uint32_t words;
+	uint32_t pad_;
+};
+
+#define MULLS_STEP_TICK_STRIDE 16u
+inline uint32_t step_tick_words(uint32_t npairs) { return (1u + (npairs + 63u) / 64u) * MULLS_STEP_TICK_STRIDE; }
+
 #define MULLS_COPY_SEGS 24
 struct CopySeg
 {
@@ -166,6 +180,7 @@
 	uint8_t normal_shooting;
 	uint8_t faithful;
 	uint8_t rej_strict;
+	uint8_t store_w;
 	float z_xy_ratio;
 	float win_pt, win_pl, win_li;
 	uint8_t force_class_w;
diff --git a/mulls_amd/csrc/device_util.h b/mulls_amd/csrc/device_util.h
--- a/mulls_amd/csrc/device_util.h
+++ b/mulls_amd/csrc/device_util.h
@@ -81,10 +81,11 @@
 
 __device__ __forceinline__ uint32_t live_word_base(const CloudDesc &d, uint32_t cloud) { return (d.src_off >> 6) + cloud; }
 
-__device__ __forceinline__ bool class_called(const RunParams &rp, const CloudDesc &d, int cls)
-{
-	return rp.used[cls] && d.alive_cur >= 3u && d.tgt_n >= 3u;
-}
+__device__ __forceinline__ bool residual_reads_d2(const RunParams &rp, uint32_t cls) { return cls == 5u && rp.faithful; }
+__device__ __forceinline__ bool tail_stores_d2(const RunParams &rp, uint32_t cls) { return residual_reads_d2(rp, cls); }
+
+__device__ __forceinline__ bool class_called(const RunParams &rp, int cls, uint32_t alive_cur, uint32_t tgt_n) { return rp.used[cls] && alive_cur >= 3u && tgt_n >= 3u; }
+__device__ __forceinline__ bool class_called(const RunParams &rp, const CloudDesc &d, int cls) { return class_called(rp, cls, d.alive_cur, d.tgt_n); }
 
 __device__ __forceinline__ uint32_t block_sum_u32(uint32_t v, uint32_t *lds4)
 {
diff --git a/mulls_amd/csrc/driver.cpp b/mulls_amd/csrc/driver.cpp
--- a/mulls_amd/csrc/driver.cpp
+++ b/mulls_amd/csrc/driver.cpp
@@ -337,7 +337,7 @@
 		void *dev[] = {B->stage, B->tmp_pos, B->tmp_nrm, B->spos, B->snrm, B->tpos, B->tnrm, B->flag, B->match, B->nn_idx, B->nn_hint, B->nn_cand, B->live_mask, B->mq, B->wd,
 					   B->nn_d2, B->winner, B->descs, B->setup, B->states, B->outs, B->ticket, B->bbox, B->setup_jobs, B->big_segs, B->big_clouds, B->seg_cnt, B->big_box, B->jobs, B->partial,
 					   B->tjobs, B->cjobs, B->bjobs, B->fjobs, B->ejobs, B->lclouds, B->bm_cs, B->wl, B->wl_ctr, B->grids, B->tsorted, B->tmap, B->dbg, B->cell_cnt, B->cell_start, B->bm, B->pf, B->descs_init, B->bbox_init,
-					   B->ajobs, B->icp_outs, B->steps, B->bm_rank, B->setup_tab};
+					   B->ajobs, B->atrips, B->icp_outs, B->steps, B->step_tick, B->bm_rank, B->setup_tab};
 		for (void *p : dev)
 			if (p)
 				staggered_free(p);
diff --git a/mulls_amd/csrc/k_reduce.hip b/mulls_amd/csrc/k_reduce.hip
--- a/mulls_amd/csrc/k_reduce.hip
+++ b/mulls_amd/csrc/k_reduce.hip
@@ -18,9 +18,8 @@
 	const CloudDesc *pd = descs + job.pair * MULLS_NC;
 	const bool residual_pass = ps.want_residual != 0;
 	int cnt[MULLS_NC];
-	for (int c = 0; c < MULLS_NC; c++)
-		cnt[c] = (int)(class_called(rp, pd[c], c) ? pd[c].valid_next : pd[c].n_valid);
-	const AccumCtx A = accum_ctx(rp, job.cls, ps.iter, residual_pass, class_weight(rp, job.cls, residual_pass, cnt));
+	class_counts(rp, pd, residual_pass, cnt);
+	const AccumCtx A = accum_ctx(rp, job.cls, ps.iter, residual_pass, class_weight(rp, job.cls, false, cnt));
 	trip_sum<true, LANES>(A, ps.x, pd[job.cls], job.start, spos, mq, flag, wd, lds_raw, part);
 	if (threadIdx.x < MULLS_NTERM)
 		partial[(size_t)job_idx * MULLS_NTERM + threadIdx.x] = part[threadIdx.x];
@@ -55,10 +54,13 @@
 	if constexpr (REM > WIN)
 		add_windows<TS, W0 + WIN, REM - WIN, MODE, METRIC, A0>(A, x, P, Q, N, wi, w, acc, wpre);
 }
+struct TripCloud
+{
+	uint32_t src_n, src_off, src_c, compacted;
+};
 template <typename TS, int NT, int MODE, int METRIC, int T0, int NTW>
-__device__ __forceinline__ void wave_trip(const AccumCtx &A, const double *x, const CloudDesc &d, uint32_t trip0, const float4 *__restrict__ spos, const float4 *__restrict__ mq,
-										   const uint8_t *__restrict__ flag, float *__restrict__ wd, double *__restrict__ out, bool owner, const LiveWord *__restrict__ live,
-										   uint32_t cloud)
+__device__ __forceinline__ void wave_trip(const AccumCtx &A, const double *x, const TripCloud &d, uint32_t trip0, const float4 *__restrict__ spos, const float4 *__restrict__ mq,
+										   const uint8_t *__restrict__ flag, float *__restrict__ wd, double *__restrict__ out, bool owner, const LiveWord &lw)
 {
 	const uint32_t lane = threadIdx.x & 63u;
 	const uint32_t src_n = d.src_n, src_off = d.src_off;
@@ -67,12 +69,7 @@
 	const uint32_t last = src_off + (compacted ? max(d.src_c, 1u) : src_n) - 1u;
 	const unsigned long long below_me = (1ull << lane) - 1ull;
 	static_assert(MULLS_ACC_LANES / 64 <= 64, "one LiveWord per lane covers a trip");
-	uint32_t lw_lo = 0u, lw_hi = 0u, lw_below = 0u;
-	if (compacted)
-	{
-		const LiveWord w = live[live_word_base(d, cloud) + (trip0 >> 6) + min(lane, iters - 1u)];
-		lw_lo = (uint32_t)w.alive, lw_hi = (uint32_t)(w.alive >> 32), lw_below = w.below;
-	}
+	const uint32_t lw_lo = (uint32_t)lw.alive, lw_hi = (uint32_t)(lw.alive >> 32), lw_below = lw.below;
 	struct Rec
 	{
 		uint32_t f, g;
@@ -81,7 +78,7 @@
 		float3 N;
 		float w;
 	};
-	const bool need_w = A.residual_pass, writes_w = !A.residual_pass && (METRIC != 2 || !A.faithful);
+	const bool need_w = A.residual_pass && METRIC == 2 && A.d2_word, writes_w = A.store_w && !A.residual_pass && !(METRIC == 2 && A.d2_word);
 	auto load = [&](uint32_t i) {
 		Rec r;
 		uint32_t g = src_off + trip0 + lane + 64u * i;
@@ -124,8 +121,10 @@
 		{
 			float w = cur.w;
 			const float4 N4 = make_float4(cur.N.x, cur.N.y, cur.N.z, 0.0f);
-			const float wi = (A.inten_w && !A.residual_pass) ? point_wi(cur.P, cur.Q) : 1.0f;
-			const float wpre = A.residual_pass ? 0.0f : corr_weight(A, METRIC, cur.P, cur.Q, N4, wi);
+			const float wi = (A.inten_w && !need_w) ? point_wi(cur.P, cur.Q) : 1.0f;
+			const float wpre = need_w ? 0.0f : corr_weight(A, METRIC, cur.P, cur.Q, N4, wi);
+			if (A.residual_pass && !need_w)
+				w = wpre;
 			add_windows<TS, T0, NTW, MODE, METRIC, T0>(A, x, cur.P, cur.Q, N4, wi, w, acc, A.residual_pass ? nullptr : &wpre);
 			if (owner && writes_w)
 				wd[cur.g] = w;
@@ -171,30 +170,43 @@
 #define MULLS_ACCW_OCC 4
 #endif
 #define MULLS_ACCW_WAVES 4
-__global__ __launch_bounds__(64 * MULLS_ACCW_WAVES, MULLS_ACCW_OCC) void k_accum_wave(const uint32_t *__restrict__ leaders, uint32_t n_trips, const Job *__restrict__ jobs,
-																					   const CloudDesc *__restrict__ descs, const PairState *__restrict__ states, RunParams rp,
-																					   const float4 *__restrict__ spos, const float4 *__restrict__ mq, const uint8_t *__restrict__ flag,
-																					   float *__restrict__ wd, double *__restrict__ partial)
-{
-	const uint32_t wave = threadIdx.x >> 6, part = wave % MULLS_ACCW_SPLIT;
-	const uint32_t trip = blockIdx.x * (MULLS_ACCW_WAVES / MULLS_ACCW_SPLIT) + wave / MULLS_ACCW_SPLIT;
+__global__ __launch_bounds__(64 * MULLS_ACCW_WAVES, MULLS_ACCW_OCC) void k_accum_wave(const TripRec *__restrict__ trips, uint32_t n_trips, const CloudDesc *__restrict__ descs,
+																					   const PairState *__restrict__ states, RunParams rp, const float4 *__restrict__ spos,
+																					   const float4 *__restrict__ mq, const uint8_t *__restrict__ flag, float *__restrict__ wd,
+																					   double *__restrict__ partial)
+{
+	const uint32_t wave = threadIdx.x >> 6, part = wave % MULLS_ACCW_SPLIT, lane = threadIdx.x & 63u;
+	const uint32_t trip = (uint32_t)__builtin_amdgcn_readfirstlane((int)(blockIdx.x * (MULLS_ACCW_WAVES / MULLS_ACCW_SPLIT) + wave / MULLS_ACCW_SPLIT));
 	if (trip >= n_trips)
 		return;
-	const uint32_t job_idx = leaders[trip];
-	const Job job = jobs[job_idx];
-	const PairState &ps = states[job.pair];
-	if (!ps.active && !ps.want_residual)
-		return;
-	const CloudDesc *pd = descs + job.pair * MULLS_NC;
-	const bool residual_pass = ps.want_residual != 0;
+	TripRec tr = trips[trip];
+	asm volatile("" : "+s"(tr.pair), "+s"(tr.cls), "+s"(tr.start), "+s"(tr.job), "+s"(tr.src_off), "+s"(tr.live0), "+s"(tr.words));
+	static_assert(sizeof(TripRec) == 32 && sizeof(LiveWord) <= sizeof(TripRec) && alignof(LiveWord) <= 8, "a trip record can stand in for a LiveWord");
+	const LiveWord *lwp = rp.live_mask ? rp.live_mask + (tr.live0 + min(lane, tr.words - 1u)) : reinterpret_cast<const LiveWord *>(trips + trip);
+	LiveWord lw = *lwp;
+	const PairState &ps = states[tr.pair];
+	const CloudDesc *pd = descs + tr.pair * MULLS_NC, *pc = pd + tr.cls;
+	TripCloud d = {pc->src_n, tr.src_off, pc->src_c, pc->compacted};
+	int active = ps.active, want_residual = ps.want_residual, iter = ps.iter;
+	ClassCnt n[MULLS_NC];
+#pragma unroll
+	for (int c = 0; c < MULLS_NC; c++)
+		n[c] = ClassCnt{pd[c].alive_cur, pd[c].tgt_n, pd[c].valid_next, pd[c].n_valid};
+	asm volatile("" ::: "memory");
+	asm volatile("" : "+s"(active), "+s"(want_residual), "+s"(iter), "+s"(d.src_n), "+s"(d.src_c), "+s"(d.compacted), "+v"(lw.alive), "+v"(lw.below));
+#pragma unroll
+	for (int c = 0; c < MULLS_NC; c++)
+		asm volatile("" : "+s"(n[c].alive_cur), "+s"(n[c].tgt_n), "+s"(n[c].valid_next), "+s"(n[c].n_valid));
+	if (!active && !want_residual)
+		return;
+	const bool residual_pass = want_residual != 0;
 	int cnt[MULLS_NC];
+#pragma unroll
 	for (int c = 0; c < MULLS_NC; c++)
-		cnt[c] = (int)(class_called(rp, pd[c], c) ? pd[c].valid_next : pd[c].n_valid);
-	const AccumCtx A = accum_ctx(rp, job.cls, ps.iter, residual_pass, class_weight(rp, job.cls, residual_pass, cnt));
-	const CloudDesc &d = pd[job.cls];
-	const uint32_t ci = job.pair * MULLS_NC + job.cls;
-	double *out = partial + (size_t)job_idx * MULLS_NTERM;
-	if (d.src_n <= job.start)
+		cnt[c] = class_count(rp, c, residual_pass, n[c]);
+	const AccumCtx A = accum_ctx(rp, (int)tr.cls, iter, residual_pass, class_weight(rp, (int)tr.cls, false, cnt));
+	double *out = partial + (size_t)tr.job * MULLS_NTERM;
+	if (d.src_n <= tr.start)
 	{
 		if (part == 0u && (threadIdx.x & 63u) < MULLS_NTERM)
 			out[threadIdx.x & 63u] = 0.0;
@@ -205,34 +217,34 @@
 		if (part)
 			return;
 		if (!residual_pass)
-			wave_trip<double, 12, 1, 1, 0, 12>(A, ps.x, d, job.start, spos, mq, flag, wd, out, true, rp.live_mask, ci);
+			wave_trip<double, 12, 1, 1, 0, 12>(A, ps.x, d, tr.start, spos, mq, flag, wd, out, true, lw);
 		else if (A.metric == 0)
-			wave_trip<double, 2, 0, 0, 0, 2>(A, ps.x, d, job.start, spos, mq, flag, wd, out, true, rp.live_mask, ci);
+			wave_trip<double, 2, 0, 0, 0, 2>(A, ps.x, d, tr.start, spos, mq, flag, wd, out, true, lw);
 		else if (A.metric == 1)
-			wave_trip<double, 2, 0, 1, 0, 2>(A, ps.x, d, job.start, spos, mq, flag, wd, out, true, rp.live_mask, ci);
+			wave_trip<double, 2, 0, 1, 0, 2>(A, ps.x, d, tr.start, spos, mq, flag, wd, out, true, lw);
 		else
-			wave_trip<double, 2, 0, 2, 0, 2>(A, ps.x, d, job.start, spos, mq, flag, wd, out, true, rp.live_mask, ci);
+			wave_trip<double, 2, 0, 2, 0, 2>(A, ps.x, d, tr.start, spos, mq, flag, wd, out, true, lw);
 	}
 #if MULLS_ACCW_SPLIT == 2
 	else if (A.metric == 0)
 	{
 		if (part == 0u)
-			wave_trip<float, 27, 0, 0, 0, 14>(A, ps.x, d, job.start, spos, mq, flag, wd, out, true, rp.live_mask, ci);
+			wave_trip<float, 27, 0, 0, 0, 14>(A, ps.x, d, tr.start, spos, mq, flag, wd, out, true, lw);
 		else
-			wave_trip<float, 27, 0, 0, 14, 13>(A, ps.x, d, job.start, spos, mq, flag, wd, out, false, rp.live_mask, ci);
+			wave_trip<float, 27, 0, 0, 14, 13>(A, ps.x, d, tr.start, spos, mq, flag, wd, out, false, lw);
 	}
 	else
 	{
 		if (part == 0u)
-			wave_trip<float, 27, 0, 2, 0, 14>(A, ps.x, d, job.start, spos, mq, flag, wd, out, true, rp.live_mask, ci);
+			wave_trip<float, 27, 0, 2, 0, 14>(A, ps.x, d, tr.start, spos, mq, flag, wd, out, true, lw);
 		else
-			wave_trip<float, 27, 0, 2, 14, 13>(A, ps.x, d, job.start, spos, mq, flag, wd, out, false, rp.live_mask, ci);
+			wave_trip<float, 27, 0, 2, 14, 13>(A, ps.x, d, tr.start, spos, mq, flag, wd, out, false, lw);
 	}
 #else
 	else if (A.metric == 0)
-		wave_trip<float, 27, 0, 0, 0, 27>(A, ps.x, d, job.start, spos, mq, flag, wd, out, true, rp.live_mask, ci);
+		wave_trip<float, 27, 0, 0, 0, 27>(A, ps.x, d, tr.start, spos, mq, flag, wd, out, true, lw);
 	else
-		wave_trip<float, 27, 0, 2, 0, 27>(A, ps.x, d, job.start, spos, mq, flag, wd, out, true, rp.live_mask, ci);
+		wave_trip<float, 27, 0, 2, 0, 27>(A, ps.x, d, tr.start, spos, mq, flag, wd, out, true, lw);
 #endif
 }
 
@@ -685,7 +697,8 @@
 
 __global__ __launch_bounds__(64) void k_sum_step(CloudDesc *__restrict__ descs, PairState *__restrict__ states, RunParams rp, mulls::IcpConst K,
 												 const double *__restrict__ partial, PairOut *__restrict__ out, const uint32_t *__restrict__ bbox,
-												 mulls::StepState *__restrict__ steps, IcpOut *__restrict__ results, int brute, uint32_t pair_base)
+												 mulls::StepState *__restrict__ steps, IcpOut *__restrict__ results, int brute, uint32_t pair_base,
+												 unsigned long long *__restrict__ tick, volatile unsigned long long *host_word, uint32_t epoch)
 {
 	__shared__ StepLds L;
 	__shared__ FinishLds F;
@@ -705,7 +718,27 @@
 		L.comb[threadIdx.x] = F.comb[threadIdx.x];
 	if (threadIdx.x < 30u)
 		L.cnt[threadIdx.x] = F.cnt[threadIdx.x];
-	(void)step_pair(pair, descs, states, rp, K, out, steps, results, brute, L, sw);
+	const bool left = step_pair(pair, descs, states, rp, K, out, steps, results, brute, L, sw);
+	if (threadIdx.x == 0)
+	{
+		const uint32_t group = blockIdx.x >> 6, n_groups = (gridDim.x + 63u) >> 6, in_group = min(64u, gridDim.x - (group << 6));
+		unsigned long long *gw = tick + (size_t)(group + 1u) * MULLS_STEP_TICK_STRIDE;
+		const unsigned long long mine = ((unsigned long long)(left ? 1u : 0u) << 32) | 1ull;
+		const unsigned long long old = atomicAdd(gw, mine);
+		if ((uint32_t)old == in_group - 1u)
+		{
+			*gw = 0ull;
+			const unsigned long long group_left = (old + mine) >> 32;
+			const unsigned long long old_top = atomicAdd(tick, (group_left << 32) | 1ull);
+			if ((uint32_t)old_top == n_groups - 1u)
+			{
+				const uint32_t n_left = (uint32_t)((old_top >> 32) + group_left);
+				*tick = 0ull;
+				__threadfence_system();
+				*host_word = (unsigned long long)epoch << 32 | n_left;
+			}
+		}
+	}
 }
 
 __global__ __launch_bounds__(MULLS_BLOCK) void k_finish_step(CloudDesc *__restrict__ descs, PairState *__restrict__ states, RunParams rp, mulls::IcpConst K,
@@ -824,7 +857,7 @@
 	const uint32_t n_trips = split[3] - split[0];
 	if (accum_takes_waves(rp, split, wave_min_trips))
 	{
-		hipLaunchKernelGGL(k_accum_wave, dim3((n_trips + MULLS_ACCW_WAVES / MULLS_ACCW_SPLIT - 1u) / (MULLS_ACCW_WAVES / MULLS_ACCW_SPLIT)), dim3(64 * MULLS_ACCW_WAVES), 0, st, b.ajobs + split[0], n_trips, b.jobs, b.descs, b.states, rp, b.spos,
+		hipLaunchKernelGGL(k_accum_wave, dim3((n_trips + MULLS_ACCW_WAVES / MULLS_ACCW_SPLIT - 1u) / (MULLS_ACCW_WAVES / MULLS_ACCW_SPLIT)), dim3(64 * MULLS_ACCW_WAVES), 0, st, b.atrips + split[0], n_trips, b.descs, b.states, rp, b.spos,
 						   b.mq, b.flag, b.wd, b.partial);
 		return;
 	}
@@ -870,7 +903,7 @@
 }
 
 void launch_finish_step(hipStream_t st, const BatchDev &b, const RunParams &rp, const mulls::IcpConst &K, uint32_t pair_base, uint32_t npairs, unsigned long long *host_word, uint32_t epoch,
-						int brute, uint32_t *ticket, bool sum_step)
+						int brute, uint32_t *ticket, bool sum_step, unsigned long long *step_tick)
 {
 	if (!npairs)
 		return;
@@ -880,8 +913,12 @@
 						   pair_base);
 		return;
 	}
-	if (sum_step && rp.pull_comb)
-		hipLaunchKernelGGL(k_sum_step, dim3(npairs), dim3(64), 0, st, b.descs, b.states, rp, K, b.partial, b.outs, b.bbox, b.steps, b.icp_outs, brute, pair_base);
+	if (sum_step && rp.pull_comb && step_tick)
+	{
+		hipLaunchKernelGGL(k_sum_step, dim3(npairs), dim3(64), 0, st, b.descs, b.states, rp, K, b.partial, b.outs, b.bbox, b.steps, b.icp_outs, brute, pair_base, step_tick, host_word,
+						   epoch);
+		return;
+	}
 	else
 	{
 		hipLaunchKernelGGL(k_finish, dim3(npairs), dim3(MULLS_BLOCK), 0, st, b.descs, b.states, rp, b.partial, b.outs, b.bbox, pair_base, static_cast<uint4 *>(nullptr),
diff --git a/mulls_amd/csrc/k_search.hip b/mulls_amd/csrc/k_search.hip
--- a/mulls_amd/csrc/k_search.hip
+++ b/mulls_amd/csrc/k_search.hip
@@ -197,7 +197,7 @@
 		return;
 	const float thr = ps.thr[job.cls];
 	const FilterCtx F = {d.alive_cur >= 500u, d.n_matched > 0u, job.cls != 5, rp.lds_dedup != 0u && !big, rp.rej_strict != 0, thr * thr, rp.cos_bearing,
-						 (unsigned long long)(0xffffffffu - (rp.tick_base + (uint32_t)ps.iter)) << 32, big ? nullptr : rp.tgt_stage, big ? nullptr : rp.tgt_map};
+						 (unsigned long long)(0xffffffffu - (rp.tick_base + (uint32_t)ps.iter)) << 32, big ? nullptr : rp.tgt_stage, big ? nullptr : rp.tgt_map, tail_stores_d2(rp, job.cls)};
 	uint32_t n_alive = 0, n_valid = 0;
 #pragma unroll
 	for (int u = 0; u < MULLS_SRC_PER_THREAD; u++)
diff --git a/mulls_amd/csrc/launch.h b/mulls_amd/csrc/launch.h
--- a/mulls_amd/csrc/launch.h
+++ b/mulls_amd/csrc/launch.h
@@ -68,6 +68,7 @@
 	uint32_t *bm_cs = nullptr;
 	uint32_t *bm_rank = nullptr;
 	uint32_t *ajobs = nullptr;
+	TripRec *atrips = nullptr;
 	IcpOut *icp_outs = nullptr;
 	mulls::StepState *steps = nullptr;
 	uint32_t *wl = nullptr;
@@ -105,6 +106,6 @@
 void launch_push_states(hipStream_t st, const BatchDev &b, uint32_t pair_base, uint32_t npairs);
 void launch_step_init(hipStream_t st, const BatchDev &b, const mulls::IcpConst &K, uint32_t npairs);
 void launch_finish_step(hipStream_t st, const BatchDev &b, const RunParams &rp, const mulls::IcpConst &K, uint32_t pair_base, uint32_t npairs, unsigned long long *host_word, uint32_t epoch,
-						int brute, uint32_t *ticket = nullptr, bool sum_step = false);
+						int brute, uint32_t *ticket = nullptr, bool sum_step = false, unsigned long long *step_tick = nullptr);
 void launch_transform_aos(hipStream_t st, float4 *recs, uint32_t n, const double *T12);
 void launch_set_corr(hipStream_t st, const BatchDev &b, uint32_t src_off, const int32_t *cs, const int32_t *ct, const float *cd, uint32_t n, uint32_t tgt_off);
diff --git a/mulls_amd/csrc/lds_tier.h b/mulls_amd/csrc/lds_tier.h
--- a/mulls_amd/csrc/lds_tier.h
+++ b/mulls_amd/csrc/lds_tier.h
@@ -8,6 +8,7 @@
 	unsigned long long key_hi;
 	const float4 *tgt_stage;
 	const uint16_t *tgt_map;
+	bool store_d2;
 };
 __device__ __forceinline__ void filter_point(const FilterCtx &F, const CloudDesc &d, uint32_t s, const float4 *__restrict__ snrm,
 											  const float4 *__restrict__ tnrm, uint8_t *__restrict__ flag, const int32_t *__restrict__ nn_idx,
@@ -37,7 +38,8 @@
 			valid = F.strict ? dist < F.max_sqr : !(dist > F.max_sqr);
 			if (valid)
 			{
-				wd[g] = dist;
+				if (F.store_d2)
+					wd[g] = dist;
 				if (match[g] == m)
 					n2 = mq[2u * g + 1u];
 				else
@@ -541,7 +543,7 @@
 	for (int w = 0; w < BLK / 64; w++)
 		total_matched += red[w];
 	const float thr = ps.thr[job.cls];
-	const FilterCtx F = {C.gate, total_matched > 0u, job.cls != 5, true, rp.rej_strict != 0, thr * thr, rp.cos_bearing, C.key_hi, rp.tgt_stage, rp.tgt_map};
+	const FilterCtx F = {C.gate, total_matched > 0u, job.cls != 5, true, rp.rej_strict != 0, thr * thr, rp.cos_bearing, C.key_hi, rp.tgt_stage, rp.tgt_map, tail_stores_d2(rp, job.cls)};
 	uint32_t n_alive = 0, n_valid = 0;
 	for (uint32_t s = job.start + threadIdx.x; s < q_end; s += BLK)
 		filter_point(F, d, s, snrm, tnrm, flag, nn_idx, nn_d2, match, wd, winner, tpos, mq, n_alive, n_valid);
@@ -634,6 +636,7 @@
 		total_matched += red[w];
 	const float thr = ps.thr[job.cls], max_sqr = thr * thr;
 	const bool any_match = total_matched > 0u, normal_check = job.cls != 5, strict = rp.rej_strict != 0;
+	const bool store_d2 = tail_stores_d2(rp, job.cls);
 	uint32_t n_alive = 0, n_valid = 0;
 #pragma unroll
 	for (int k = 0; k < TRIPS; k++)
@@ -662,7 +665,7 @@
 				valid = strict ? dist < max_sqr : !(dist > max_sqr);
 				if (valid)
 				{
-					if (!COMPACT)
+					if (!COMPACT && store_d2)
 						wd[gi] = dist;
 					if (PM[k] != m)
 					{
@@ -766,7 +769,7 @@
 #endif
 				flag[ci] = (uint8_t)(nf & (MULLS_F_ALIVE | MULLS_F_VALID));
 				match[ci] = M[k];
-				if (nf & MULLS_F_VALID)
+				if ((nf & MULLS_F_VALID) && store_d2)
 					wd[ci] = D[k];
 				if (nf & 8u)
 				{
@@ -1352,7 +1355,7 @@
 	FLAT_TICK(3)
 
 	const float thr = ps.thr[job.cls], max_sqr = thr * thr;
-	const bool any_match = total_matched > 0u, strict = rp.rej_strict != 0;
+	const bool any_match = total_matched > 0u, strict = rp.rej_strict != 0, store_d2 = tail_stores_d2(rp, job.cls);
 	uint32_t n_alive = 0, n_valid = 0;
 #pragma unroll
 	for (int k = 0; k < TRIPS; k++)
@@ -1399,7 +1402,7 @@
 					}
 				}
 				valid = strict ? dist < max_sqr : !(dist > max_sqr);
-				if (valid)
+				if (valid && store_d2)
 					wd[gi] = dist;
 			}
 		}
diff --git a/mulls_amd/csrc/loop.cpp b/mulls_amd/csrc/loop.cpp
--- a/mulls_amd/csrc/loop.cpp
+++ b/mulls_amd/csrc/loop.cpp
@@ -317,12 +317,21 @@
 		volatile unsigned long long *word = nullptr;
 		unsigned long long *word_dev = nullptr;
 		uint32_t *epoch_ctr = nullptr, *ticket = nullptr, *wl = nullptr, *wl_ctr = nullptr;
+		unsigned long long *step_tick = nullptr;
 		uint32_t epoch0 = 0, nn_launches = 0, left = 0;
 		int s = 0;
 		bool done = false;
 		EvTimer ev2[2] = {EvTimer{nullptr}, EvTimer{nullptr}};
 	};
 	const int nsub = B->nsub;
+	const bool step_ticks = sum_step && rp.pull_comb && !(few_launches || n <= (int)ctx->opt[MULLS_OPT_STEP_LAUNCH_MAX_PAIRS]);
+	const size_t tick_words = step_tick_words((uint32_t)((n + nsub - 1) / nsub));
+	if (step_ticks)
+	{
+		if (grow(ctx, &B->step_tick, &B->cap_step_tick, tick_words * (size_t)nsub) != MULLS_OK)
+			return MULLS_E_HIP;
+		HIPCHK(ctx, hipMemsetAsync(B->step_tick, 0, sizeof(unsigned long long) * tick_words * (size_t)nsub, st));
+	}
 	Sub subs[2];
 	for (int k = 0; k < nsub; k++)
 	{
@@ -330,6 +339,7 @@
 		S.lo = (int)((long)n * k / nsub);
 		S.hi = (int)((long)n * (k + 1) / nsub);
 		S.L = slice_of(B, S.lo, S.hi, k);
+		S.step_tick = step_ticks ? B->step_tick + tick_words * (size_t)k : nullptr;
 		S.st = k == 0 ? ctx->stream : ctx->stream2;
 		S.word = reinterpret_cast<volatile unsigned long long *>(B->epoch_h + 32 + 16 * k);
 		S.word_dev = reinterpret_cast<unsigned long long *>(B->epoch_dev + 32 + 16 * k);
@@ -418,7 +428,7 @@
 		ev.begin(search ? &ctx->prof.ms_accum : &ctx->prof.ms_residual);
 		launch_accum(sst, *B, rp, S.L.ajob_split, few_launches, (uint32_t)ctx->opt[MULLS_OPT_ACCUM_WAVE_MIN_TRIPS]);
 		launch_finish_step(sst, *B, rp, R.K, (uint32_t)S.lo, (uint32_t)(S.hi - S.lo), S.word_dev, ++*S.epoch_ctr, R.use_grid ? 0 : 1,
-						   (few_launches || n <= (int)ctx->opt[MULLS_OPT_STEP_LAUNCH_MAX_PAIRS]) ? S.ticket : nullptr, sum_step);
+						   (few_launches || n <= (int)ctx->opt[MULLS_OPT_STEP_LAUNCH_MAX_PAIRS]) ? S.ticket : nullptr, sum_step, S.step_tick);
 		ev.end();
 		{
 			const hipError_t e = hipGetLastError();
diff --git a/mulls_amd/csrc/stage.cpp b/mulls_amd/csrc/stage.cpp
--- a/mulls_amd/csrc/stage.cpp
+++ b/mulls_amd/csrc/stage.cpp
@@ -259,6 +259,7 @@
 			rp.win_pl = rp.win_li = rp.win_pt = window;
 			rp.force_class_w = 1;
 			rp.class_w_value = class_weight;
+			rp.store_w = 1;
 			hipStream_t st = ctx->stream;
 			hipError_t e = hipSuccess;
 			if (dmalloc(ctx, &dcs, ncorr) != MULLS_OK || dmalloc(ctx, &dct, ncorr) != MULLS_OK || dmalloc(ctx, &dcd, ncorr) != MULLS_OK)
```

Result: faster. 320,800 (median of 6 runs) (+3.7%).
